# mauro3/KissMCMC.jl

Measured on AMD Instinct MI355X. Metric: walker-steps/sec, higher is better.
Workload: dtype f64

## Files before the change

include/kissmcmc_hip.h:

```cpp
#ifndef KISSMCMC_HIP_H
#define KISSMCMC_HIP_H

#include <stdint.h>

#ifdef __cplusplus
extern "C" {
#endif

#define KMC_VERSION 100

typedef enum kmc_status {
    KMC_OK = 0,
    KMC_ERR_A_SCALE = 1,
    KMC_ERR_ODD_WALKERS = 2,
    KMC_ERR_TOO_FEW_WALKERS = 3,
    KMC_ERR_BAD_ARG = 4,
    KMC_ERR_NONFINITE_LOGP = 5,
    KMC_ERR_HIP = 6,
    KMC_ERR_OOM = 7,
    KMC_ERR_NO_DEVICE = 8,
    KMC_ERR_UNSUPPORTED = 9
} kmc_status;

typedef enum kmc_density {
// ... 220 lines not shown
    int64_t  nchains;
    int64_t  ndim;
    int64_t  niter;
    int64_t  nburnin;
    int64_t  nthin;
    const double* step;
    uint64_t seed;
    uint32_t flags;
    int32_t  device;
    void*    user_density;
    kmc_host_logpdf_fn   host_logpdf;
    void*                host_user;
    kmc_host_accepted_fn host_accepted;
    kmc_host_propose_fn  host_propose;
} kmc_metropolis_config;

typedef struct kmc_metropolis_outputs {
    double*  chain;
    double*  chain_logp;
    double*  accept_ratio;
    int64_t* naccept;
    double*  final_pos;
    double*  final_logp;
    double*  chain_sum;
    double*  chain_sumsq;
    int64_t  nsamples;
    double   device_ms;
    double*  blobs;
    double*  final_blob;
} kmc_metropolis_outputs;

kmc_status  kmc_metropolis_validate(const kmc_metropolis_config* cfg);
kmc_status  kmc_metropolis_run(const kmc_metropolis_config* cfg, const double* theta0 ,
                               kmc_metropolis_outputs* out);

kmc_status  kmc_int_acorr(const double* chain_host, int64_t nsamples, int64_t nwalkers, int64_t ndim, double c ,
                          int device, double* tau , double* converged );
kmc_status  kmc_sampler_int_acorr(kmc_sampler* s, double c, double* tau, double* converged);

kmc_status  kmc_sampler_order_stats(kmc_sampler* s, int64_t first_sample, const uint8_t* walker_mask ,
                                    const int64_t* ranks, int32_t nranks,
                                    double* theta_out , double* logp_out , int64_t* n_out);
kmc_status  kmc_sampler_chain_argmax(kmc_sampler* s, int64_t first_sample, const uint8_t* walker_mask,
                                     int64_t* sample, int64_t* walker, double* theta , double* logp);
kmc_status  kmc_chain_order_stats(const double* chain_host , const double* logp_host ,
                                  int64_t nsamples, int64_t nwalkers, int64_t ndim, int64_t first_sample, const uint8_t* walker_mask,
                                  const int64_t* ranks, int32_t nranks, int device, double* theta_out, double* logp_out, int64_t* n_out);
kmc_status  kmc_chain_argmax(const double* chain_host, const double* logp_host, int64_t nsamples, int64_t nwalkers, int64_t ndim,
                             int64_t first_sample, const uint8_t* walker_mask, int device,
                             int64_t* sample, int64_t* walker, double* theta, double* logp);

kmc_status  kmc_sampler_histograms(kmc_sampler* s, int64_t first_sample, const uint8_t* walker_mask ,
                                   const int32_t* dims, int32_t ndims, const double* edges , int32_t nbins,
                                   int32_t with_logp, int64_t* counts1 , int64_t* outside ,
                                   int64_t* counts2 , int64_t* n_out);
kmc_status  kmc_chain_histograms(const double* chain_host , const double* logp_host ,
                                 int64_t nsamples, int64_t nwalkers, int64_t ndim, int64_t first_sample, const uint8_t* walker_mask,
                                 const int32_t* dims, int32_t ndims, const double* edges, int32_t nbins, int device,
                                 int64_t* counts1, int64_t* outside, int64_t* counts2, int64_t* n_out);
kmc_status  kmc_hist_pair_plan(int32_t ndims, int32_t nbins, int32_t* pairs_per_group, int32_t* ngroups, int32_t* lds_budget);

#define KMC_CONV_NEED_LAGS 1
#define KMC_CONV_TRUNCATED 2
kmc_status  kmc_sampler_lag_sums(kmc_sampler* s, int64_t first_sample, const uint8_t* walker_mask , int32_t split,
                                 int32_t with_logp, int64_t lag0, int64_t nlags, double* chain_mean, double* chain_var, double* lagsum,
                                 int64_t* m_out, int64_t* h_out);
kmc_status  kmc_chain_lag_sums(const double* chain_host , const double* logp_host ,
                               int64_t nsamples, int64_t nwalkers, int64_t ndim, int64_t first_sample, const uint8_t* walker_mask,
                               int32_t split, int64_t lag0, int64_t nlags, int device, double* chain_mean, double* chain_var,
                               double* lagsum, int64_t* m_out, int64_t* h_out);
kmc_status  kmc_convergence_stats(int64_t m, int64_t h, int64_t ncols, const double* chain_mean, const double* chain_var,
                                  const double* lagsum, int64_t nlags, int64_t max_lag, double* mean, double* W, double* B,
                                  double* var_plus, double* rhat, double* ess, double* mcse, int64_t* T, int32_t* flags);
kmc_status  kmc_sampler_convergence(kmc_sampler* s, int64_t first_sample, const uint8_t* walker_mask, int32_t split, int32_t with_logp,
                                    int64_t max_lag, double* mean, double* W, double* B, double* var_plus, double* rhat, double* ess,
                                    double* mcse, int64_t* T, int32_t* flags, int64_t* m_out, int64_t* h_out, int64_t* info);
kmc_status  kmc_convergence_plan(int32_t* lag_block, int32_t* tile_samples, int32_t* lanes, int32_t* lds_bytes);
kmc_status  kmc_chain_convergence(const double* chain_host, const double* logp_host , int64_t nsamples, int64_t nwalkers,
                                  int64_t ndim, int64_t first_sample, const uint8_t* walker_mask, int32_t split, int64_t max_lag,
                                  int device, double* mean, double* W, double* B, double* var_plus, double* rhat, double* ess,
                                  double* mcse, int64_t* T, int32_t* flags, int64_t* m_out, int64_t* h_out, int64_t* info);
kmc_status  kmc_convergence_plan(int32_t* lag_block, int32_t* tile_samples, int32_t* lanes, int32_t* lds_bytes);

#define KMC_CONV_HAS_NAN 4
kmc_status  kmc_rank_plan(int32_t* tile_keys, int32_t* digit_bits, int32_t* passes, int32_t* lds_bytes);
kmc_status  kmc_rank_normal_scores(const int64_t* rank2, int64_t n, int64_t S, double* z);
kmc_status  kmc_sampler_rank_scores(kmc_sampler* s, int64_t first_sample, const uint8_t* walker_mask , int32_t split,
                                    int32_t with_logp, int32_t folded, int64_t* rank2, double* z, double* centre, int64_t* nan_count,
                                    int64_t* m_out, int64_t* h_out);
kmc_status  kmc_chain_rank_scores(const double* chain_host , const double* logp_host ,
                                  int64_t nsamples, int64_t nwalkers, int64_t ndim, int64_t first_sample, const uint8_t* walker_mask,
                                  int32_t split, int32_t folded, int device, int64_t* rank2, double* z, double* centre,
                                  int64_t* nan_count, int64_t* m_out, int64_t* h_out);
kmc_status  kmc_sampler_rank_convergence(kmc_sampler* s, int64_t first_sample, const uint8_t* walker_mask, int32_t split, int32_t with_logp,
                                         int64_t max_lag, double* rhat, double* rhat_bulk, double* rhat_folded, double* ess_bulk,
                                         double* ess_tail, double* ess_q05, double* ess_q95, double* median, double* q05, double* q95,
                                         int64_t* T, int32_t* flags, int64_t* m_out, int64_t* h_out, int64_t* info);
kmc_status  kmc_chain_rank_convergence(const double* chain_host, const double* logp_host , int64_t nsamples, int64_t nwalkers,
                                       int64_t ndim, int64_t first_sample, const uint8_t* walker_mask, int32_t split, int64_t max_lag,
                                       int device, double* rhat, double* rhat_bulk, double* rhat_folded, double* ess_bulk,
                                       double* ess_tail, double* ess_q05, double* ess_q95, double* median, double* q05, double* q95,
                                       int64_t* T, int32_t* flags, int64_t* m_out, int64_t* h_out, int64_t* info);

kmc_status  kmc_sampler_covariance(kmc_sampler* s, int64_t first_sample, const uint8_t* walker_mask ,
                                   int32_t with_logp, double* mean, double* cov, int64_t* n_out, int64_t* info);
kmc_status  kmc_chain_covariance(const double* chain_host , const double* logp_host ,
                                 int64_t nsamples, int64_t nwalkers, int64_t ndim, int64_t first_sample, const uint8_t* walker_mask,
                                 int device, double* mean, double* cov, int64_t* n_out, int64_t* info);
kmc_status  kmc_cov_plan(int64_t ncols, int32_t* tile_cols, int32_t* strip_tiles, int32_t* nstrips, int32_t* rows_per_wave_block);
kmc_status  kmc_cov_correlation(int64_t ncols, const double* cov, double* corr, double* sd);

kmc_status  kmc_sampler_pointwise_stats(kmc_sampler* s, int64_t first_sample, const uint8_t* walker_mask ,
                                        int64_t thin, const double* data , int64_t ndata2, int32_t ncols2,
                                        double* stats, int64_t* n_out, int64_t* info);
kmc_status  kmc_chain_pointwise_stats(kmc_user_density* density, const double* params, const double* chain_host ,
                                      int64_t nsamples, int64_t nwalkers, int64_t ndim, int64_t first_sample, const uint8_t* walker_mask,
                                      int64_t thin, const double* data, int64_t ndata2, int32_t ncols2, int device, double* stats,
                                      int64_t* n_out, int64_t* info);
kmc_status  kmc_sampler_pointwise_loglike(kmc_sampler* s, int64_t first_sample, const uint8_t* walker_mask, int64_t thin, const double* data,
                                          int64_t ndata2, int32_t ncols2, int64_t obs_first, int64_t obs_count, double* out, int64_t* n_out);
kmc_status  kmc_chain_pointwise_loglike(kmc_user_density* density, const double* params, const double* chain_host, int64_t nsamples,
                                        int64_t nwalkers, int64_t ndim, int64_t first_sample, const uint8_t* walker_mask, int64_t thin,
                                        const double* data, int64_t ndata2, int32_t ncols2, int64_t obs_first, int64_t obs_count, int device,
                                        double* out, int64_t* n_out);
kmc_status  kmc_pointwise_plan(int64_t n, int64_t ndata, int64_t* run_len, int64_t* nruns, int32_t* lanes_per_run, int32_t* slots,
                               int64_t* nwaves);
kmc_status  kmc_waic_stats(int64_t J, int64_t n, const double* stats, double* lppd_j, double* p_waic_j, double* elpd_j, double* totals);

kmc_status  kmc_sampler_psis_loo(kmc_sampler* s, int64_t first_sample, const uint8_t* walker_mask , int64_t thin,
                                 double r_eff, int64_t obs_first, int64_t obs_count, int64_t workspace_bytes, double* stats, double* lppd_j,
                                 int64_t* n_out, int64_t* info);
kmc_status  kmc_chain_psis_loo(kmc_user_density* density, const double* params, const double* chain_host ,
                               int64_t nsamples, int64_t nwalkers, int64_t ndim, int64_t first_sample, const uint8_t* walker_mask, int64_t thin,
                               double r_eff, int64_t obs_first, int64_t obs_count, int64_t workspace_bytes, int device, double* stats,
                               double* lppd_j, int64_t* n_out, int64_t* info);
kmc_status  kmc_sampler_psis_tail(kmc_sampler* s, int64_t first_sample, const uint8_t* walker_mask, int64_t thin, double r_eff, int64_t obs_first,
                                  int64_t obs_count, int64_t workspace_bytes, double* tail, double* m_j, double* xc_j, int32_t* n_tail_j,
                                  int64_t* tail_len, int64_t* n_out);
kmc_status  kmc_chain_psis_tail(kmc_user_density* density, const double* params, const double* chain_host, int64_t nsamples, int64_t nwalkers,
                                int64_t ndim, int64_t first_sample, const uint8_t* walker_mask, int64_t thin, double r_eff, int64_t obs_first,
                                int64_t obs_count, int64_t workspace_bytes, int device, double* tail, double* m_j, double* xc_j,
                                int32_t* n_tail_j, int64_t* tail_len, int64_t* n_out);
kmc_status  kmc_psis_plan(int64_t n, int64_t ndata, double r_eff, int64_t workspace_bytes, int64_t* tail_len, int64_t* m_est,
                          int64_t* obs_per_block, int64_t* passes);
kmc_status  kmc_loo_stats(int64_t J, int64_t n, const double* stats, const double* lppd_j, double* p_loo_j, double* totals);
kmc_status  kmc_psis_smooth_host(int64_t nt, const double* x, double xc, double* k_hat, double* sigma, double* s, double* sums);

kmc_status  kmc_debug_accept_terms(uint64_t seed, uint64_t step, uint64_t walker0, int64_t n, int64_t nhalf, double a_scale,
                                   int64_t ndim, int device, int64_t* partner_host, double* z_host, double* t1_host, double* lu_host);
kmc_status  kmc_debug_chain_by_walker(const void* src_host, int is_float, int64_t K, int64_t nl, int64_t ld, int64_t nd, int64_t w0,
                                      int64_t nw, int64_t dst_stride, double* dst_host, int64_t dst_len, int device);
kmc_status  kmc_debug_rows_compact(const double* src_host, int64_t rows, int64_t ld, int64_t nd, double* dst_host, int64_t dst_len,
                                   int device);

#ifdef __cplusplus
}
#endif
#endif
```

kissmcmc.jl_amd/_lib.py:

```python
from __future__ import annotations

import ctypes as C
import os

_HERE = os.path.dirname(os.path.abspath(__file__))
LIB_PATH = os.environ.get("KMC_LIB_PATH") or os.path.join(_HERE, "libkissmcmc_hip.so")

OK, ERR_A_SCALE, ERR_ODD_WALKERS, ERR_TOO_FEW_WALKERS, ERR_BAD_ARG, ERR_NONFINITE_LOGP, \
    ERR_HIP, ERR_OOM, ERR_NO_DEVICE, ERR_UNSUPPORTED = range(10)
GAUSSIAN_ISO, EXPONENTIAL, ROSENBROCK, LOGNORMAL, MVNORMAL2 = range(5)
USER_DENSITY = 100
HOST_DENSITY = 101
DATA_DENSITY = 102
HOST_LOGPDF_FN = C.CFUNCTYPE(C.c_int, C.POINTER(C.c_double), C.c_int64, C.c_int64, C.POINTER(C.c_double), C.c_void_p)
HOST_PROPOSE_FN = C.CFUNCTYPE(C.c_int, C.POINTER(C.c_double), C.c_int64, C.c_int64, C.POINTER(C.c_double), C.c_void_p)
HOST_ACCEPTED_FN = C.CFUNCTYPE(C.c_int, C.POINTER(C.c_uint8), C.c_int64, C.c_int64, C.c_int64, C.c_int32, C.c_void_p)
F64 = 0
F32 = 1
STORE_CHAIN, STORE_LOGP, MOMENTS, NO_GRAPH, P2P, ISLANDS, P2P_FINEGRAINED, P2P_PUSH = 1, 2, 4, 8, 16, 64, 128, 512
STREAM_CHAIN = 2048
CHAIN_BY_WALKER = 4096
STORE_BLOBS = 8192
MOVE_STRETCH, MOVE_DE, MOVE_SNOOKER, MOVE_MIX = 0, 1, 3, 4
MIX_MAX = 4
TEMPS_MAX = 64
CONV_NEED_LAGS, CONV_TRUNCATED = 1, 2
CONV_HAS_NAN = 4
TEMPER_WHOLE, TEMPER_LIKELIHOOD = 0, 1
P2P_HANDLE_BYTES = 128
RCCL_ID_BYTES = 128

SYMBOLS = [
    "kmc_version", "kmc_device_count", "kmc_last_error", "kmc_status_string", "kmc_validate",
    "kmc_g_pdf", "kmc_cdf_g_inv", "kmc_emcee_run", "kmc_sampler_create", "kmc_sampler_destroy",
    "kmc_sampler_set_stream", "kmc_sampler_bind_positions", "kmc_sampler_p2p_export", "kmc_sampler_p2p_connect", "kmc_sampler_p2p_connect_local", "kmc_sampler_p2p_link_probe", "kmc_sampler_set_positions", "kmc_sampler_init_ball", "kmc_sampler_set_state", "kmc_sampler_run", "kmc_sampler_half_step",
    "kmc_sampler_sync", "kmc_sampler_last_run_ms", "kmc_sampler_generation", "kmc_sampler_nsamples",
    "kmc_sampler_launch_count", "kmc_sampler_describe", "kmc_sampler_device_ptr", "kmc_sampler_get_positions",
    "kmc_sampler_get_logp", "kmc_sampler_get_naccept", "kmc_sampler_get_accept_ratio",
    "kmc_sampler_get_moments", "kmc_sampler_get_chain", "kmc_sampler_get_chain_by_walker", "kmc_logpdf_eval", "kmc_logpdf_eval_host",
    "kmc_user_density_create", "kmc_user_density_create_body", "kmc_user_density_destroy", "kmc_metropolis_validate", "kmc_metropolis_run", "kmc_int_acorr", "kmc_sampler_int_acorr",
    "kmc_sizeof_config", "kmc_sizeof_metropolis_config", "kmc_sizeof_outputs", "kmc_sizeof_metropolis_outputs", "kmc_deal_seed", "kmc_deal_perm", "kmc_sampler_deal_pack", "kmc_sampler_deal_unpack",
    "kmc_sampler_get_walker_ids", "kmc_sampler_set_walker_ids", "kmc_sampler_set_chain_host", "kmc_rccl_unique_id", "kmc_sampler_rccl_init",
    "kmc_sampler_rccl_capture", "kmc_sampler_rccl_set_capture", "kmc_rccl_version", "kmc_device_free_bytes",
    "kmc_sampler_launch_mode", "kmc_updated_budget", "kmc_set_updated_budget_mb", "kmc_debug_accept_terms",
    "kmc_debug_chain_by_walker", "kmc_debug_rows_compact",
    "kmc_user_density_create_body_blob", "kmc_user_density_nblob", "kmc_logpdf_blob_eval_host", "kmc_sampler_get_blobs",
    "kmc_device_cache_release", "kmc_user_density_is_separable", "kmc_host_prefault", "kmc_data_density_create",
    "kmc_sampler_get_rung_state", "kmc_sampler_set_rung_state", "kmc_sampler_get_swaps",
    "kmc_sampler_get_rung_loglike", "kmc_sampler_set_rung_loglike_sum", "kmc_sampler_get_ladder", "kmc_sampler_set_ladder",
    "kmc_sampler_order_stats", "kmc_sampler_chain_argmax", "kmc_chain_order_stats", "kmc_chain_argmax",
    "kmc_sampler_histograms", "kmc_chain_histograms", "kmc_hist_pair_plan",
    "kmc_sampler_lag_sums", "kmc_chain_lag_sums", "kmc_convergence_stats", "kmc_sampler_convergence", "kmc_chain_convergence",
    "kmc_convergence_plan",
    "kmc_rank_plan", "kmc_rank_normal_scores", "kmc_sampler_rank_scores", "kmc_chain_rank_scores", "kmc_sampler_rank_convergence",
    "kmc_chain_rank_convergence",
    "kmc_sampler_covariance", "kmc_chain_covariance", "kmc_cov_plan", "kmc_cov_correlation",
    "kmc_sampler_pointwise_stats", "kmc_chain_pointwise_stats", "kmc_sampler_pointwise_loglike", "kmc_chain_pointwise_loglike",
    "kmc_pointwise_plan", "kmc_waic_stats",
    "kmc_sampler_psis_loo", "kmc_chain_psis_loo", "kmc_sampler_psis_tail", "kmc_chain_psis_tail", "kmc_psis_plan", "kmc_loo_stats",
    "kmc_psis_smooth_host",
]


class Config(C.Structure):
    _fields_ = [
        ("dtype", C.c_int32),
        ("density", C.c_int32),
        ("params", C.c_double * 8),
        ("nwalkers", C.c_int64),
        ("ndim", C.c_int64),
        ("ngenerations", C.c_int64),
        ("nburnin", C.c_int64),
        ("nthin", C.c_int64),
        ("a_scale", C.c_double),
        ("seed", C.c_uint64),
        ("flags", C.c_uint32),
        ("device", C.c_int32),
        ("shard_rank", C.c_int32),
        ("shard_count", C.c_int32),
        ("user_density", C.c_void_p),
        ("island_gens", C.c_int32),
        ("island_size", C.c_int32),
        ("host_logpdf", C.c_void_p),
        ("host_user", C.c_void_p),
        ("host_accepted", C.c_void_p),
        ("deal_rank", C.c_int32),
        ("deal_count", C.c_int32),
        ("temper_mode", C.c_int32),
        ("temper_pad_", C.c_int32),
        ("adapt_until", C.c_int64),
        ("adapt_lag", C.c_double),
        ("adapt_time", C.c_double),
        ("adapt", C.c_int32),
        ("adapt_pad_", C.c_int32),
        ("snooker_gamma", C.c_double),
        ("mix_count", C.c_int32),
        ("mix_move0", C.c_int32), ("mix_move1", C.c_int32), ("mix_move2", C.c_int32), ("mix_move3", C.c_int32),
        ("mix_pad0_", C.c_int32), ("mix_pad1_", C.c_int32), ("mix_pad2_", C.c_int32),
        ("mix_weight0", C.c_double), ("mix_weight1", C.c_double), ("mix_weight2", C.c_double), ("mix_weight3", C.c_double),
        ("mix_gamma0", C.c_double), ("mix_gamma1", C.c_double), ("mix_gamma2", C.c_double), ("mix_gamma3", C.c_double),
        ("mix_sigma0", C.c_double), ("mix_sigma1", C.c_double), ("mix_sigma2", C.c_double), ("mix_sigma3", C.c_double),
        ("betas", C.c_void_p),
        ("ntemps", C.c_int32),
        ("swap_every", C.c_int32),
        ("move", C.c_int32),
        ("move_pad_", C.c_int32),
        ("de_gamma0", C.c_double),
        ("de_sigma", C.c_double),
    ]


class Outputs(C.Structure):
    _fields_ = [
        ("chain", C.POINTER(C.c_double)),
        ("chain_logp", C.POINTER(C.c_double)),
        ("accept_ratio", C.POINTER(C.c_double)),
        ("naccept", C.POINTER(C.c_int64)),
        ("final_pos", C.POINTER(C.c_double)),
        ("final_logp", C.POINTER(C.c_double)),
        ("sum", C.POINTER(C.c_double)),
        ("sumsq", C.POINTER(C.c_double)),
        ("nmoment", C.c_int64),
        ("nsamples", C.c_int64),
        ("device_ms", C.c_double),
        ("blobs", C.POINTER(C.c_double)),
    ]


class MetropolisConfig(C.Structure):
    _fields_ = [
        ("dtype", C.c_int32),
        ("density", C.c_int32),
        ("params", C.c_double * 8),
        ("nchains", C.c_int64),
        ("ndim", C.c_int64),
        ("niter", C.c_int64),
        ("nburnin", C.c_int64),
        ("nthin", C.c_int64),
        ("step", C.POINTER(C.c_double)),
        ("seed", C.c_uint64),
        ("flags", C.c_uint32),
        ("device", C.c_int32),
        ("user_density", C.c_void_p),
        ("host_logpdf", C.c_void_p),
        ("host_user", C.c_void_p),
        ("host_accepted", C.c_void_p),
        ("host_propose", C.c_void_p),
    ]


class MetropolisOutputs(C.Structure):
    _fields_ = [
        ("chain", C.POINTER(C.c_double)),
        ("chain_logp", C.POINTER(C.c_double)),
        ("accept_ratio", C.POINTER(C.c_double)),
        ("naccept", C.POINTER(C.c_int64)),
        ("final_pos", C.POINTER(C.c_double)),
        ("final_logp", C.POINTER(C.c_double)),
        ("chain_sum", C.POINTER(C.c_double)),
        ("chain_sumsq", C.POINTER(C.c_double)),
        ("nsamples", C.c_int64),
        ("device_ms", C.c_double),
        ("blobs", C.POINTER(C.c_double)),
        ("final_blob", C.POINTER(C.c_double)),
    ]


class KmcError(RuntimeError):

    def __init__(self, status: int, message: str):
        super().__init__(message)
        self.status = status


_lib = None


def lib() -> C.CDLL:
    global _lib
    if _lib is not None:
        return _lib
    if "no-torch-preload" not in os.environ.get("KMC_DEBUG", "").split(","):
        try:
            import torch
        except Exception:
            pass
    if not os.path.exists(LIB_PATH):
        raise ImportError(
            f"{LIB_PATH} is missing: build it with `python -m kissmcmc_jl_amd.build` "
            "(hipcc --offload-arch=gfx950). The emcee hot path has no CPU fallback.")
    L = C.CDLL(LIB_PATH)
    dp = C.POINTER(C.c_double)
    ip = C.POINTER(C.c_int64)
    vp = C.c_void_p
    cfgp = C.POINTER(Config)
    L.kmc_version.restype = C.c_int
    L.kmc_device_count.restype = C.c_int
    L.kmc_last_error.restype = C.c_char_p
    L.kmc_status_string.restype = C.c_char_p
    L.kmc_status_string.argtypes = [C.c_int]
    L.kmc_validate.argtypes = [cfgp]
    L.kmc_g_pdf.restype = C.c_double
    L.kmc_g_pdf.argtypes = [C.c_double, C.c_double]
    L.kmc_cdf_g_inv.restype = C.c_double
    L.kmc_cdf_g_inv.argtypes = [C.c_double, C.c_double]
    L.kmc_emcee_run.argtypes = [cfgp, dp, C.POINTER(Outputs)]
    L.kmc_sampler_create.argtypes = [cfgp, C.POINTER(vp)]
    L.kmc_sampler_destroy.restype = None
    L.kmc_sampler_destroy.argtypes = [vp]
    L.kmc_sampler_set_stream.argtypes = [vp, vp]
    L.kmc_sampler_bind_positions.argtypes = [vp, vp]
    L.kmc_sampler_p2p_export.argtypes = [vp, vp]
    L.kmc_sampler_p2p_connect.argtypes = [vp, vp]
    L.kmc_sampler_p2p_connect_local.argtypes = [vp, C.POINTER(C.c_void_p)]
    L.kmc_sampler_p2p_link_probe.argtypes = [vp, C.c_int, C.c_int64, C.c_int, C.POINTER(C.c_double), C.POINTER(C.c_double)]
    L.kmc_sampler_set_positions.argtypes = [vp, dp]
    L.kmc_sampler_init_ball.argtypes = [vp, dp, dp, C.c_uint64, C.c_int, C.c_int]
    L.kmc_sampler_set_state.argtypes = [vp, dp, dp, ip, C.c_int64]
    L.kmc_sampler_get_rung_state.argtypes = [vp, dp, dp, ip, dp]
    L.kmc_sampler_set_rung_state.argtypes = [vp, dp, dp, ip, C.POINTER(C.c_uint64), dp, C.c_int64]
    L.kmc_sampler_get_swaps.argtypes = [vp, C.POINTER(C.c_uint64)]
    L.kmc_sampler_get_rung_loglike.argtypes = [vp, dp, dp, dp]
    L.kmc_sampler_set_rung_loglike_sum.argtypes = [vp, dp]
    L.kmc_sampler_get_ladder.argtypes = [vp, dp, dp, C.POINTER(C.c_uint64), C.POINTER(C.c_uint64)]
    L.kmc_sampler_set_ladder.argtypes = [vp, dp, dp, C.POINTER(C.c_uint64), C.POINTER(C.c_uint64)]
    L.kmc_sampler_run.argtypes = [vp, C.c_int64]
    L.kmc_sampler_half_step.argtypes = [vp, C.c_int]
    L.kmc_sampler_sync.argtypes = [vp]
    L.kmc_sampler_last_run_ms.argtypes = [vp, dp]
    L.kmc_sampler_generation.restype = C.c_int64
    L.kmc_sampler_generation.argtypes = [vp]
    L.kmc_sampler_nsamples.restype = C.c_int64
    L.kmc_sampler_nsamples.argtypes = [vp]
    L.kmc_sampler_launch_count.restype = C.c_int64
    L.kmc_sampler_launch_count.argtypes = [vp]
    L.kmc_sampler_describe.argtypes = [vp, C.c_char_p, C.c_int64]
    L.kmc_sampler_device_ptr.restype = vp
    L.kmc_sampler_device_ptr.argtypes = [vp, C.c_int]
    L.kmc_sampler_get_positions.argtypes = [vp, dp]
    L.kmc_sampler_get_logp.argtypes = [vp, dp]
    L.kmc_sampler_get_naccept.argtypes = [vp, ip]
    L.kmc_sampler_get_accept_ratio.argtypes = [vp, dp]
    L.kmc_sampler_get_moments.argtypes = [vp, dp, dp, ip]
    L.kmc_sampler_get_chain.argtypes = [vp, dp, dp]
    L.kmc_sampler_get_chain_by_walker.argtypes = [vp, dp, dp]
    L.kmc_logpdf_eval.argtypes = [cfgp, vp, vp, C.c_int64, vp]
    L.kmc_logpdf_eval_host.argtypes = [cfgp, dp, dp, C.c_int64]
    L.kmc_user_density_create.argtypes = [C.c_char_p, C.c_char_p, C.POINTER(vp)]
    L.kmc_user_density_create_body.argtypes = [C.c_char_p, C.POINTER(vp)]
    L.kmc_user_density_create_body_blob.argtypes = [C.c_char_p, C.c_int, C.POINTER(vp)]
    L.kmc_data_density_create.argtypes = [C.c_char_p, C.c_char_p, C.POINTER(C.c_double), C.c_int64, C.c_int32, C.POINTER(vp)]
    L.kmc_user_density_is_separable.restype = C.c_int
    L.kmc_user_density_is_separable.argtypes = [vp]
    L.kmc_user_density_nblob.restype = C.c_int
    L.kmc_user_density_nblob.argtypes = [vp]
    L.kmc_logpdf_blob_eval_host.argtypes = [cfgp, dp, dp, dp, C.c_int64]
    L.kmc_sampler_get_blobs.argtypes = [vp, dp, dp, C.c_int]
    L.kmc_user_density_destroy.restype = None
    L.kmc_user_density_destroy.argtypes = [vp]
    L.kmc_metropolis_validate.argtypes = [C.POINTER(MetropolisConfig)]
    L.kmc_metropolis_run.argtypes = [C.POINTER(MetropolisConfig), dp, C.POINTER(MetropolisOutputs)]
    L.kmc_int_acorr.argtypes = [dp, C.c_int64, C.c_int64, C.c_int64, C.c_double, C.c_int, dp, dp]
    L.kmc_sampler_int_acorr.argtypes = [vp, C.c_double, dp, dp]
    bp = C.POINTER(C.c_uint8)
    L.kmc_sampler_order_stats.argtypes = [vp, C.c_int64, bp, ip, C.c_int32, dp, dp, ip]
    L.kmc_sampler_chain_argmax.argtypes = [vp, C.c_int64, bp, ip, ip, dp, dp]
    L.kmc_chain_order_stats.argtypes = [dp, dp, C.c_int64, C.c_int64, C.c_int64, C.c_int64, bp, ip, C.c_int32, C.c_int, dp, dp, ip]
    L.kmc_chain_argmax.argtypes = [dp, dp, C.c_int64, C.c_int64, C.c_int64, C.c_int64, bp, C.c_int, ip, ip, dp, dp]
    i32p = C.POINTER(C.c_int32)
    L.kmc_sampler_histograms.argtypes = [vp, C.c_int64, bp, i32p, C.c_int32, dp, C.c_int32, C.c_int32, ip, ip, ip, ip]
    L.kmc_chain_histograms.argtypes = [dp, dp, C.c_int64, C.c_int64, C.c_int64, C.c_int64, bp, i32p, C.c_int32, dp, C.c_int32, C.c_int, ip, ip, ip, ip]
    L.kmc_hist_pair_plan.argtypes = [C.c_int32, C.c_int32, i32p, i32p, i32p]
    L.kmc_sampler_lag_sums.argtypes = [vp, C.c_int64, bp, C.c_int32, C.c_int32, C.c_int64, C.c_int64, dp, dp, dp, ip, ip]
    L.kmc_chain_lag_sums.argtypes = [dp, dp, C.c_int64, C.c_int64, C.c_int64, C.c_int64, bp, C.c_int32, C.c_int64, C.c_int64, C.c_int, dp, dp, dp, ip, ip]
    L.kmc_convergence_stats.argtypes = [C.c_int64, C.c_int64, C.c_int64, dp, dp, dp, C.c_int64, C.c_int64, dp, dp, dp, dp, dp, dp, dp, ip, i32p]
    L.kmc_sampler_convergence.argtypes = [vp, C.c_int64, bp, C.c_int32, C.c_int32, C.c_int64, dp, dp, dp, dp, dp, dp, dp, ip, i32p, ip, ip, ip]
    L.kmc_chain_convergence.argtypes = [dp, dp, C.c_int64, C.c_int64, C.c_int64, C.c_int64, bp, C.c_int32, C.c_int64, C.c_int, dp, dp, dp, dp, dp, dp, dp, ip, i32p, ip, ip, ip]
    L.kmc_convergence_plan.argtypes = [i32p, i32p, i32p, i32p]
    L.kmc_rank_plan.argtypes = [i32p, i32p, i32p, i32p]
    L.kmc_rank_normal_scores.argtypes = [ip, C.c_int64, C.c_int64, dp]
    L.kmc_sampler_rank_scores.argtypes = [vp, C.c_int64, bp, C.c_int32, C.c_int32, C.c_int32, ip, dp, dp, ip, ip, ip]
    L.kmc_chain_rank_scores.argtypes = [dp, dp, C.c_int64, C.c_int64, C.c_int64, C.c_int64, bp, C.c_int32, C.c_int32, C.c_int, ip, dp, dp, ip, ip, ip]
    L.kmc_sampler_rank_convergence.argtypes = [vp, C.c_int64, bp, C.c_int32, C.c_int32, C.c_int64] + [dp] * 10 + [ip, i32p, ip, ip, ip]
    L.kmc_chain_rank_convergence.argtypes = [dp, dp, C.c_int64, C.c_int64, C.c_int64, C.c_int64, bp, C.c_int32, C.c_int64, C.c_int] + [dp] * 10 + [ip, i32p, ip, ip, ip]
    L.kmc_sampler_covariance.argtypes = [vp, C.c_int64, bp, C.c_int32, dp, dp, ip, ip]
    L.kmc_chain_covariance.argtypes = [dp, dp, C.c_int64, C.c_int64, C.c_int64, C.c_int64, bp, C.c_int, dp, dp, ip, ip]
    L.kmc_cov_plan.argtypes = [C.c_int64, i32p, i32p, i32p, i32p]
    L.kmc_cov_correlation.argtypes = [C.c_int64, dp, dp, dp]
    held_out = [dp, C.c_int64, C.c_int32]
    host_chain = [vp, dp, dp, C.c_int64, C.c_int64, C.c_int64, C.c_int64, bp, C.c_int64]
    L.kmc_sampler_pointwise_stats.argtypes = [vp, C.c_int64, bp, C.c_int64] + held_out + [dp, ip, ip]
    L.kmc_chain_pointwise_stats.argtypes = host_chain + held_out + [C.c_int, dp, ip, ip]
    L.kmc_sampler_pointwise_loglike.argtypes = [vp, C.c_int64, bp, C.c_int64] + held_out + [C.c_int64, C.c_int64, dp, ip]
    L.kmc_chain_pointwise_loglike.argtypes = host_chain + held_out + [C.c_int64, C.c_int64, C.c_int, dp, ip]
    L.kmc_pointwise_plan.argtypes = [C.c_int64, C.c_int64, ip, ip, i32p, i32p, ip]
    L.kmc_waic_stats.argtypes = [C.c_int64, C.c_int64, dp, dp, dp, dp, dp]
    psis_sel = [C.c_double, C.c_int64, C.c_int64, C.c_int64]
    L.kmc_sampler_psis_loo.argtypes = [vp, C.c_int64, bp, C.c_int64] + psis_sel + [dp, dp, ip, ip]
    L.kmc_chain_psis_loo.argtypes = host_chain + psis_sel + [C.c_int, dp, dp, ip, ip]
    L.kmc_sampler_psis_tail.argtypes = [vp, C.c_int64, bp, C.c_int64] + psis_sel + [dp, dp, dp, i32p, ip, ip]
    L.kmc_chain_psis_tail.argtypes = host_chain + psis_sel + [C.c_int, dp, dp, dp, i32p, ip, ip]
    L.kmc_psis_plan.argtypes = [C.c_int64, C.c_int64, C.c_double, C.c_int64, ip, ip, ip, ip]
    L.kmc_loo_stats.argtypes = [C.c_int64, C.c_int64, dp, dp, dp, dp]
    L.kmc_psis_smooth_host.argtypes = [C.c_int64, dp, C.c_double, dp, dp, dp, dp]
    L.kmc_deal_seed.restype = C.c_uint64
    L.kmc_deal_seed.argtypes = [C.c_uint64, C.c_int32]
    L.kmc_deal_perm.argtypes = [C.c_uint64, C.c_int64, C.c_int32, C.c_int64, ip, ip]
    L.kmc_sampler_deal_pack.argtypes = [vp, C.c_int64, vp]
    L.kmc_sampler_deal_unpack.argtypes = [vp, vp]
    L.kmc_sampler_get_walker_ids.argtypes = [vp, ip]
    L.kmc_sampler_set_walker_ids.argtypes = [vp, ip]
    L.kmc_sampler_set_chain_host.argtypes = [vp, dp, dp]
    L.kmc_rccl_unique_id.argtypes = [vp]
    L.kmc_sampler_rccl_init.argtypes = [vp, vp]
    L.kmc_sampler_rccl_capture.argtypes = [vp, C.POINTER(C.c_int)]
    L.kmc_sampler_rccl_set_capture.argtypes = [vp, C.c_int]
    L.kmc_rccl_version.argtypes = [C.POINTER(C.c_int), C.c_char_p, C.c_int64]
    L.kmc_device_free_bytes.argtypes = [C.c_int, C.POINTER(C.c_uint64), C.POINTER(C.c_uint64)]
    L.kmc_device_cache_release.argtypes = []
    L.kmc_device_cache_release.restype = None
    L.kmc_host_prefault.argtypes = [C.c_void_p, C.c_uint64, C.c_int]
    L.kmc_host_prefault.restype = None
    L.kmc_sampler_launch_mode.restype = C.c_int
    L.kmc_sampler_launch_mode.argtypes = [vp, C.POINTER(C.c_int)]
    L.kmc_updated_budget.restype = None
    L.kmc_updated_budget.argtypes = [ip, ip]
    L.kmc_set_updated_budget_mb.restype = None
    L.kmc_set_updated_budget_mb.argtypes = [C.c_double]
    L.kmc_debug_accept_terms.argtypes = [C.c_uint64, C.c_uint64, C.c_uint64, C.c_int64, C.c_int64, C.c_double, C.c_int64, C.c_int, ip, dp, dp, dp]
    L.kmc_debug_chain_by_walker.argtypes = [vp, C.c_int, C.c_int64, C.c_int64, C.c_int64, C.c_int64, C.c_int64, C.c_int64, C.c_int64, dp, C.c_int64, C.c_int]
    L.kmc_debug_rows_compact.argtypes = [dp, C.c_int64, C.c_int64, C.c_int64, dp, C.c_int64, C.c_int]
    for fn, T in ((L.kmc_sizeof_config, Config), (L.kmc_sizeof_metropolis_config, MetropolisConfig),
                  (L.kmc_sizeof_outputs, Outputs), (L.kmc_sizeof_metropolis_outputs, MetropolisOutputs)):
        if fn() != C.sizeof(T):
            raise ImportError(f"{LIB_PATH}: struct layout mismatch ({fn.__name__}() = {fn()}, the ctypes mirror {T.__name__} is {C.sizeof(T)} bytes): "
                              "rebuild the library or update kissmcmc_jl_amd/_lib.py from include/kissmcmc_hip.h")
    _lib = L
    return L


def check(status: int) -> None:
    if status != OK:
        L = lib()
        msg = L.kmc_last_error().decode() or L.kmc_status_string(status).decode()
        raise KmcError(status, msg)
```

kissmcmc.jl_amd/build.py:

```python
from __future__ import annotations

import os
import shutil
import subprocess

_HERE = os.path.dirname(os.path.abspath(__file__))
CSRC = os.path.join(_HERE, "csrc")
LIB = os.path.join(_HERE, "libkissmcmc_hip.so")
SOURCES = ["kmc_sampler.hip", "kmc_plan.hip", "kmc_launch.hip", "kmc_updated.hip", "kmc_state.hip", "kmc_copy.hip", "kmc_rtc.hip", "kmc_p2p.hip", "kmc_metropolis_api.hip", "kmc_acorr.hip", "kmc_summary.hip", "kmc_hist.hip", "kmc_convergence.hip", "kmc_rank.hip", "kmc_cov.hip", "kmc_pointwise.hip", "kmc_rccl.hip", "kmc_diag.hip", "kmc_inst_host.hip", "kmc_inst_host_temper.hip", "kmc_inst_host_temper_snooker.hip", "kmc_data.hip"] + \
          [f"kmc_inst_{d}{part}.hip" for part in ("", "_var", "_p2p", "_lds", "_de", "_snooker", "_temper", "_temper_snooker") for d in ("lognormal", "exponential", "gaussian_iso", "rosenbrock", "mvnormal2")]
HEADERS = ["kmc_psis_fit.hpp", "kmc_host.hpp", "kmc_sampler.hpp", "kmc_device.hpp", "kmc_kernels.hpp", "kmc_islands.hpp", "kmc_generation.hpp", "kmc_copy_kernels.hpp", "kmc_summary_kernels.hpp", "kmc_hist_kernels.hpp", "kmc_convergence_kernels.hpp", "kmc_convergence_host.hpp", "kmc_rank_kernels.hpp", "kmc_cov_kernels.hpp", "kmc_chain_view.hpp", "kmc_chain_kernels.hpp", "kmc_metropolis.hpp", "kmc_tables.hpp", "kmc_recognise.hpp", "kmc_data.hpp", "kmc_pointwise.hpp", os.path.join("..", "..", "include", "kissmcmc_hip.h")]
PRELOAD = ["-mllvm", "-amdgpu-kernarg-preload-count=14"]
FLAGS = ["--offload-arch=gfx950", "-O3", "-std=c++17", "-fPIC", "-ffp-contract=off",
         "-fvisibility=hidden", "-Wall", "-Wno-unused-function"]


def _hipcc() -> str:
    for c in (shutil.which("hipcc"), "/opt/rocm/bin/hipcc"):
        if c and os.path.exists(c):
            return c
    raise RuntimeError("hipcc not found: the HIP library cannot be built")




def stale(lib: str = LIB) -> bool:
    if not os.path.exists(lib):
        return True
    t = os.path.getmtime(lib)
    deps = [os.path.join(CSRC, f) for f in SOURCES + HEADERS]
    return any(os.path.getmtime(d) > t for d in deps)


def build(force: bool = False, verbose: bool = False, extra_flags=(), out: str = LIB, preload: bool = True) -> str:
    if not (force or out != LIB or stale()):
        return out
    from concurrent.futures import ThreadPoolExecutor
    hipcc = _hipcc()
    objdir = os.path.join(_HERE, "build_obj" + ("" if out == LIB else "_" + os.path.basename(out)))
    os.makedirs(objdir, exist_ok=True)

    def compile_one(src):
        obj = os.path.join(objdir, os.path.splitext(src)[0] + ".o")
        cmd = [hipcc, *FLAGS, *(PRELOAD if preload else ()), *extra_flags, "-c", os.path.join(CSRC, src), "-o", obj]
        if verbose:
            print(" ".join(cmd))
        subprocess.check_call(cmd)
        return obj

    order = sorted(SOURCES, key=lambda f: not f.startswith("kmc_inst_"))
    with ThreadPoolExecutor(max_workers=min(len(SOURCES), os.cpu_count() or 1)) as ex:
        objs = list(ex.map(compile_one, order))
    cmd = [hipcc, "--offload-arch=gfx950", "-shared", "-fPIC", *objs, "-o", out + ".tmp", "-lhiprtc", "-ldl"]
    if verbose:
        print(" ".join(cmd))
    subprocess.check_call(cmd)
    os.replace(out + ".tmp", out)
    shutil.rmtree(objdir, ignore_errors=True)
    return out


if __name__ == "__main__":
    print(build(force=True, verbose=True))
```

kissmcmc.jl_amd/csrc/kmc_kernels.hpp:

```cpp
#pragma once
#include "kmc_device.hpp"

namespace kmc {

constexpr int kTPB = 256;
__host__ __device__ constexpr int vec_tpb(int L) { return L <= 8 ? 128 : L == 16 ? 64 : kTPB; }

struct SchedEntry {
    int64_t  gen;
    int64_t  slot;
    uint32_t flags;
    uint32_t nbefore;
    uint32_t pad_[2];
};
static_assert(sizeof(SchedEntry) == 32, "schedule_of loads an entry as eight dwords");
enum : uint32_t { kCount = 1u, kSample = 2u };

__host__ __device__ inline SchedEntry make_sched(int64_t gen, int64_t nburnin, int64_t nthin, int64_t nsamples, int64_t ring_slots = 0)
{
    SchedEntry e{gen, 0, 0u, 0u, {0u, 0u}};
    const int64_t n = gen + 1 - nburnin;
    if (n > 1) {
        const int64_t nb = (n - 1) / nthin;
        e.nbefore = (uint32_t)(nb < nsamples ? nb : nsamples);
    }
    if (n > 0) {
        e.flags |= kCount;
        if (n % nthin == 0) {
            const int64_t k = n / nthin - 1;
            if (k < nsamples) { e.flags |= kSample; e.slot = ring_slots > 0 ? k % ring_slots : k; }
        }
    }
    return e;
}

struct HalfStepArgs {
    double*           pos;
    double*           logp;
    uint32_t*         naccept;
    const SchedEntry* sched_table;
    SchedEntry        sched_inline;
    int32_t           sched_index;
    int32_t           half;
    int64_t           gw0;
    int64_t           own_row0;
    int64_t           oth_row0;
    int32_t           n_active;
    int32_t           ndim;
    int32_t           ld;
    int32_t           hloc_shift;
    uint32_t          hloc;
    int32_t           nranks;
    double*           peer_pos[8];
    const unsigned long long* flags;
    unsigned long long* err;
    DrawConsts        dc;
    DensityParams     dp;
    double*           chain;
    double*           chain_logp;
    int64_t           chain_rows;
    int64_t           chain_row0;
    double*           msum;
    double*           msumsq;
    int64_t           macc_stride;
    uint32_t*         klast;
    double2*          ring;
    int64_t           ring_rows;
    int32_t           ring_slot;
    int32_t           prop_ld;
    double*           prop_out;
    const double*     p1_in;
    unsigned char*    acc_out;
    double2*          mring;
    double*           mring_w;
    uint32_t*         mcnt;
    const uint32_t*   mswept;
    int32_t           mring_depth;
    double*           blob;
    double*           chain_blob;
};

__host__ __device__ inline int32_t pack_ranks(int nranks, int me, bool push) { return (int32_t)(nranks | (me << 8) | (push ? 1 << 16 : 0)); }
__device__ __forceinline__ int  p2p_nranks(const HalfStepArgs& a) { return a.nranks & 0xff; }
__device__ __forceinline__ int  p2p_me(const HalfStepArgs& a) { return (a.nranks >> 8) & 0xff; }
__device__ __forceinline__ bool p2p_push(const HalfStepArgs& a) { return ((a.nranks >> 16) & 1) != 0; }

struct HalfStepFront {
    double*           pos;
    const SchedEntry* sched;
    const double2*    ring_now;
    double*           logp;
    uint32_t          gw0;
    uint32_t          nact_half;
    uint32_t          seed_lo, seed_hi, nhalf;
    uint32_t          step;
    __host__ __device__ int32_t n_active() const { return (int32_t)(nact_half & 0x7fffffffu); }
    __host__ __device__ int32_t half() const { return (int32_t)(nact_half >> 31); }
};
#define KMC_FRONT_PARAMS double* f_pos, const kmc::SchedEntry* f_sched, const double2* f_ring_now, double* f_logp, uint32_t f_gw0, \
                         uint32_t f_nact_half, uint32_t f_seed_lo, uint32_t f_seed_hi, uint32_t f_nhalf, uint32_t f_step
#define KMC_FRONT_PACK kmc::HalfStepFront{f_pos, f_sched, f_ring_now, f_logp, f_gw0, f_nact_half, f_seed_lo, f_seed_hi, f_nhalf, f_step}
#define KMC_FRONT_TYPES double*, const kmc::SchedEntry*, const double2*, double*, uint32_t, uint32_t, uint32_t, uint32_t, uint32_t, uint32_t

__device__ __forceinline__ SchedEntry schedule_entry(const HalfStepFront& f)
{
    typedef uint32_t u32x8 __attribute__((ext_vector_type(8)));
    u32x8 r;
    asm volatile("s_load_dwordx8 %0, %1, 0x0\n\ts_waitcnt lgkmcnt(0)" : "=s"(r) : "s"(f.sched));
    SchedEntry t;
    t.gen     = (int64_t)(((uint64_t)r[1] << 32) | r[0]);
    t.slot    = (int64_t)(((uint64_t)r[3] << 32) | r[2]);
    t.flags   = r[4];
    t.nbefore = r[5];
    return t;
}
__device__ __forceinline__ SchedEntry schedule_of(const HalfStepFront& f, const HalfStepArgs& a)
{
    if (f.sched == nullptr) return a.sched_inline;
    return schedule_entry(f);
}

__device__ __forceinline__ void store_wt(double2* p, const double2& v)
{
    typedef double v2d __attribute__((ext_vector_type(2)));
    const v2d t = {v.x, v.y};
    asm volatile("global_store_dwordx4 %0, %1, off sc0 sc1\n\ts_nop 1" :: "v"(p), "v"(t) : "memory");
}
__device__ __forceinline__ void store_wt(double* p, double v)
{
    asm volatile("global_store_dwordx2 %0, %1, off sc0 sc1\n\ts_nop 1" :: "v"(p), "v"(v) : "memory");
}
__device__ __forceinline__ void store_wt(uint32_t* p, uint32_t v)
{
    asm volatile("global_store_dword %0, %1, off sc0 sc1\n\ts_nop 0" :: "v"(p), "v"(v) : "memory");
}
__device__ __forceinline__ void store_wt(unsigned char* p, unsigned char v)
{
    const uint32_t t = v;
    asm volatile("global_store_byte %0, %1, off sc0 sc1\n\ts_nop 0" :: "v"(p), "v"(t) : "memory");
}
__device__ __forceinline__ double2 load_row16(const double2* p)
{
    return *p;
}

template <class T> struct RowOf;
template <> struct RowOf<double> { using V2 = double2; };
template <> struct RowOf<float>  { using V2 = float2; };
__device__ __forceinline__ void store_wt(float2* p, const float2& v)
{
    typedef float v2f __attribute__((ext_vector_type(2)));
    const v2f t = {v.x, v.y};
    asm volatile("global_store_dwordx2 %0, %1, off sc0 sc1\n\ts_nop 1" :: "v"(p), "v"(t) : "memory");
}
__device__ __forceinline__ double2 load_row(const double2* p) { return load_row16(p); }
__device__ __forceinline__ double2 load_row(const float2* p) { const float2 v = *p; return make_double2((double)v.x, (double)v.y); }
__device__ __forceinline__ void store_row(double2* p, const double2& v) { store_wt(p, v); }
__device__ __forceinline__ void store_row(float2* p, const double2& v) { store_wt(p, make_float2((float)v.x, (float)v.y)); }
template <class T> __device__ __forceinline__ double as_stored(double v)
{
    if constexpr (sizeof(T) == 4) return (double)(float)v; else return v;
}

__device__ __forceinline__ double2 sel2(bool c, const double2& a, const double2& b)
{
    return make_double2(c ? a.x : b.x, c ? a.y : b.y);
}

template <int L, int K>
struct FoldT {
    static constexpr bool on = (K == 2) && (L == 8 || L == 16 || L == 32);
    static constexpr int NVL = on ? (8 * L) / 64 : 1;
};

__device__ __forceinline__ double swap16_sum(double a, double b)
{
    const auto lo = __builtin_amdgcn_permlane16_swap((unsigned)__double2loint(a), (unsigned)__double2loint(b), false, false);
    const auto hi = __builtin_amdgcn_permlane16_swap((unsigned)__double2hiint(a), (unsigned)__double2hiint(b), false, false);
    return __hiloint2double((int)hi[0], (int)lo[0]) + __hiloint2double((int)hi[1], (int)lo[1]);
}
__device__ __forceinline__ double swap32_sum(double a, double b)
{
    const auto lo = __builtin_amdgcn_permlane32_swap((unsigned)__double2loint(a), (unsigned)__double2loint(b), false, false);
    const auto hi = __builtin_amdgcn_permlane32_swap((unsigned)__double2hiint(a), (unsigned)__double2hiint(b), false, false);
    return __hiloint2double((int)hi[0], (int)lo[0]) + __hiloint2double((int)hi[1], (int)lo[1]);
}

template <int L, int K>
__device__ __forceinline__ void fold_scatter(int lane, const double2 (&ms)[K], const double2 (&mq)[K], double (&v)[8])
{
    static_assert(FoldT<L, K>::on, "K == 2, L = 8 / 16 / 32");
    {
        v[0] = ms[0].x; v[1] = ms[0].y; v[2] = ms[1].x; v[3] = ms[1].y; v[4] = mq[0].x; v[5] = mq[0].y; v[6] = mq[1].x; v[7] = mq[1].y;
        int n = 8;
        if constexpr (L == 8) {
            const bool hi = (lane & 8) != 0;
#pragma unroll
            for (int i = 0; i < 4; ++i) {
                double lo_v = v[i], hi_v = v[i + 4];
                asm volatile("" : "+v"(lo_v), "+v"(hi_v));
                const double keep = hi ? hi_v : lo_v, send = hi ? lo_v : hi_v;
                v[i] = keep + dpp_f64<0x128>(send);
            }
            n = 4;
        }
        if constexpr (L <= 16) {
#pragma unroll
            for (int i = 0; i < 4; ++i) if (i < n / 2) v[i] = swap16_sum(v[i], v[i + n / 2]);
            n /= 2;
        }
#pragma unroll
        for (int i = 0; i < 4; ++i) if (i < n / 2) v[i] = swap32_sum(v[i], v[i + n / 2]);
    }
}

template <int L, int K, bool HAVE_OLD>
__device__ __forceinline__ void accumulate_wave(double* msum, double* msumsq, int64_t stride, int tid, int g,
                                                double2 (&ms)[K], double2 (&mq)[K],
                                                const double2 (&olds)[K], const double2 (&oldq)[K], const double (&oldt)[4])
{
    if constexpr (FoldT<L, K>::on) {
        constexpr int NVL = FoldT<L, K>::NVL;
        const int lane = tid & 63;
        double v[8];
        fold_scatter<L, K>(lane, ms, mq, v);
        double* slot = msum + ((int64_t)(tid >> 6) * NVL) * 64 + lane;
#pragma unroll
        for (int r = 0; r < NVL; ++r) store_wt(&slot[r * 64], (HAVE_OLD ? oldt[r] : slot[r * 64]) + v[r]);
        return;
    }
    if constexpr (L < 64) {
#pragma unroll
        for (int k = 0; k < K; ++k) {
            ms[k].x = wave_fold<L>(ms[k].x); ms[k].y = wave_fold<L>(ms[k].y);
            mq[k].x = wave_fold<L>(mq[k].x); mq[k].y = wave_fold<L>(mq[k].y);
        }
    }
    if (g == 0) {
        double2* s = reinterpret_cast<double2*>(msum);
        double2* q = reinterpret_cast<double2*>(msumsq);
#pragma unroll
        for (int k = 0; k < K; ++k) {
            const int64_t idx = (int64_t)k * stride + tid;
            const double2 sv = HAVE_OLD ? olds[k] : s[idx], qv = HAVE_OLD ? oldq[k] : q[idx];
            if constexpr (HAVE_OLD) {
                store_wt(&s[idx], make_double2(sv.x + ms[k].x, sv.y + ms[k].y));
                store_wt(&q[idx], make_double2(qv.x + mq[k].x, qv.y + mq[k].y));
            } else {
                s[idx] = make_double2(sv.x + ms[k].x, sv.y + ms[k].y);
                q[idx] = make_double2(qv.x + mq[k].x, qv.y + mq[k].y);
            }
        }
    }
}

__device__ __forceinline__ void wait_for_peers(const HalfStepArgs& a, unsigned long long need, int lane)
{
    const int nranks = p2p_nranks(a);
    bool ok = lane >= nranks ||
              __hip_atomic_load(a.flags + lane, __ATOMIC_RELAXED, __HIP_MEMORY_SCOPE_SYSTEM) >= need;
    unsigned spins = 0;
    if (__hip_atomic_load(a.err, __ATOMIC_RELAXED, __HIP_MEMORY_SCOPE_AGENT) != 0ull) ok = true;
    while (!__all(ok)) {
        __builtin_amdgcn_s_sleep(2);
        ok = lane >= nranks ||
             __hip_atomic_load(a.flags + lane, __ATOMIC_RELAXED, __HIP_MEMORY_SCOPE_SYSTEM) >= need;
        if (++spins > 30000000u) {
            if (lane == 0) __hip_atomic_store(a.err, need + 1ull, __ATOMIC_RELAXED, __HIP_MEMORY_SCOPE_AGENT);
            break;
        }
    }
    __builtin_amdgcn_fence(__ATOMIC_ACQUIRE, "wavefront");
}

__device__ __forceinline__ double2 load_row_sys(const double2* p)
{
    const unsigned long long* q = reinterpret_cast<const unsigned long long*>(p);
    const unsigned long long lo = __hip_atomic_load(q, __ATOMIC_RELAXED, __HIP_MEMORY_SCOPE_SYSTEM);
    const unsigned long long hi = __hip_atomic_load(q + 1, __ATOMIC_RELAXED, __HIP_MEMORY_SCOPE_SYSTEM);
    return make_double2(__longlong_as_double((long long)lo), __longlong_as_double((long long)hi));
}

#ifdef KMC_PROBE
static __device__ unsigned long long g_probe[2][8192][8];
#define KMC_STAMP_AT(lo, hi) asm volatile("s_memrealtime s[" #lo ":" #hi "]" ::: "s" #lo, "s" #hi, "memory")
#define KMC_STAMP(i) KMC_STAMP_##i
#define KMC_STAMP_0 KMC_STAMP_AT(80, 81)
#define KMC_STAMP_7 KMC_STAMP_AT(94, 95)
#if KMC_PROBE == 2
#define KMC_PROBE_PINS 0
#define KMC_STAMP_1 do { } while (0)
#define KMC_STAMP_2 do { } while (0)
#define KMC_STAMP_3 do { } while (0)
#define KMC_STAMP_4 do { } while (0)
#define KMC_STAMP_5 do { } while (0)
#define KMC_STAMP_6 do { } while (0)
#define KMC_STAMP_READ(dst, lo, hi) do { if ((lo) == 80 || (lo) == 94) asm volatile("s_mov_b64 %0, s[" #lo ":" #hi "]" : "=s"(dst)); else (dst) = 0ull; } while (0)
#else
#define KMC_PROBE_PINS 1
#define KMC_STAMP_1 KMC_STAMP_AT(82, 83)
#define KMC_STAMP_2 KMC_STAMP_AT(84, 85)
#define KMC_STAMP_3 KMC_STAMP_AT(86, 87)
#define KMC_STAMP_4 KMC_STAMP_AT(88, 89)
#define KMC_STAMP_5 KMC_STAMP_AT(90, 91)
#define KMC_STAMP_6 KMC_STAMP_AT(92, 93)
#define KMC_STAMP_READ(dst, lo, hi) asm volatile("s_mov_b64 %0, s[" #lo ":" #hi "]" : "=s"(dst))
#endif
#else
#define KMC_PROBE_PINS 0
#define KMC_STAMP(i) do { } while (0)
#endif

template <class Dens, int L, int K, int ITER, bool P2P, bool RAGGED, class T = double, Move M = Move::Stretch, bool TEMPER = false>
__device__ __forceinline__ void half_step_vec_body(const HalfStepFront& f, const HalfStepArgs& a, const DrawConsts* over = nullptr)
{
    static_assert(!TEMPER || (!P2P && sizeof(T) == 8 && BlobTrait<Dens>::n == 0), "tempering: one GPU, double rows, no blobs (kmc_validate)");
    const uint32_t rung = TEMPER ? (uint32_t)blockIdx.y : 0u;
    const uint32_t rung_w0 = TEMPER ? rung * (2u * f.nhalf) : 0u;
    static_assert(M != Move::Mix, "a mixture picks its member in front of the body (half_step_mix_vec_body)");
    static_assert(L >= 1 && L <= 64 && (L & (L - 1)) == 0, "L must be a power of two <= 64");
    static_assert(!P2P || sizeof(T) == 8, "the peer-to-peer kernels keep double rows");
    constexpr bool kDE = M == Move::DE;
    constexpr bool kSnk = M == Move::Snooker;
    constexpr bool kOwn = kDE || kSnk;
    static_assert(!kOwn || (!P2P && sizeof(T) == 8 && BlobTrait<Dens>::n == 0), "the DE move: one GPU, double rows, no blobs (kmc_validate)");
    using V2 = typename RowOf<T>::V2;
    T* const posT = reinterpret_cast<T*>(f.pos);
    static_assert(ITER >= 1 && ITER <= L, "a group's scalar lanes must cover its iterations");
    constexpr int G = 64 / L;
    constexpr int W = G * ITER;
    const uint64_t ndim_tag = RAGGED ? reinterpret_cast<uint64_t>(f.logp) >> 48 : 0ull;
    double* const logp_p = RAGGED ? reinterpret_cast<double*>(reinterpret_cast<char*>(f.logp) - (ndim_tag << 48)) : f.logp;
    const int ndim = RAGGED ? (int)ndim_tag : 2 * L * K;
    const int64_t ld = RAGGED ? (int64_t)((ndim + 1) & ~1) : (int64_t)(2 * L * K);
    const int tid   = blockIdx.x * vec_tpb(L) + threadIdx.x;
    const int lane  = threadIdx.x & 63;
    const int j     = lane & (L - 1);
    const int g     = lane / L;
    const int gbase = lane & ~(L - 1);
    const int w0    = (tid >> 6) * W;
    const int nact  = f.n_active();
    const int half  = f.half();
    const int64_t own_row0 = P2P ? (int64_t)half * nact : (int64_t)f.gw0;
    bool cv[K];
#pragma unroll
    for (int k = 0; k < K; ++k) cv[k] = !RAGGED || 2 * (k * L + j) < (int)ld;
    int ck[K];
#pragma unroll
    for (int k = 0; k < K; ++k) ck[k] = cv[k] ? k * L + j : (int)(ld >> 1) - 1;
    auto row_off = [&](int64_t row) -> int64_t { return RAGGED ? (int64_t)((uint64_t)(uint32_t)row * (uint64_t)(uint32_t)ld) : row * ld; };
    const double2 zero2 = make_double2(0.0, 0.0);
    KMC_STAMP(0);

    constexpr int Q = (L / ITER) >= 4 ? 4 : (L / ITER);
    constexpr bool kRing = !kOwn && Q >= 2 && L >= 16 && L <= 32;
    const int64_t oth_row0 = (int64_t)(1 - half) * (int64_t)(P2P ? (uint32_t)nact : f.nhalf);
    const int  jq     = j / ITER, js = j - jq * ITER;
    const bool useA   = jq == 0;
    const int  iA     = w0 + (kOwn || jq < Q ? js : 0) * G + g;
    const bool validA = useA && (iA < nact);
    const int      iAc = iA < nact ? iA : nact - 1;
    const int64_t  rowA = own_row0 + iAc;
    const bool ring_on = kRing && f.ring_now != nullptr;
    double2 e0 = zero2, e1 = zero2;
    if constexpr (kRing) {
        if (ring_on && useA) { e0 = f.ring_now[2 * rowA]; e1 = f.ring_now[2 * rowA + 1]; }
    }

    bool    validB[ITER];
    double2 xc[ITER][K], xo[ITER][K];
    double2 xk[ITER][K];
    double2 xl[ITER][K];
#pragma unroll
    for (int it = 0; it < ITER; ++it) {
        const int i = w0 + it * G + g;
        validB[it] = i < nact;
        const V2* own = reinterpret_cast<const V2*>(posT + row_off(own_row0 + (validB[it] ? i : nact - 1)));
#pragma unroll
        for (int k = 0; k < K; ++k) xc[it][k] = load_row(&own[ck[k]]);
    }

    const int64_t nrows_blk = 2 * (int64_t)(P2P ? (uint32_t)nact : f.nhalf);
    uint32_t* const naccept_p = reinterpret_cast<uint32_t*>(logp_p + nrows_blk);
    uint32_t* const klast_p = naccept_p + nrows_blk;
    const double   p0 = logp_p[rowA];
    const uint32_t na = naccept_p[rowA];
    const uint32_t kl = klast_p[rowA];

    const bool eager = f.sched == nullptr;
    SchedEntry sch_t{0, 0, 0u, 0u, {0u, 0u}};
    if (!eager) sch_t = schedule_entry(f);
    const uint64_t step = eager ? (uint64_t)f.step : 2ull * (uint64_t)sch_t.gen + (uint64_t)half;
    DrawConsts dcf{};
    dcf.seed_lo = f.seed_lo; dcf.seed_hi = f.seed_hi; dcf.nhalf = f.nhalf;
    const uint32_t e1y_lo = (uint32_t)__double2loint(e1.y), e1y_hi = (uint32_t)__double2hiint(e1.y);
    const bool fresh = ring_on && __all(!useA || e1y_hi == (uint32_t)step);
    U4 bits{0u, 0u, 0u, 0u};
    uint32_t partnerA = e1y_lo;
    uint32_t partnerK = 0u;
    uint32_t partnerL = 0u;
    if constexpr (kSnk) {
        bits = de_bits(f.seed_lo, f.seed_hi, step, f.gw0 + (uint32_t)iAc + rung_w0, 2u);
        snooker_partners(bits, f.nhalf, &partnerA, &partnerK, &partnerL);
    } else if constexpr (kDE) {
        bits = de_bits(f.seed_lo, f.seed_hi, step, f.gw0 + (uint32_t)iAc + rung_w0, 0u);
        partnerA = __umulhi(bits.x, f.nhalf);
        partnerK = de_partner_k(bits.y, f.nhalf, partnerA);
    } else if (!fresh) {
        bits = draw_bits(dcf, step + 2ull * (uint64_t)jq, (uint64_t)f.gw0 + (uint64_t)iAc + (uint64_t)rung_w0);
        partnerA = draw_partner(dcf, bits);
    }
#if KMC_PROBE_PINS
    if constexpr (!kOwn) asm volatile("" :: "v"(partnerA));
#endif
    KMC_STAMP(1);

    unsigned long long addrA = 0ull;
    const int nranks = P2P ? p2p_nranks(a) : 1, me_rank = P2P ? p2p_me(a) : 0;
    const bool push = P2P && p2p_push(a);
    const int64_t shard_stride = 2 * (int64_t)a.hloc * ld;
    auto load_partner_rows = [&](int it) {
        const V2* oth;
        const V2* othk = nullptr;
        const V2* othl = nullptr;
        if constexpr (!P2P) {
            const uint32_t partner = (uint32_t)__builtin_amdgcn_ds_bpermute((gbase + it) * 4, (int)partnerA);
            const uint32_t pk = kOwn ? (uint32_t)__builtin_amdgcn_ds_bpermute((gbase + it) * 4, (int)partnerK) : 0u;
            oth = reinterpret_cast<const V2*>(posT + row_off(oth_row0 + partner));
            if constexpr (kOwn) othk = reinterpret_cast<const V2*>(posT + row_off(oth_row0 + pk));
            if constexpr (kSnk) {
                const uint32_t pl = (uint32_t)__builtin_amdgcn_ds_bpermute((gbase + it) * 4, (int)partnerL);
                othl = reinterpret_cast<const V2*>(posT + row_off(oth_row0 + pl));
            }
        } else {
            const int src = (gbase + it) * 4;
            const unsigned lo = (unsigned)__builtin_amdgcn_ds_bpermute(src, (int)(unsigned)addrA);
            const unsigned hi = (unsigned)__builtin_amdgcn_ds_bpermute(src, (int)(unsigned)(addrA >> 32));
            const unsigned long long ad = ((unsigned long long)hi << 32) | lo;
            oth = reinterpret_cast<const V2*>(ad);
        }
        if constexpr (P2P) {
            if (nranks > 1) {
#pragma unroll
                for (int k = 0; k < K; ++k) xo[it][k] = load_row_sys(reinterpret_cast<const double2*>(&oth[ck[k]]));
                return;
            }
        }
#pragma unroll
        for (int k = 0; k < K; ++k) xo[it][k] = load_row(&oth[ck[k]]);
        if constexpr (kOwn) {
#pragma unroll
            for (int k = 0; k < K; ++k) xk[it][k] = load_row(&othk[ck[k]]);
        }
        if constexpr (kSnk) {
#pragma unroll
            for (int k = 0; k < K; ++k) xl[it][k] = load_row(&othl[ck[k]]);
        }
    };
    if constexpr (P2P) {
        const uint32_t q = a.hloc_shift >= 0 ? partnerA >> a.hloc_shift : partnerA / a.hloc;
        const uint32_t r = partnerA - q * a.hloc;
        const double* base = a.peer_pos[0];
#pragma unroll
        for (int t = 1; t < 8; ++t) base = (q == (uint32_t)t) ? a.peer_pos[t] : base;
        if (push) base = (q == (uint32_t)me_rank) ? a.pos : a.pos + (int64_t)(1u + q) * shard_stride;
        addrA = (unsigned long long)(base + (oth_row0 + r) * ld);
        if (nranks > 1) {
            if ((threadIdx.x >> 6) == 0) wait_for_peers(a, step, lane);
            __syncthreads();
        }
    }
    constexpr int kFirst = ITER >= 2 && !kSnk ? ITER / 2 : ITER;
#pragma unroll
    for (int it = 0; it < kFirst; ++it) load_partner_rows(it);
    __builtin_amdgcn_sched_barrier(0);
    KMC_STAMP(2);

    asm volatile("" :: "s"(a.chain), "s"(a.chain_logp), "s"(a.chain_rows), "s"(a.chain_row0),
                 "s"(a.msum), "s"(a.msumsq), "s"(a.macc_stride), "s"(a.sched_inline.gen), "s"(a.sched_inline.slot),
                 "s"(a.sched_inline.flags), "s"(a.sched_inline.nbefore));
    int eager_late = eager ? 1 : 0;
    asm volatile("" : "+v"(eager_late));
    eager_late = __builtin_amdgcn_readfirstlane(eager_late);
    SchedEntry sch = sch_t;
    if (eager_late != 0) sch = a.sched_inline;
    const bool count  = (sch.flags & kCount) != 0;
    const bool sample = (sch.flags & kSample) != 0 && (!TEMPER || rung == 0u);
    double beta = 1.0;
    if constexpr (TEMPER) beta = reinterpret_cast<const double*>(a.peer_pos[1])[rung];
    DrawConsts dc = a.dc;
    dc.seed_lo = f.seed_lo; dc.seed_hi = f.seed_hi; dc.nhalf = f.nhalf;
    if (over != nullptr) { dc.c0 = over->c0; dc.c1 = over->c1; }
    const bool do_mom = count && a.msum != nullptr && (!TEMPER || rung == 0u);
    constexpr bool kPrefetchAcc = K <= 2 && L != 64;
    constexpr bool kMomRing = !kPrefetchAcc && !FoldT<L, K>::on && L == 64;
    if constexpr (kMomRing) asm volatile("" :: "s"(a.mring), "s"(a.mring_w), "s"(a.mcnt), "s"(a.mswept), "s"(a.mring_depth));
    double2 accs[K], accq[K];
    double  acct[4] = {0.0, 0.0, 0.0, 0.0};
    constexpr bool kWgFold = FoldT<L, K>::on && vec_tpb(L) > 64 && ITER >= 4;
    const bool acc_owner = !kWgFold || (threadIdx.x >> 6) == 0;
    if constexpr (FoldT<L, K>::on) {
        if (do_mom && acc_owner) {
#pragma unroll
            for (int r = 0; r < FoldT<L, K>::NVL; ++r) acct[r] = a.msum[((int64_t)(tid >> 6) * FoldT<L, K>::NVL + r) * 64 + lane];
        }
    } else if constexpr (kPrefetchAcc) {
        if (do_mom && g == 0) {
#pragma unroll
            for (int k = 0; k < K; ++k) {
                const int64_t idx = (int64_t)k * a.macc_stride + tid;
                accs[k] = reinterpret_cast<const double2*>(a.msum)[idx];
                accq[k] = reinterpret_cast<const double2*>(a.msumsq)[idx];
            }
        }
    }
    uint32_t ring_posted = 0u, ring_swept = 0u;
    if constexpr (kMomRing) {
        if (do_mom && a.mring != nullptr) { ring_posted = a.mcnt[tid >> 6]; ring_swept = a.mswept[tid >> 6]; }
    }
#if KMC_PROBE_PINS
    if constexpr (!kOwn) asm volatile("" :: "s"(count ? 1 : 0), "s"(a.dc.c0));
#endif
    KMC_STAMP(3);
    Draw dr;
    dr.partner = partnerA; dr.z = e1.x; dr.t1 = e0.x; dr.lu = e0.y;
    double ua = 0.5;
    if constexpr (kSnk) {
        bits = de_bits(f.seed_lo, f.seed_hi, step, f.gw0 + (uint32_t)iAc + rung_w0, 3u);
        dr.z = dc.c0;
        dr.t1 = 0.0;
    } else if constexpr (kDE) {
        const U4 b1 = de_bits(f.seed_lo, f.seed_hi, step, f.gw0 + (uint32_t)iAc + rung_w0, 1u);
        dr.z = de_gamma(dc, b1.x);
        dr.t1 = 0.0;
    } else if (!fresh) {
        const double uz = ((double)bits.y + 0.5) * 0x1.0p-32;
        const double t  = fma(uz, dc.c1, dc.c0);
        dr.z = t * t;
        const uint64_t kk = ((uint64_t)bits.z << 20) | (uint64_t)(bits.w >> 12);
        ua = ((double)kk + 0.5) * 0x1.0p-52;
        dr.t1 = dc.nm1 * log_pos_normal(dr.z);
    }
    __builtin_amdgcn_sched_barrier(0);
#pragma unroll
    for (int it = kFirst; it < ITER; ++it) load_partner_rows(it);
    __builtin_amdgcn_sched_barrier(0);
    if constexpr (kOwn) {
        dr.lu = log_pos_normal(de_accept_u(bits));
    } else if (!fresh) {
        dr.lu = log_pos_normal(ua);
        if constexpr (kRing) {
            if (ring_on && jq >= 1 && jq < Q && iA < nact) {
                double2* slot = a.ring + ((int64_t)((a.ring_slot + jq) & 3) * a.ring_rows + rowA) * 2;
                store_wt(&slot[0], make_double2(dr.t1, dr.lu));
                store_wt(&slot[1], make_double2(dr.z, __hiloint2double((int)(uint32_t)(step + 2ull * (uint64_t)jq), (int)dr.partner)));
            }
        }
    }
#if KMC_PROBE_PINS
    if constexpr (!kOwn) asm volatile("" :: "v"(dr.lu), "v"(dr.t1));
#endif
    KMC_STAMP(4);
    double zB[ITER];
#pragma unroll
    for (int it = 0; it < ITER; ++it) zB[it] = kSnk ? dc.c0 : bperm_f64((gbase + it) * 4, dr.z);

    double myp1 = 0.0;
    double mys = 0.0;
    constexpr int kRowND = RowEvalTrait<Dens>::n;
    double blob1[BlobTrait<Dens>::n > 0 ? BlobTrait<Dens>::n : 1];
#pragma unroll
    for (int it = 0; it < ITER; ++it) {
        if constexpr (kSnk) {
            double vn[K], vq[K];
#pragma unroll
            for (int k = 0; k < K; ++k) {
                const int e0 = 2 * (k * L + j);
                const double dx = xc[it][k].x - xo[it][k].x, dy = xc[it][k].y - xo[it][k].y;
                const double nx = dx * dx, ny = dy * dy;
                const double qx = dx * (xk[it][k].x - xl[it][k].x), qy = dy * (xk[it][k].y - xl[it][k].y);
                vn[k] = group_sum<L>(((e0 < ndim) ? nx : 0.0) + ((e0 + 1 < ndim) ? ny : 0.0));
                vq[k] = group_sum<L>(((e0 < ndim) ? qx : 0.0) + ((e0 + 1 < ndim) ? qy : 0.0));
                xo[it][k] = make_double2(dx, dy);
            }
#pragma unroll
            for (int w = 1; w < K; w *= 2) {
#pragma unroll
                for (int k = 0; k + w < K; k += 2 * w) { vn[k] = vn[k] + vn[k + w]; vq[k] = vq[k] + vq[k + w]; }
            }
            const double sB = snooker_s(zB[it], vq[0] + 0.0, vn[0] + 0.0);
            mys = (j == it) ? sB : mys;
            zB[it] = sB;
        }
#pragma unroll
        for (int k = 0; k < K; ++k) {
            if constexpr (kSnk) {
                xo[it][k].x = xc[it][k].x + xo[it][k].x * zB[it];
                xo[it][k].y = xc[it][k].y + xo[it][k].y * zB[it];
            } else if constexpr (kDE) {
                xo[it][k].x = xc[it][k].x + zB[it] * (xo[it][k].x - xk[it][k].x);
                xo[it][k].y = xc[it][k].y + zB[it] * (xo[it][k].y - xk[it][k].y);
            } else {
                xo[it][k].x = as_stored<T>(fma(zB[it], xc[it][k].x - xo[it][k].x, xo[it][k].x));
                xo[it][k].y = as_stored<T>(fma(zB[it], xc[it][k].y - xo[it][k].y, xo[it][k].y));
            }
        }
        if constexpr (MultiSumTrait<Dens>::n > 0) {
            double S[MultiSumTrait<Dens>::n];
            Dens::template frag_partial_n<L, K>(xo[it], j, ndim, a.dp, S);
#pragma unroll
            for (int q = 0; q < MultiSumTrait<Dens>::n; ++q) S[q] = group_sum<L>(S[q]);
            const double p1 = Dens::finish_n(S, a.dp);
            myp1 = (j == it) ? p1 : myp1;
        } else if constexpr (kRowND == 0) {
            const double S  = group_sum<L>(Dens::template frag_partial<L, K>(xo[it], j, ndim, a.dp));
            const double p1 = Dens::finish(S, a.dp);
            myp1 = (j == it) ? p1 : myp1;
        }
    }
    if constexpr (kRowND > 0) {
        extern __shared__ __attribute__((aligned(16))) double vec_rows[];
        constexpr int TS = 2 * L * K + 2;
        double* tile = vec_rows + (size_t)(threadIdx.x >> 6) * (size_t)(W * TS);
#pragma unroll
        for (int it = 0; it < ITER; ++it) {
#pragma unroll
            for (int k = 0; k < K; ++k)
                *reinterpret_cast<double2*>(&tile[(it * G + g) * TS + 2 * (k * L + j)]) = xo[it][k];
        }
        __builtin_amdgcn_fence(__ATOMIC_RELEASE, "wavefront");
        __builtin_amdgcn_wave_barrier();
        __builtin_amdgcn_fence(__ATOMIC_ACQUIRE, "wavefront");
        if constexpr (BlobTrait<Dens>::n > 0) {
            if (useA) {
#pragma unroll 1
                for (int i = 0; i < BlobTrait<Dens>::n; ++i) blob1[i] = 0.0;
                myp1 = Dens::eval_row(&tile[(js * G + g) * TS], ndim, a.dp, blob1);
            }
        } else {
            if (useA) myp1 = Dens::eval_row(&tile[(js * G + g) * TS], ndim, a.dp);
        }
    }

#if KMC_PROBE_PINS
    if constexpr (!kOwn) asm volatile("" :: "v"(myp1));
#endif
    KMC_STAMP(5);
    bool snk_ok = true;
    if constexpr (kSnk) snk_ok = snooker_hastings(dr, dc.nm1, mys);
    const bool acc = validA && snk_ok && (TEMPER ? accept_test_beta<M>(dr, myp1, p0, beta) : kDE ? de_accept_test(dr, myp1, p0) : accept_test(dr, myp1, p0));
    const unsigned long long accmask = __ballot(acc);
    if (acc) {
        store_wt(&logp_p[rowA], myp1);
        if (count) store_wt(&naccept_p[rowA], na + 1u);
        if (do_mom) store_wt(&klast_p[rowA], sch.nbefore);
    }
    if constexpr (BlobTrait<Dens>::n > 0) {
        constexpr int NB = BlobTrait<Dens>::n;
        const bool keep = validA && sample && a.chain_blob != nullptr;
        if (acc || keep) {
            double* cur = a.blob + rowA * NB;
            double* dst = a.chain_blob + (sch.slot * a.chain_rows + a.chain_row0 + iA) * NB;
#pragma unroll 1
            for (int i = 0; i < NB; ++i) {
                const double b = acc ? blob1[i] : cur[i];
                if (acc) cur[i] = b;
                if (keep) dst[i] = b;
            }
        }
    }
    const uint32_t wA = (acc && do_mom) ? sch.nbefore - kl : 0u;
    const bool any_w = __ballot(wA != 0u) != 0ull;
    if (sample && a.chain_logp != nullptr && validA)
        store_wt(&a.chain_logp[sch.slot * a.chain_rows + a.chain_row0 + iA], acc ? myp1 : p0);

    KMC_STAMP(6);
    double2 ms[K], mq[K];
#pragma unroll
    for (int k = 0; k < K; ++k) { ms[k] = make_double2(0.0, 0.0); mq[k] = make_double2(0.0, 0.0); }
    const bool use_ring = kMomRing && a.mring != nullptr && ring_posted - ring_swept + (uint32_t)ITER <= (uint32_t)a.mring_depth;
    uint32_t ring_new = 0u;
#pragma unroll
    for (int it = 0; it < ITER; ++it) {
        const bool accB = ((accmask >> (gbase + it)) & 1ull) != 0;
        if (accB) {
            V2* own = reinterpret_cast<V2*>(posT + row_off(own_row0 + w0 + it * G + g));
#pragma unroll
            for (int k = 0; k < K; ++k) store_row(&own[ck[k]], xo[it][k]);
            if constexpr (P2P) {
                if (push) {
                    const int64_t off = (int64_t)(1 + me_rank) * shard_stride + (own_row0 + w0 + it * G + g) * ld;
                    for (int r = 0; r < nranks; ++r) {
                        if (r == me_rank) continue;
                        double2* rem = reinterpret_cast<double2*>(a.peer_pos[r] + off);
#pragma unroll
                        for (int k = 0; k < K; ++k) if (cv[k]) store_wt(&rem[k * L + j], xo[it][k]);
                    }
                }
            }
        }
        if (any_w) {
            const double wB = (double)(uint32_t)__builtin_amdgcn_ds_bpermute((gbase + it) * 4, (int)wA);
            if (use_ring) {
                if (wB != 0.0) {
                    const int64_t e = (int64_t)(tid >> 6) * a.mring_depth + (int64_t)((ring_posted + ring_new) % (uint32_t)a.mring_depth);
                    double2* slot = a.mring + e * K * 64 + lane;
#pragma unroll
                    for (int k = 0; k < K; ++k) slot[k * 64] = xc[it][k];
                    if (lane == 0) a.mring_w[e] = wB;
                    ring_new += 1u;
                }
            } else {
#pragma unroll
                for (int k = 0; k < K; ++k) {
                    ms[k].x += xc[it][k].x * wB; ms[k].y += xc[it][k].y * wB;
                    mq[k].x += (xc[it][k].x * xc[it][k].x) * wB; mq[k].y += (xc[it][k].y * xc[it][k].y) * wB;
                }
            }
        }
        if (sample && a.chain != nullptr && validB[it]) {
            V2* dst = reinterpret_cast<V2*>(reinterpret_cast<T*>(a.chain) + (sch.slot * a.chain_rows + a.chain_row0 + w0 + it * G + g) * ld);
#pragma unroll
            for (int k = 0; k < K; ++k) store_row(&dst[ck[k]], sel2(accB, xo[it][k], xc[it][k]));
        }
    }
    if constexpr (kWgFold) {
        if (do_mom) {
            constexpr int NVL = FoldT<L, K>::NVL, NWV = vec_tpb(L) / 64;
            __shared__ double wg_fold[NWV - 1][NVL][64];
            const int wv = (int)(threadIdx.x >> 6);
            double v[8] = {0.0, 0.0, 0.0, 0.0, 0.0, 0.0, 0.0, 0.0};
            if (any_w) fold_scatter<L, K>(lane, ms, mq, v);
            if (wv != 0) {
#pragma unroll
                for (int r = 0; r < NVL; ++r) wg_fold[wv - 1][r][lane] = v[r];
            }
            lds_barrier();
            if (wv == 0) {
                double* slot = a.msum + ((int64_t)(tid >> 6) * NVL) * 64 + lane;
#pragma unroll
                for (int r = 0; r < NVL; ++r) {
                    double t = v[r];
#pragma unroll
                    for (int w = 0; w < NWV - 1; ++w) t += wg_fold[w][r][lane];
                    store_wt(&slot[r * 64], acct[r] + t);
                }
            }
        }
    } else if (any_w) {
        if (use_ring) {
            if (lane == 0) a.mcnt[tid >> 6] = ring_posted + ring_new;
        } else {
            if constexpr (kPrefetchAcc) accumulate_wave<L, K, true>(a.msum, a.msumsq, a.macc_stride, tid, g, ms, mq, accs, accq, acct);
            else accumulate_wave<L, K, false>(a.msum, a.msumsq, a.macc_stride, tid, g, ms, mq, accs, accq, acct);
        }
    }
    KMC_STAMP(7);
#ifdef KMC_PROBE
    if constexpr (!kOwn) {
        unsigned long long st[8];
        asm volatile("s_waitcnt lgkmcnt(0)" ::: "memory");
        KMC_STAMP_READ(st[0], 80, 81); KMC_STAMP_READ(st[1], 82, 83); KMC_STAMP_READ(st[2], 84, 85); KMC_STAMP_READ(st[3], 86, 87);
        KMC_STAMP_READ(st[4], 88, 89); KMC_STAMP_READ(st[5], 90, 91); KMC_STAMP_READ(st[6], 92, 93); KMC_STAMP_READ(st[7], 94, 95);
        if (lane == 0 && (tid >> 6) < 8192) for (int q = 0; q < 8; q += (KMC_PROBE == 2 ? 7 : 1)) g_probe[half][tid >> 6][q] = st[q];
    }
#endif
}

template <class Dens, int L, int K, int ITER, bool P2P, bool RAGGED, class T = double>
__global__ __launch_bounds__(vec_tpb(L)) void half_step_vec(KMC_FRONT_PARAMS, const HalfStepArgs a)
{
    half_step_vec_body<Dens, L, K, ITER, P2P, RAGGED, T>(KMC_FRONT_PACK, a);
}
template <class Dens, int L, int K, int ITER, bool RAGGED>
__global__ __launch_bounds__(vec_tpb(L)) void half_step_de_vec(KMC_FRONT_PARAMS, const HalfStepArgs a)
{
    half_step_vec_body<Dens, L, K, ITER, false, RAGGED, double, Move::DE>(KMC_FRONT_PACK, a);
}
template <class Dens, int L, int K, int ITER, bool RAGGED>
__global__ __launch_bounds__(vec_tpb(L)) void half_step_snooker_vec(KMC_FRONT_PARAMS, const HalfStepArgs a)
{
    half_step_vec_body<Dens, L, K, ITER, false, RAGGED, double, Move::Snooker>(KMC_FRONT_PACK, a);
}
__device__ __forceinline__ const MixTable* mix_table(const HalfStepArgs& a) { return reinterpret_cast<const MixTable*>(a.peer_pos[0]); }
__device__ __forceinline__ bool mix_pick(const HalfStepArgs& a, uint32_t seed_lo, uint32_t seed_hi, uint64_t step, DrawConsts* dc)
{
    const MixTable* t = mix_table(a);
    const int i = mix_member(t, seed_lo, seed_hi, step);
    *dc = a.dc;
    dc->c0 = i == 0 ? t->c0[0] : i == 1 ? t->c0[1] : i == 2 ? t->c0[2] : t->c0[3];
    dc->c1 = i == 0 ? t->c1[0] : i == 1 ? t->c1[1] : i == 2 ? t->c1[2] : t->c1[3];
    const int mv = i == 0 ? t->move[0] : i == 1 ? t->move[1] : i == 2 ? t->move[2] : t->move[3];
    return mv == kMoveIdSnooker;
}
template <class Dens, int L, int K, int ITER, bool RAGGED, bool TEMPER = false>
__device__ __forceinline__ void half_step_mix_vec_body(const HalfStepFront& f, const HalfStepArgs& a)
{
    const uint64_t step = f.sched == nullptr ? (uint64_t)f.step : 2ull * (uint64_t)schedule_entry(f).gen + (uint64_t)f.half();
    DrawConsts dc;
    if (mix_pick(a, f.seed_lo, f.seed_hi, step, &dc)) half_step_vec_body<Dens, L, K, ITER, false, RAGGED, double, Move::Snooker, TEMPER>(f, a, &dc);
    else half_step_vec_body<Dens, L, K, ITER, false, RAGGED, double, Move::DE, TEMPER>(f, a, &dc);
}
template <class Dens, int L, int K, int ITER, bool RAGGED>
__global__ __launch_bounds__(vec_tpb(L)) void half_step_mix_vec(KMC_FRONT_PARAMS, const HalfStepArgs a)
{
    half_step_mix_vec_body<Dens, L, K, ITER, RAGGED>(KMC_FRONT_PACK, a);
}
template <int L, int K, bool RAGGED>
__device__ __forceinline__ HalfStepFront temper_front(HalfStepFront f)
{
    const uint64_t t = blockIdx.y, nw = 2ull * f.nhalf;
    const uint64_t ld = RAGGED ? (((reinterpret_cast<uint64_t>(f.logp) >> 48) + 1ull) & ~1ull) : (uint64_t)(2 * L * K);
    f.pos += t * nw * ld;
    f.logp += t * nw * 2ull;
    return f;
}
template <class Dens, int L, int K, int ITER, bool RAGGED, Move M>
__global__ __launch_bounds__(vec_tpb(L)) void half_step_temper_vec(KMC_FRONT_PARAMS, const HalfStepArgs a)
{
    const HalfStepFront f = temper_front<L, K, RAGGED>(KMC_FRONT_PACK);
    if constexpr (M == Move::Mix) half_step_mix_vec_body<Dens, L, K, ITER, RAGGED, true>(f, a);
    else half_step_vec_body<Dens, L, K, ITER, false, RAGGED, double, M, true>(f, a);
}

struct FlushArgs {
    const double* pos;
    uint32_t*     klast;
    double*       msum;
    double*       msumsq;
    int64_t       macc_stride;
    int64_t       row0;
    int32_t       n_active;
    uint32_t      nsamp;
    int32_t       ld;
};

template <int L, int K, int ITER, class T = double>
__global__ __launch_bounds__(vec_tpb(L)) void flush_moments_vec(const FlushArgs a)
{
    using V2 = typename RowOf<T>::V2;
    constexpr int G = 64 / L;
    constexpr int W = G * ITER;
    const int64_t ld = a.ld;
    const int tid  = blockIdx.x * vec_tpb(L) + threadIdx.x;
    const int lane = threadIdx.x & 63;
    const int j    = lane & (L - 1);
    const int g    = lane / L;
    const int w0   = (tid >> 6) * W;
    double2 ms[K], mq[K];
#pragma unroll
    for (int k = 0; k < K; ++k) { ms[k] = make_double2(0.0, 0.0); mq[k] = make_double2(0.0, 0.0); }
#pragma unroll
    for (int it = 0; it < ITER; ++it) {
        const int i = w0 + it * G + g;
        if (i < a.n_active) {
            const int64_t row = a.row0 + i;
            const double w = (double)(a.nsamp - a.klast[row]);
            const V2* x = reinterpret_cast<const V2*>(reinterpret_cast<const T*>(a.pos) + row * ld);
#pragma unroll
            for (int k = 0; k < K; ++k) {
                const double2 v = 2 * (k * L + j) < (int)ld ? load_row(&x[k * L + j]) : make_double2(0.0, 0.0);
                ms[k].x += v.x * w; ms[k].y += v.y * w;
                mq[k].x += (v.x * v.x) * w; mq[k].y += (v.y * v.y) * w;
            }
        }
    }
    __syncthreads();
#pragma unroll
    for (int it = 0; it < ITER; ++it) {
        const int i = w0 + it * G + g;
        if (i < a.n_active && j == 0) a.klast[a.row0 + i] = a.nsamp;
    }
    const double none[4] = {0.0, 0.0, 0.0, 0.0};
    accumulate_wave<L, K, false>(a.msum, a.msumsq, a.macc_stride, tid, g, ms, mq, ms, mq, none);
}

template <class Dens, bool P2P, class T = double, Move M = Move::Stretch, bool TEMPER = false>
__device__ __forceinline__ void half_step_generic_body(const HalfStepFront& f, const HalfStepArgs& a, const DrawConsts* over = nullptr)
{
    static_assert(!TEMPER || (!P2P && sizeof(T) == 8 && BlobTrait<Dens>::n == 0), "tempering: one GPU, double rows, no blobs");
    const bool rung0 = !TEMPER || blockIdx.y == 0u;
    static_assert(!P2P || sizeof(T) == 8, "the peer-to-peer kernels keep double rows");
    static_assert(M != Move::Mix, "a mixture picks its member in front of the body (half_step_mix_generic_body)");
    constexpr bool kDE = M == Move::DE;
    constexpr bool kSnk = M == Move::Snooker;
    constexpr bool kOwn = kDE || kSnk;
    static_assert(!kOwn || (!P2P && sizeof(T) == 8 && BlobTrait<Dens>::n == 0), "the DE move: one GPU, double rows, no blobs (kmc_validate)");
    const int tid = blockIdx.x * 256 + threadIdx.x;
    const SchedEntry sch = schedule_of(f, a);
    const uint64_t step = 2ull * (uint64_t)sch.gen + (uint64_t)a.half;
    if constexpr (P2P) { if (p2p_nranks(a) > 1) wait_for_peers(a, step, (int)(threadIdx.x & 63)); }
    if (tid >= a.n_active) return;
    const int ndim = a.ndim;
    const bool count  = (sch.flags & kCount) != 0;
    const bool sample = (sch.flags & kSample) != 0 && rung0;
    const int64_t gw = a.own_row0 + tid;
    uint32_t partner_k = 0u;
    uint32_t partner_l = 0u;
    const DrawConsts& dcm = over != nullptr ? *over : a.dc;
    Draw dr = kSnk ? snooker_draw(dcm, step, (uint32_t)(a.gw0 + tid), &partner_k, &partner_l)
            : kDE ? de_draw(dcm, step, (uint32_t)(a.gw0 + tid), &partner_k)
                  : draw_step(a.dc, step, (uint64_t)(a.gw0 + tid));
    const int64_t ld = a.ld;
    T* own = reinterpret_cast<T*>(a.pos) + gw * ld;
    const T* oth;
    const T* othk = nullptr;
    const T* othl = nullptr;
    if constexpr (!P2P) {
        oth = reinterpret_cast<const T*>(a.pos) + (a.oth_row0 + dr.partner) * ld;
        if constexpr (kOwn) othk = reinterpret_cast<const T*>(a.pos) + (a.oth_row0 + partner_k) * ld;
        if constexpr (kSnk) othl = reinterpret_cast<const T*>(a.pos) + (a.oth_row0 + partner_l) * ld;
    } else {
        const uint32_t q = a.hloc_shift >= 0 ? dr.partner >> a.hloc_shift : dr.partner / a.hloc;
        const uint32_t r = dr.partner - q * a.hloc;
        const double* base = a.peer_pos[0];
#pragma unroll
        for (int t = 1; t < 8; ++t) base = (q == (uint32_t)t) ? a.peer_pos[t] : base;
        oth = reinterpret_cast<const T*>(base) + (a.oth_row0 + r) * ld;
    }
    const double p0 = a.logp[gw];
    auto oth_at = [&](int d) -> double {
        if constexpr (P2P) {
            if (p2p_nranks(a) > 1)
                return __longlong_as_double((long long)__hip_atomic_load(reinterpret_cast<const unsigned long long*>(oth) + d,
                                                                         __ATOMIC_RELAXED, __HIP_MEMORY_SCOPE_SYSTEM));
// ... 921 lines not shown
```

kissmcmc.jl_amd/csrc/kmc_launch.hip:

```cpp
#include <algorithm>
#include <cmath>
#include <cstdio>
#include <cstdlib>

#define KMC_DEFINE_LAUNCH_KERNELS
#include "kmc_sampler.hpp"

using namespace kmc;
using namespace kmc_host;

namespace kmc_host {

template <int L, int K, int ITER, class T>
FlushFn flush_one()
{
    if constexpr (ITER <= L && ITER * K <= 16) return flush_moments_vec<L, K, ITER, T>;
    else return nullptr;
}

template <int L, int K>
FlushFn flush_iter(int iter, bool f32)
{
    switch (iter) {
    case 1: return f32 ? flush_one<L, K, 1, float>() : flush_one<L, K, 1, double>();
// ... 487 lines not shown
        if (!s->host_ev[i]) HIP_TRY(hipEventCreateWithFlags(&s->host_ev[i], hipEventDisableTiming));
    bool zero_copy = npiece == 1 && s->h_prop_dev != nullptr && hh * nd * sizeof(double) <= ((size_t)256 << 10);
    { std::string e; if (debug_opt("host-zerocopy", &e)) zero_copy = e == "1" && npiece == 1 && s->h_prop_dev != nullptr; }
    for (; ngen > 0; --ngen) {
        KMC_TRY(chain_before(s, s->generation + 1));
        for (int half = 0; half < 2; ++half) {
            HalfStepArgs a = make_args(s, half, false, s->generation);
            a.prop_out = zero_copy ? s->h_prop_dev : s->d_prop;
            a.prop_ld = zero_copy ? (int32_t)nd : (int32_t)ld;
            HIP_TRY(launch_half_kernel(s, a));
            bool cb_failed = false;
            if (npiece == 1) {
                if (!zero_copy) HIP_TRY(hipMemcpy2DAsync(s->h_prop, nd * sizeof(double), s->d_prop, ld * sizeof(double), nd * sizeof(double), hh,
                                                         hipMemcpyDeviceToHost, s->stream));
                HIP_TRY(hipStreamSynchronize(s->stream));
                cb_failed = s->cfg.host_logpdf(s->h_prop, (int64_t)hh, (int64_t)nd, s->h_p1, s->cfg.host_user) != 0;
            } else {
                auto r0 = [&](int c) { return hh * (size_t)c / (size_t)npiece; };
                for (int c = 0; c < npiece; ++c) {
                    HIP_TRY(hipMemcpy2DAsync(s->h_prop + r0(c) * nd, nd * sizeof(double), s->d_prop + r0(c) * ld, ld * sizeof(double), nd * sizeof(double),
                                             r0(c + 1) - r0(c), hipMemcpyDeviceToHost, s->stream));
                    HIP_TRY(hipEventRecord(s->host_ev[c], s->stream));
                }
                for (int c = 0; c < npiece; ++c) {
                    HIP_TRY(hipEventSynchronize(s->host_ev[c]));
                    if (!cb_failed)
                        cb_failed = s->cfg.host_logpdf(s->h_prop + r0(c) * nd, (int64_t)(r0(c + 1) - r0(c)), (int64_t)nd, s->h_p1 + r0(c), s->cfg.host_user) != 0;
                }
            }
            if (cb_failed) {
                s->positions_set = false;
                return fail(KMC_ERR_BAD_ARG, "the host log-pdf callback failed in generation " + std::to_string(s->generation));
            }
            if (!zero_copy) HIP_TRY(hipMemcpyAsync(s->d_p1, s->h_p1, hh * sizeof(double), hipMemcpyHostToDevice, s->stream));
            a.prop_out = nullptr;
            a.p1_in = zero_copy ? s->h_p1_dev : s->d_p1;
            a.acc_out = s->d_acc;
            HIP_TRY(launch_half_kernel(s, a));
            s->launches += 2;
            if (s->cfg.host_accepted) {
                HIP_TRY(hipMemcpyAsync(s->h_acc, s->d_acc, hh, hipMemcpyDeviceToHost, s->stream));
                HIP_TRY(hipStreamSynchronize(s->stream));
                const int32_t stored = (a.sched_inline.flags & kSample) != 0 ? 1 : 0;
                if (s->cfg.host_accepted(s->h_acc, (int64_t)hh, (int64_t)half * (int64_t)hh, s->generation, stored, s->cfg.host_user) != 0) {
                    s->positions_set = false;
                    return fail(KMC_ERR_BAD_ARG, "the host accept callback failed in generation " + std::to_string(s->generation));
                }
            }
        }
        s->generation += 1;
        KMC_TRY(chain_after(s));
    }
    return KMC_OK;
}

kmc_status eager_generations(kmc_sampler* s, int64_t n, int64_t* left)
{
    for (; n > 0; --n, --*left) {
        KMC_TRY(chain_before(s, s->generation + 1));
        if (s->fused) {
            HIP_TRY(launch_generation(s, s->fused_cur, false, s->generation));
            s->fused_cur ^= 1;
        } else {
            for (int half = 0; half < 2; ++half) KMC_TRY(launch_half(s, half, false, s->generation));
        }
        s->generation += 1;
        s->launches += launches_per_generation(s);
        if (!s->fused && ++s->gens_since_sweep >= kSweepEvery) HIP_TRY(launch_sweep(s));
        KMC_TRY(chain_after(s));
    }
    return KMC_OK;
}

kmc_status graph_chunk(kmc_sampler* s, int64_t* left)
{
    if (s->fused) HIP_TRY(generation_settle(s));
    KMC_TRY(ensure_graph(s));
    if (!s->graph_exec) return eager_generations(s, kGraphChunk, left);
    KMC_TRY(sync_device_counter(s));
    KMC_TRY(chain_before(s, s->generation + kGraphChunk));
    HIP_TRY(hipGraphLaunch(s->graph_exec, s->stream));
    if (!s->fused) HIP_TRY(launch_sweep(s));
    s->generation += kGraphChunk;
    s->dev_gen += kGraphChunk;
    s->launches += (launches_per_generation(s) + (s->temper ? 1 : 0)) * kGraphChunk;
    *left -= kGraphChunk;
    return chain_after(s);
}

kmc_status updated_chunk(kmc_sampler* s, int64_t* left)
{
    if (s->fused) HIP_TRY(generation_settle(s));
    KMC_TRY(chain_before(s, s->generation + s->uchunk));
    bool launched = false;
    if (launch_updated_graph(s, &launched) != KMC_OK) {
        s->launch_mode = 1;
        if (debug_opt("feed-stats")) std::fprintf(stderr, "[kissmcmc_hip] the updated-graph replay failed (%s): table graph from here on\n", kmc_last_error());
        if (!launched) return KMC_OK;
        HIP_TRY(hipStreamSynchronize(s->stream));
    }
    if (!s->fused) HIP_TRY(launch_sweep(s));
    s->generation += s->uchunk;
    s->launches += launches_per_generation(s) * s->uchunk;
    *left -= s->uchunk;
    return chain_after(s);
}

inline int64_t calib_gens(const kmc_sampler* s) { return std::max<int64_t>(4 * kGraphChunk, 2 * s->uchunk); }
inline int64_t calib_min(const kmc_sampler* s) { return kGraphChunk + 2 * std::max<int64_t>(kGraphChunk, s->uchunk) + 2 * calib_gens(s) + kGraphChunk; }

kmc_status calibrate(kmc_sampler* s, bool with_updated, int64_t* left)
{
    hipEvent_t e0 = nullptr, e1 = nullptr, e2 = nullptr;
    HIP_TRY(hipEventCreate(&e0));
    HIP_TRY(hipEventCreate(&e1));
    HIP_TRY(hipEventCreate(&e2));
    const int64_t gens = calib_gens(s);
    kmc_status st = graph_chunk(s, left);
    if (st == KMC_OK) st = with_updated ? updated_chunk(s, left) : eager_generations(s, kGraphChunk, left);
    if (st == KMC_OK) st = with_updated ? updated_chunk(s, left) : eager_generations(s, kGraphChunk, left);
    if (st == KMC_OK && hipEventRecord(e0, s->stream) != hipSuccess) st = KMC_ERR_HIP;
    for (int64_t r = 0; r < gens / kGraphChunk && st == KMC_OK; ++r) st = graph_chunk(s, left);
    if (st == KMC_OK && hipEventRecord(e1, s->stream) != hipSuccess) st = KMC_ERR_HIP;
    if (with_updated) { for (int64_t r = 0; r < gens / s->uchunk && st == KMC_OK && s->launch_mode == 0; ++r) st = updated_chunk(s, left); }
    else if (st == KMC_OK) st = eager_generations(s, gens, left);
    if (st == KMC_OK && hipEventRecord(e2, s->stream) != hipSuccess) st = KMC_ERR_HIP;
    float tg = 0.f, tu = 0.f;
    if (st == KMC_OK && (hipEventSynchronize(e2) != hipSuccess || hipEventElapsedTime(&tg, e0, e1) != hipSuccess ||
                         hipEventElapsedTime(&tu, e1, e2) != hipSuccess)) st = KMC_ERR_HIP;
    (void)hipEventDestroy(e0); (void)hipEventDestroy(e1); (void)hipEventDestroy(e2);
    if (st != KMC_OK) return st == KMC_ERR_HIP ? fail(st, "launch-mode calibration failed") : st;
    if (s->launch_mode == 0) {
        s->launch_mode = tu < 0.98f * tg ? (with_updated ? 3 : 2) : 1;
        s->calib_graph_ms = tg * (float)kGraphChunk / (float)gens; s->calib_eager_ms = tu * (float)kGraphChunk / (float)gens;
    }
    return KMC_OK;
}

enum class LaunchEnv { none, graph, eager, updated, updated_budget };
LaunchEnv launch_env()
{
    static const char* const names[] = {"graph", "eager", "updated", "updated,budget"};
    const char* const e = std::getenv("KMC_LAUNCH");
    for (int i = 0; e && i < 4; ++i)
        if (std::strcmp(e, names[i]) == 0) return (LaunchEnv)(i + 1);
    return LaunchEnv::none;
}

kmc_status decide_launch_mode(kmc_sampler* s, LaunchEnv env, bool use_graph, int64_t* left)
{
    constexpr int64_t kWorthMeasuring = 4096;
    const bool long_job = s->cfg.ngenerations >= kWorthMeasuring || s->generation + *left >= kWorthMeasuring;
    const bool updated_asked = env == LaunchEnv::updated || env == LaunchEnv::updated_budget;
    if (use_graph && s->launch_mode == 0 && s->user && updated_graph_possible(s) && !s->uexec[0] && (updated_asked || (long_job && *left >= calib_min(s)))) {
        if (ensure_updated_graph(s) != KMC_OK) {
            (void)hipGetLastError();
            drop_updated_graph(s);
            s->updated_refused = true;
        }
    }
    if (s->temper && updated_asked) s->temper_updated_fallback = true;
    if (!use_graph || s->launch_mode != 0) return KMC_OK;
    if (env == LaunchEnv::graph) s->launch_mode = 1;
    else if (env == LaunchEnv::eager) s->launch_mode = 2;
    else if (env == LaunchEnv::updated && updated_graph_possible(s)) { s->launch_mode = 3; s->updated_forced = true; }
    else if (env == LaunchEnv::updated_budget && updated_graph_possible(s) && update_budget_left(s)) s->launch_mode = 3;
    else if (!updated_graph_possible(s)) s->launch_mode = 1;
    else if (*left >= calib_min(s) && long_job) {
        const bool room = update_budget_left(s);
        if (!room) note_budget_spent(s);
        KMC_TRY(calibrate(s, room, left));
    }
    return KMC_OK;
}

kmc_status run_launches(kmc_sampler* s, int64_t ngen)
{
    if (s->fused && s->fused_L > 0 && ngen > 0 && !(s->pos2_current && s->own_pos && !s->pos_exposed)) {
        HIP_TRY(generation_settle(s));
        HIP_TRY(hipMemcpyAsync(s->d_pos2, s->d_pos, (size_t)s->nrows * (size_t)s->ld * sizeof(double), hipMemcpyDeviceToDevice, s->stream));
        HIP_TRY(hipMemcpyAsync(s->d_logp2, s->d_logp, (size_t)s->nrows * sizeof(double), hipMemcpyDeviceToDevice, s->stream));
        s->pos2_current = true;
    }
    int64_t left = ngen;
    bool use_graph = !(s->cfg.flags & KMC_NO_GRAPH);
    if (s->comm && !s->comm_graph_ok) use_graph = false;
    KMC_TRY(decide_launch_mode(s, launch_env(), use_graph, &left));
    while (use_graph && s->launch_mode == 3 && left >= s->uchunk) {
        if (!s->updated_forced && !update_budget_left(s)) {
            note_budget_spent(s);
            s->launch_mode = 0;
            if (left >= calib_min(s)) KMC_TRY(calibrate(s, false, &left));
            break;
        }
        KMC_TRY(updated_chunk(s, &left));
    }
    if (s->launch_mode == 2) use_graph = false;
    while (use_graph && left >= kGraphChunk) KMC_TRY(graph_chunk(s, &left));
    KMC_TRY(eager_generations(s, left, &left));
    if (s->fused) HIP_TRY(generation_settle(s));
    return KMC_OK;
}

}

KMC_EXPORT kmc_status kmc_sampler_run(kmc_sampler* s, int64_t ngen)
{
    if (!s || ngen < 0) return fail(KMC_ERR_BAD_ARG, "bad argument");
    if (!s->positions_set) return fail(KMC_ERR_BAD_ARG, "kmc_sampler_set_positions has not succeeded yet");
    if (s->cfg.shard_count != 1 && !s->p2p && !s->comm)
        return fail(KMC_ERR_UNSUPPORTED, "kmc_sampler_run needs shard_count == 1, KMC_P2P or an RCCL communicator (kmc_sampler_rccl_init); "
                                         "other replica-sharded drivers call kmc_sampler_half_step and exchange themselves");
    if (s->p2p && !s->connected) return fail(KMC_ERR_BAD_ARG, "kmc_sampler_p2p_connect has not been called");
    if (s->generation + ngen >= (int64_t)1 << 31) return fail(KMC_ERR_UNSUPPORTED, "at most 2^31 - 1 generations (the step index is 32 bits)");
    if (s->stream_chain && ((s->d_chain && !s->dst_chain) || (s->d_chain_logp && !s->dst_logp)))
        return fail(KMC_ERR_BAD_ARG, "KMC_STREAM_CHAIN: call kmc_sampler_set_chain_host before kmc_sampler_run");
    HIP_TRY(hipSetDevice(s->cfg.device));
    HIP_TRY(hipEventRecord(s->ev0, s->stream));
    const kmc_status st = s->resident ? run_resident(s, ngen) : s->islands ? run_islands(s, ngen) : s->data_eval ? run_data(s, ngen) :
                          s->host_eval ? run_host(s, ngen) : run_launches(s, ngen);
    KMC_TRY(st);
    HIP_TRY(hipEventRecord(s->ev1, s->stream));
    s->have_run_events = true;
    return KMC_OK;
}

KMC_EXPORT kmc_status kmc_sampler_half_step(kmc_sampler* s, int half)
{
    if (!s || (half != 0 && half != 1)) return fail(KMC_ERR_BAD_ARG, "bad argument");
    if (!s->positions_set) return fail(KMC_ERR_BAD_ARG, "kmc_sampler_set_positions has not succeeded yet");
    if (s->p2p && !s->connected) return fail(KMC_ERR_BAD_ARG, "kmc_sampler_p2p_connect has not been called");
    if (s->islands) return fail(KMC_ERR_UNSUPPORTED, "island mode advances whole generations: use kmc_sampler_run");
    if (s->data_eval) return fail(KMC_ERR_UNSUPPORTED, "KMC_DATA_DENSITY: whole generations only; use kmc_sampler_run");
    if (s->host_eval) return fail(KMC_ERR_UNSUPPORTED, "KMC_HOST_DENSITY: a half-step includes the host callback; use kmc_sampler_run");
    if (s->resident) return fail(KMC_ERR_UNSUPPORTED, "this small ensemble runs in resident mode (whole generations per launch); create it with KMC_NO_GRAPH to step by halves");
    HIP_TRY(hipSetDevice(s->cfg.device));
    if (s->fused) KMC_TRY(unfuse(s));
    if (s->generation >= ((int64_t)1 << 31) - 1) return fail(KMC_ERR_UNSUPPORTED, "at most 2^31 - 1 generations (the step index is 32 bits)");
    if (half == 0) KMC_TRY(chain_before(s, s->generation + 1));
    KMC_TRY(launch_half(s, half, false, s->generation));
    s->launches += 1;
    if (half == 1) {
        s->generation += 1;
        if (++s->gens_since_sweep >= kSweepEvery) HIP_TRY(launch_sweep(s));
        KMC_TRY(chain_after(s));
    }
    return KMC_OK;
}

KMC_EXPORT kmc_status kmc_sampler_sync(kmc_sampler* s)
{
    if (!s) return fail(KMC_ERR_BAD_ARG, "null sampler");
    HIP_TRY(hipSetDevice(s->cfg.device));
    HIP_TRY(hipStreamSynchronize(s->stream));
    KMC_TRY(chain_flush(s));
    return check_p2p_err(s);
}

KMC_EXPORT kmc_status kmc_sampler_last_run_ms(kmc_sampler* s, double* ms)
{
    if (!s || !ms) return fail(KMC_ERR_BAD_ARG, "null argument");
    if (!s->have_run_events) return fail(KMC_ERR_BAD_ARG, "no kmc_sampler_run yet");
    HIP_TRY(hipSetDevice(s->cfg.device));
    HIP_TRY(hipEventSynchronize(s->ev1));
    float f = 0.f;
    HIP_TRY(hipEventElapsedTime(&f, s->ev0, s->ev1));
    *ms = (double)f;
    return KMC_OK;
}

KMC_EXPORT int kmc_sampler_launch_mode(const kmc_sampler* s, int* budget_fallback)
{
    if (!s) return -1;
    if (budget_fallback) *budget_fallback = s->budget_fallback ? 1 : 0;
    if (s->resident || s->islands || s->host_eval) return KMC_LAUNCH_SINGLE;
    if ((s->cfg.flags & KMC_NO_GRAPH) || (s->comm && !s->comm_graph_ok)) return KMC_LAUNCH_EAGER;
    return s->launch_mode;
}
```

kissmcmc.jl_amd/csrc/kmc_plan.hip:

```cpp
#include <algorithm>
#include <cmath>
#include <cstdlib>
#include <cstring>

#include "kmc_sampler.hpp"

using namespace kmc;
using namespace kmc_host;

namespace kmc_host {
bool lookup(int density, int L, int K, int iter, bool p2p, bool ragged, bool f32, HalfStepFn* vec, HalfStepFn* gen)
{
    return with_density(density, false, [&](auto d) {
        using D = decltype(d);
        if (p2p && f32) { *vec = nullptr; *gen = nullptr; }
        else if (p2p) density_part<D, 2>(L, K, iter, ragged, false, vec, gen);
        else if (ragged || f32) density_part<D, 1>(L, K, iter, ragged, f32, vec, gen);
        else density_part<D, 0>(L, K, iter, false, false, vec, gen);
        return true;
    });
}

bool lookup_move(int move, int density, int L, int K, int iter, bool ragged, HalfStepFn* vec, HalfStepFn* gen)
{
    return with_density(density, false, [&](auto d) {
        if (move == KMC_MOVE_SNOOKER) density_part<decltype(d), 4>(L, K, iter, ragged, false, vec, gen);
        else if (move == KMC_MOVE_MIX) density_part<decltype(d), 5>(L, K, iter, ragged, false, vec, gen);
        else density_part<decltype(d), 3>(L, K, iter, ragged, false, vec, gen);
        return true;
    });
}

bool lookup_temper(int move, int density, int L, int K, int iter, bool ragged, HalfStepFn* vec, HalfStepFn* gen)
{
    return with_density(density, false, [&](auto d) {
        using D = decltype(d);
        if (move == KMC_MOVE_SNOOKER) temper_part<D, Move::Snooker>(L, K, iter, ragged, vec, gen);
        else if (move == KMC_MOVE_MIX) temper_part<D, Move::Mix>(L, K, iter, ragged, vec, gen);
        else if (move == KMC_MOVE_DE) temper_part<D, Move::DE>(L, K, iter, ragged, vec, gen);
        else temper_part<D, Move::Stretch>(L, K, iter, ragged, vec, gen);
        return true;
    });
}

LogpdfFn logpdf_fn(int density)
{
    return with_density(density, LogpdfFn(nullptr), [](auto d) { return logpdf_lookup<decltype(d)>(); });
}

bool resident_lane_wanted(int64_t ndim)
{
    std::string e;
    if (debug_opt("resident", &e) && e == "pair") return false;
    return ndim <= 8;
}
int lane_nd(int64_t ndim) { return (int)ndim; }

void philox_host(const uint32_t ctr[4], const uint32_t key[2], uint32_t out[4])
{
    uint32_t c0 = ctr[0], c1 = ctr[1], c2 = ctr[2], c3 = ctr[3], k0 = key[0], k1 = key[1];
    for (int r = 0; r < 10; ++r) {
        const uint64_t p0 = (uint64_t)0xD2511F53u * c0, p1 = (uint64_t)0xCD9E8D57u * c2;
        const uint32_t n0 = (uint32_t)(p1 >> 32) ^ c1 ^ k0, n2 = (uint32_t)(p0 >> 32) ^ c3 ^ k1;
        c0 = n0; c1 = (uint32_t)p1; c2 = n2; c3 = (uint32_t)p0;
        k0 += 0x9E3779B9u; k1 += 0xBB67AE85u;
    }
    out[0] = c0; out[1] = c1; out[2] = c2; out[3] = c3;
}

static void affine_perm(const uint32_t ctr[4], uint64_t seed, int64_t n, int64_t* A, int64_t* C)
{
    const uint32_t key[2] = {(uint32_t)seed, (uint32_t)(seed >> 32)};
    uint32_t w[4];
    philox_host(ctr, key, w);
    auto gcd = [](int64_t a, int64_t b) { while (b) { const int64_t t = a % b; a = b; b = t; } return a; };
    int64_t a = (int64_t)((((uint64_t)w[0] << 32) | w[1]) % (uint64_t)n);
    if (a < 1) a = 1;
    while (gcd(a, n) != 1) a = (a + 1 >= n) ? 1 : a + 1;
    *A = a;
    *C = (int64_t)((((uint64_t)w[2] << 32) | w[3]) % (uint64_t)n);
}

void island_perm(uint64_t seed, int64_t epoch, int64_t N, int64_t* A, int64_t* C)
{
    if (epoch == 0 || N <= 2) { *A = 1; *C = 0; return; }
    const uint32_t ctr[4] = {(uint32_t)epoch, (uint32_t)((uint64_t)epoch >> 32), 0x49534c41u, 0u};
    affine_perm(ctr, seed, N, A, C);
}

constexpr uint64_t kDealSeedStride = 0x9E3779B97F4A7C15ull;
uint64_t deal_seed(uint64_t seed, int32_t rank) { return seed + (uint64_t)(rank + 1) * kDealSeedStride; }
void deal_perm(uint64_t seed, int64_t epoch, int32_t rank, int64_t S, int64_t* A, int64_t* C)
{
    const uint32_t ctr[4] = {(uint32_t)epoch, (uint32_t)((uint64_t)epoch >> 32), 0x4445414cu, (uint32_t)rank};
    affine_perm(ctr, seed, S, A, C);
}

Plan make_plan(const kmc_config& c, int64_t n_active)
{
    Plan p;
    HalfStepFn vec = nullptr, gen = nullptr;
    int L = 0, K = 0, iter = 1;
    const char* env = std::getenv("KMC_PLAN");
    bool force_generic = false;
    if (env && std::strcmp(env, "generic") == 0) force_generic = true;
    else if (env && std::sscanf(env, "%d,%d,%d", &L, &K, &iter) == 3) {  }
    else {
        L = 0;
        const int64_t chunks = (c.ndim + 1) / 2;
        auto pow2ceil = [](int64_t v) { int p = 1; while (p < v) p <<= 1; return p; };
        if (chunks <= 4) { L = pow2ceil(chunks); K = 1; }
        else if (chunks <= 128) { L = pow2ceil((chunks + 1) / 2); K = 2; }
        else if (chunks <= 256) { L = 64; K = 4; }
        else if (chunks <= 512) { L = 64; K = 8; }
        if (c.density == KMC_USER_DENSITY && chunks > 64 && chunks <= 128) {
            const kmc_user_density* ud = static_cast<const kmc_user_density*>(c.user_density);
            if (ud && ud->is_body && !sep_routed(ud) && body_vec_possible(ud, c.ndim)) { L = 16; K = 8; }
        }
        iter = 1;
        if (L > 0) {
            const int64_t waves1 = n_active * L / 64;
            if (2 <= L && 2 * K <= 16 && waves1 >= 3072) iter = 2;
            while (iter >= 2 && iter * 2 <= L && iter * 2 * K <= 16 && waves1 / (iter * 2) >= 4096 && iter < 16) iter *= 2;
        }
    }
    const bool de = own_stream_move(c);
    const int tile_cap = c.move == KMC_MOVE_DE ? 8 : 4;
    if (de && (!env || c.move != KMC_MOVE_DE)) while (iter > 1 && iter * K > tile_cap) iter /= 2;
    const bool ragged = L > 0 && 2 * L * K != c.ndim;
    const bool f32 = c.dtype == KMC_F32;
    if ((ragged || f32) && iter > 4) iter = 4;
    if (tempered(c) && iter > 8) iter = 8;
    if ((c.flags & KMC_P2P) && iter > 8) iter = 8;
    p.ragged = ragged;
    if (c.density == KMC_HOST_DENSITY || c.density == KMC_DATA_DENSITY) {
        p.fn = c.move == KMC_MOVE_MIX ? half_step_host_mix() : c.move == KMC_MOVE_SNOOKER ? half_step_host_snooker() : de ? half_step_host_de() : half_step_host(); p.vec = false; p.ragged = false; p.L = 1; p.K = 1; p.ITER = 1;
        if (tempered(c)) {
            if (c.move == KMC_MOVE_SNOOKER) temper_part<HostEval, Move::Snooker>(1, 1, 1, false, &vec, &p.fn);
            else if (c.move == KMC_MOVE_MIX) temper_part<HostEval, Move::Mix>(1, 1, 1, false, &vec, &p.fn);
            else if (c.move == KMC_MOVE_DE) temper_part<HostEval, Move::DE>(1, 1, 1, false, &vec, &p.fn);
            else temper_part<HostEval, Move::Stretch>(1, 1, 1, false, &vec, &p.fn);
        }
        return p;
    }
    if (c.density == KMC_USER_DENSITY) {
        const kmc_user_density* ud = static_cast<const kmc_user_density*>(c.user_density);
        const bool body = ud && ud->is_body && !(sep_routed(ud) || body_vec_possible(ud, c.ndim));
        if (!body && !force_generic && L > 0 && 2 * L * K >= c.ndim && iter <= L && iter * K <= 16) {
            if (ud && ud->is_body && !sep_routed(ud)) while (iter > 1 && body_vec_lds_bytes(L, K, iter) > 65536) iter /= 2;
            p.vec = true; p.L = L; p.K = K; p.ITER = iter;
        } else {
            p.vec = false; p.L = 1; p.K = 1; p.ITER = 1;
        }
        return p;
    }
    if (tempered(c)) lookup_temper(c.move, c.density, L, K, iter, ragged, &vec, &gen);
    else if (de) lookup_move(c.move, c.density, L, K, iter, ragged, &vec, &gen);
    else lookup(c.density, L, K, iter, (c.flags & KMC_P2P) != 0, ragged, f32, &vec, &gen);
    if (!force_generic && L > 0 && 2 * L * K >= c.ndim && vec != nullptr) {
        p.fn = vec; p.vec = true; p.L = L; p.K = K; p.ITER = iter;
    } else {
        p.fn = gen; p.vec = false; p.L = 1; p.K = 1; p.ITER = 1;
    }
    return p;
}

kmc_status check_ndim(int density, int64_t ndim)
{
    if (density == KMC_ROSENBROCK && ndim < 2) return fail(KMC_ERR_BAD_ARG, "rosenbrock needs ndim >= 2");
    if (density == KMC_MVNORMAL2 && ndim != 2) return fail(KMC_ERR_BAD_ARG, "mvnormal2 needs ndim == 2");
    return KMC_OK;
}

}
kmc_status kmc_host::digest_params(const kmc_config& c, DensityParams* dp)
{
    for (double& v : dp->p) v = 0.0;
    dp->ndim = (int32_t)c.ndim;
    dp->pad_ = 0;
    const double* p = c.params;
    switch (c.density) {
    case KMC_USER_DENSITY:
        if (!c.user_density) return fail(KMC_ERR_BAD_ARG, "KMC_USER_DENSITY needs kmc_config.user_density");
        for (int i = 0; i < 6; ++i) dp->p[i] = p[i];
        return KMC_OK;
    case KMC_HOST_DENSITY:
        return KMC_OK;
    case KMC_DATA_DENSITY:
        if (!c.user_density) return fail(KMC_ERR_BAD_ARG, "KMC_DATA_DENSITY needs kmc_config.user_density");
        for (int i = 0; i < 6; ++i) dp->p[i] = p[i];
        return KMC_OK;
    case KMC_GAUSSIAN_ISO:
        if (!(p[1] > 0.0)) return fail(KMC_ERR_BAD_ARG, "gaussian: sigma must be > 0");
        dp->p[0] = p[0]; dp->p[1] = 1.0 / p[1];
        return KMC_OK;
    case KMC_EXPONENTIAL:
        if (!(p[0] > 0.0)) return fail(KMC_ERR_BAD_ARG, "exponential: rate must be > 0");
        dp->p[0] = p[0];
        return KMC_OK;
    case KMC_ROSENBROCK:
        if (!(p[2] > 0.0)) return fail(KMC_ERR_BAD_ARG, "rosenbrock: scale must be > 0");
        dp->p[0] = p[0]; dp->p[1] = p[1]; dp->p[2] = 1.0 / p[2];
        return KMC_OK;
    case KMC_LOGNORMAL:
        if (!(p[1] > 0.0)) return fail(KMC_ERR_BAD_ARG, "lognormal: sigma must be > 0");
        dp->p[0] = p[0]; dp->p[1] = p[1];
        return KMC_OK;
    case KMC_MVNORMAL2:
        for (int i = 0; i < 5; ++i) dp->p[i] = p[i];
        return KMC_OK;
    default:
        return fail(KMC_ERR_BAD_ARG, "unknown density id");
    }
}
```

kissmcmc.jl_amd/csrc/kmc_sampler.hip:

```cpp
#include <algorithm>
#include <cmath>
#include <cstdio>
#include <cstdlib>
#include <mutex>
#include <random>
#include <sstream>

#include "kmc_sampler.hpp"

using namespace kmc;
using namespace kmc_host;

thread_local std::string kmc_host::g_err;

KMC_EXPORT int kmc_version(void) { return KMC_VERSION; }

KMC_EXPORT int kmc_device_count(void)
{
    int n = 0;
    if (hipGetDeviceCount(&n) != hipSuccess) { (void)hipGetLastError(); return 0; }
    return n;
}

KMC_EXPORT const char* kmc_last_error(void) { return g_err.c_str(); }
// ... 842 lines not shown
        s->logpdf_fn = logpdf_fn(cfg->density);
        setup_menu_resident(s);
    }
    setup_generation(s);
    setup_launch_geometry(s);
    KMC_TRY(create_stream(s));
    KMC_TRY(alloc_exchange(s));
    KMC_TRY(alloc_tempering(s));
    KMC_TRY(alloc_state(s));
    KMC_TRY(alloc_draws(s));
    KMC_TRY(alloc_moments(s));
    KMC_TRY(alloc_second_state(s));
    if (s->data_eval) KMC_TRY(alloc_data_route(s));
    else if (s->host_eval) KMC_TRY(alloc_host_route(s));
    KMC_TRY(alloc_chain(s));
    HIP_TRY(hipStreamSynchronize(s->stream));
    if (s->p2p) {
        s->peer_pos[s->cfg.shard_rank] = s->d_pos;
        s->peer_flags[s->cfg.shard_rank] = s->d_flags;
        s->connected = s->cfg.shard_count == 1;
    }
    *out = owner.release();
    return KMC_OK;
}

KMC_EXPORT void kmc_sampler_destroy(kmc_sampler* s)
{
    if (!s) return;
    (void)hipSetDevice(s->cfg.device);
    if (s->stream) (void)hipStreamSynchronize(s->stream);
    if (s->copy_stream) (void)hipStreamSynchronize(s->copy_stream);
    if (s->foreign_stream_seen || s->cfg.shard_count > 1 || s->comm) (void)hipDeviceSynchronize();
    if (s->stream) check_guards(s);
    drop_updated_graph(s);
    if (s->graph_exec) (void)hipGraphExecDestroy(s->graph_exec);
    s->uk.keep.reset();
    if (s->graph) (void)hipGraphDestroy(s->graph);
    if (s->ev0) (void)hipEventDestroy(s->ev0);
    if (s->ev1) (void)hipEventDestroy(s->ev1);
    if (s->p2p) {
        for (int r = 0; r < 8; ++r) {
            if (r == s->cfg.shard_rank) continue;
            if (s->peer_pos[r]) (void)hipIpcCloseMemHandle(s->peer_pos[r]);
            if (s->peer_flags[r]) (void)hipIpcCloseMemHandle(s->peer_flags[r]);
        }
    }
    if (s->comm) { rccl_comm_destroy(s->comm); s->comm = nullptr; }
    if (s->copy_stream) { (void)hipStreamSynchronize(s->copy_stream); (void)hipStreamDestroy(s->copy_stream); }
    for (int i = 0; i < 3; ++i) {
        if (s->ev_filled[i]) (void)hipEventDestroy(s->ev_filled[i]);
        if (s->ev_copied[i]) (void)hipEventDestroy(s->ev_copied[i]);
    }
    chain_unregister(s);
    for (const DevAlloc& a : s->allocs) cache_free(a.p);
    if (s->p2p) {
        cache_free(s->d_flags);
        if ((s->cfg.flags & KMC_P2P_FINEGRAINED) && s->own_pos) cache_free(s->d_pos);
    }
    if (s->h_prop) (void)hipHostFree(s->h_prop);
    if (s->h_p1) (void)hipHostFree(s->h_p1);
    if (s->h_acc) (void)hipHostFree(s->h_acc);
    for (int i = 0; i < kHostPieces; ++i) if (s->host_ev[i]) (void)hipEventDestroy(s->host_ev[i]);
    if (s->own_stream && s->stream) (void)hipStreamDestroy(s->stream);
    (void)hipGetLastError();
    delete s;
}

KMC_EXPORT kmc_status kmc_sampler_set_stream(kmc_sampler* s, void* hip_stream)
{
    if (!s) return fail(KMC_ERR_BAD_ARG, "null sampler");
    HIP_TRY(hipSetDevice(s->cfg.device));
    HIP_TRY(hipStreamSynchronize(s->stream));
    if (s->own_stream && s->stream) (void)hipStreamDestroy(s->stream);
    s->stream = (hipStream_t)hip_stream;
    s->own_stream = false;
    s->foreign_stream_seen = true;
    return KMC_OK;
}

KMC_EXPORT kmc_status kmc_sampler_bind_positions(kmc_sampler* s, void* pos_dev)
{
    if (!s || !pos_dev) return fail(KMC_ERR_BAD_ARG, "null argument");
    if (s->p2p) return fail(KMC_ERR_UNSUPPORTED, "KMC_P2P samplers export their own position buffer");
    if (s->temper) return fail(KMC_ERR_UNSUPPORTED, "parallel tempering: the sampler keeps every rung's rows in its own buffer (no kmc_sampler_bind_positions)");
    if (s->f32) return fail(KMC_ERR_UNSUPPORTED, "kmc_sampler_bind_positions takes double rows; a KMC_F32 sampler keeps its own float rows");
    if (s->ld != s->cfg.ndim) return fail(KMC_ERR_UNSUPPORTED, "kmc_sampler_bind_positions needs an even ndim (16-byte rows)");
    HIP_TRY(hipSetDevice(s->cfg.device));
    HIP_TRY(hipStreamSynchronize(s->stream));
    if (s->graph_exec) { (void)hipGraphExecDestroy(s->graph_exec); s->graph_exec = nullptr; }
    if (s->graph) { (void)hipGraphDestroy(s->graph); s->graph = nullptr; }
    drop_updated_graph(s);
    if (s->own_pos) dev_free(s, s->d_pos);
    s->d_pos = static_cast<double*>(pos_dev);
    s->own_pos = false;
    s->pos2_current = false;
    s->positions_set = false;
    return KMC_OK;
}

KMC_EXPORT int64_t kmc_sampler_generation(const kmc_sampler* s) { return s ? s->generation : -1; }
KMC_EXPORT int64_t kmc_sampler_nsamples(const kmc_sampler* s) { return s ? s->nsamples : -1; }
KMC_EXPORT int64_t kmc_sampler_launch_count(const kmc_sampler* s) { return s ? s->launches : -1; }

namespace {
std::string launch_mode_text(const kmc_sampler* s, const char* what)
{
    std::string t = ((s->cfg.flags & KMC_NO_GRAPH) || s->launch_mode == 2) ? std::string(", eager launches (") + what + " among the preloaded kernel parameters)"
                    : s->launch_mode == 3 ? ", hipGraph replay of " + std::to_string(s->uchunk) + " generations with per-replay parameter updates (" + what + " preloaded)"
                                          : std::string(", hipGraph replay of 64 generations");
    if (s->calib_graph_ms > 0.f) {
        char b[128];
        std::snprintf(b, sizeof(b), " (measured per 64 generations: table graph %.3f ms, %s %.3f ms)", s->calib_graph_ms, s->launch_mode == 2 ? "eager launches" : "updated graph", s->calib_eager_ms);
        t += b;
    }
    return t;
}
}

KMC_EXPORT kmc_status kmc_sampler_describe(const kmc_sampler* s, char* buf, int64_t buflen)
{
    if (!s || !buf || buflen <= 0) return fail(KMC_ERR_BAD_ARG, "bad argument");
    std::ostringstream o;
    if (s->islands)
        o << "island mode: " << s->nislands << " islands of " << s->island_size << " walkers in LDS, " << s->island_gens
          << " generations per launch, rows 2 lanes x " << s->island_K << " chunks";
    else if (s->resident)
        o << "resident mode (exact): whole ensemble in one workgroup's LDS (" << s->resident_tpb
          << " threads), up to " << kDrawTableGens << " generations per launch, "
          << (s->resident_lane2 ? std::string("two walkers per thread") : s->resident_lane ? std::string("one walker per thread") : "rows 2 lanes x " + std::to_string(s->island_K) + " chunks")
          << ", the launch's draws from a wide kernel before it";
    else if (s->fused) {
        if (s->fused_L == 0)
            o << "one launch per generation (exact): generation_lane ND=" << s->cfg.ndim << ", one walker per lane, second-half walkers recompute their partner's first-half move, grid "
              << 2 * ((s->h + s->fused_tpb - 1) / s->fused_tpb) << " x " << s->fused_tpb;
        else
            o << "one launch per generation (exact): generation_group L=" << s->fused_L << " K=" << s->plan.K << ", rows lane-striped, second-half walkers recompute their partner's first-half move, grid "
              << 2 * ((s->h + s->fused_tpb / s->fused_L - 1) / (s->fused_tpb / s->fused_L)) << " x " << s->fused_tpb;
        o << launch_mode_text(s, "generation");
    } else if (s->data_eval) {
        const DataPlan& ph = s->plan_half;
        const int64_t np = (int64_t)s->ntemps * s->h;
        o << "data density (exact): per half-step propose kernel -> " << (ph.obs ? "data_partial_obs (one observation per lane, grid " + std::to_string(np)
                                                                                 : "data_partial_lane (one proposal per lane, grid " + std::to_string((np + 63) / 64))
          << " x " << ph.nblocks << " workgroups of 256, " << ph.rounds << " rounds per wave) -> " << (s->temper_like ? "data_fold_split" : "data_fold") << " -> accept kernel, eager launches; "
          << s->data_ud->ndata << " observations of " << s->data_ud->ncols << " doubles; scratch " << ph.nblocks << " x " << np
          << " tree nodes (at most 4096 x " << (s->temper_like ? "ntemps x " : "") << "nwalkers doubles)";
    } else if (s->host_eval)
        o << "host-evaluated density (exact): per half-step propose kernel -> D2H -> callback -> H2D -> accept kernel, grid "
          << s->grid << " x 256";
    else if (s->plan.vec) {
        o << "multi-launch (exact): half_step_vec L=" << s->plan.L << " K=" << s->plan.K << " ITER=" << s->plan.ITER
          << (s->plan.ragged ? " ragged" : " exact-size") << ", grid " << s->grid << " x " << s->tpb
          << launch_mode_text(s, "step");
    } else
        o << "multi-launch (exact): " << (s->user && s->uk.staged ? "half_step_staged (one walker per lane, rows staged through LDS)" : "half_step_generic (one walker per lane)")
          << ", grid " << s->grid << " x " << s->tpb;
    if (s->feed_replays > 0 && debug_opt("feed-stats")) {
        char b[200];
        std::snprintf(b, sizeof(b), "; feeding thread per replay of %lld generations: wait for a free executable %.1f us, parameter updates %.1f us, hipGraphLaunch %.1f us (%lld replays)",
                      (long long)s->uchunk, s->feed_wait_ns / 1e3 / s->feed_replays, s->feed_update_ns / 1e3 / s->feed_replays, s->feed_launch_ns / 1e3 / s->feed_replays, (long long)s->feed_replays);
        o << b;
    }
    if (s->cfg.move == KMC_MOVE_DE) {
        char b[160];
        std::snprintf(b, sizeof(b), "; differential-evolution move (KMC_MOVE_DE): gamma0 %.6g, sigma %.3g, kernel %s", de_gamma0_of(s->cfg), s->cfg.de_sigma,
                      s->host_eval ? "half_step_de_generic (propose / accept passes)" : s->plan.vec ? "half_step_de_vec" : "half_step_de_generic");
        o << b;
    }
    if (s->cfg.move == KMC_MOVE_SNOOKER) {
        char b[160];
        std::snprintf(b, sizeof(b), "; snooker move (KMC_MOVE_SNOOKER): gamma %.6g, kernel %s", snooker_gamma_of(s->cfg.snooker_gamma),
                      s->host_eval ? "half_step_snooker_generic (propose / accept passes)" : s->plan.vec ? "half_step_snooker_vec" : "half_step_snooker_generic");
        o << b;
    }
    if (s->cfg.move == KMC_MOVE_MIX) {
        double w[KMC_MIX_MAX] = {0.0, 0.0, 0.0, 0.0};
        const MixTable mt = mix_table_of(s->cfg, w);
        o << "; move mixture (KMC_MOVE_MIX), one member per half-step:";
        for (int i = 0; i < mt.count; ++i) {
            char b[160];
            if (mt.move[i] == KMC_MOVE_DE) std::snprintf(b, sizeof(b), " %.6g x DE (gamma0 %.6g, sigma %.3g)", w[i], mt.c0[i], mt.c1[i]);
            else std::snprintf(b, sizeof(b), " %.6g x snooker (gamma %.6g)", w[i], mt.c0[i]);
            o << (i ? "," : "") << b;
        }
        o << ", kernel " << (s->host_eval ? "half_step_mix_generic (propose / accept passes)" : s->plan.vec ? "half_step_mix_vec" : "half_step_mix_generic");
    }
    if (s->temper) {
        o << "; parallel tempering: ntemps " << s->ntemps << " rungs in one launch per half-step (grid y = rung), kernel "
          << (s->plan.vec ? "half_step_temper_vec" : "half_step_temper_generic") << ", betas 1 .. ";
        char b[64];
        std::snprintf(b, sizeof(b), "%.6g", s->betas.back());
        o << b << ", swap sweep " << (s->cfg.swap_every > 0 ? "every " + std::to_string(s->cfg.swap_every) + " generations (" + (s->adapt ? (s->temper_like ? "temper_sweep_adapt<like>" : "temper_sweep_adapt<whole>") : s->temper_like ? "temper_sweep_like" : "temper_sweep") + ")" : std::string("off"));
        if (s->adapt) {
            char ab[96];
            std::snprintf(ab, sizeof(ab), ", lag %.6g, time %.6g", s->cfg.adapt_lag, s->cfg.adapt_time);
            o << "; adaptive ladder: until generation " << s->cfg.adapt_until << ab << " (betas above: the initial ladder)";
        }
        if (s->temper_like) o << "; likelihood tempering: rung t samples prior + beta_t S, four launches per half-step for the whole ladder";
        if (s->temper_updated_fallback) o << "; KMC_LAUNCH=updated asked for: the updated-graph mode is not built for tempered samplers, fell back to the table graph";
    }
    if (s->budget_fallback) o << "; updated-graph budget of the process spent (kmc_set_updated_budget_mb): fell back to " << (s->launch_mode == 2 ? "eager launches" : "the table graph");
    if (s->push) o << "; accepted rows pushed into the peers' local copies (KMC_P2P_PUSH)";
    if (s->f32) o << "; rows kept in float (KMC_F32), arithmetic in double";
    if (s->stream_chain) o << "; chain streamed to host memory in blocks of " << s->ring_blk << " samples (device ring of 3 blocks" << (s->dst_chain_reg || s->dst_logp_reg ? ", destination page-locked" : "") << ")";
    if (s->d_ids) o << "; dealt sub-ensemble " << s->cfg.deal_rank << "/" << s->cfg.deal_count << " (walkers re-dealt between epochs)";
    if (s->d_mring) o << "; moments through a ring of " << s->mring_depth << " posted rows per wave";
    if (s->user) o << "; runtime-compiled density";
    if (s->user && s->user->is_body && s->fused)
        o << (s->fused_L == 0 ? " (function body, evaluated as written: one walker per lane)"
                              : " (function body recognised as a sum over elements and checked against the body on test rows: lane-striped)");
    else if (s->user && s->user->is_body && s->plan.vec && !s->resident && !s->islands)
    {
        const std::string& why_not = s->sep_off ? s->sep_off_note : s->user->sep_note;
        o << ((s->user->sep && !s->sep_off) ? " (function body recognised as a sum over elements and checked against the body on test rows: lane-striped)"
                                            : " (function body: rows lane-striped, the body evaluated per walker on the whole proposal" + (why_not.empty() ? std::string() : "; taken for a sum over elements, but " + why_not) + ")");
    }
    if (s->nblob > 0) o << " with a blob of " << s->nblob << " doubles per walker" << (s->d_chain_blob ? " (stored with every sample)" : "");
    if (s->p2p) o << "; P2P shard " << s->cfg.shard_rank << "/" << s->cfg.shard_count << (s->connected ? "" : " (not connected)");
    else if (s->cfg.shard_count > 1 || s->comm)
        o << "; replica shard " << s->cfg.shard_rank << "/" << s->cfg.shard_count
          << (s->comm ? ((s->comm_graph_ok && !(s->cfg.flags & KMC_NO_GRAPH) && s->launch_mode != 2) ? ", RCCL all-gather of the updated half after every half-step (captured in the graph)"
                                                                                                         : ", RCCL all-gather of the updated half after every half-step (enqueued launch by launch)") : "");
    if (debug_opt("geometry")) {
        const Plan& p = s->plan;
        auto data_plan_text = [](const DataPlan& d) { return std::to_string((int)d.obs) + "/" + std::to_string(d.rounds) + "/" + std::to_string(d.nblocks); };
        o << "; geometry: plan=" << (p.vec ? "vec" : "generic") << "/" << p.L << "/" << p.K << "/" << p.ITER << "/" << (p.ragged ? "ragged" : "exact")
          << " tpb=" << s->tpb << " grid=" << s->grid << " macc_stride=" << s->macc_stride << " macc_elems=" << s->macc_elems << " vec_lds=" << s->vec_lds
          << " nrows=" << s->nrows << " resident=" << s->resident << " resident_tpb=" << s->resident_tpb << " resident_lane=" << s->resident_lane
          << " resident_lane2=" << s->resident_lane2 << " islands=" << s->islands << " island_K=" << s->island_K << " island_ragged=" << s->island_ragged
          << " nislands=" << s->nislands << " island_lds=" << s->island_lds << " fused=" << s->fused << " fused_L=" << s->fused_L
          << " fused_tpb=" << s->fused_tpb << " fused_fold=" << s->fused_fold << " mring_depth=" << s->mring_depth << " mring_waves=" << s->mring_waves
          << " ring_blk=" << s->ring_blk << " ring_slots=" << s->ring_slots << " stream_by_walker=" << s->stream_by_walker << " push=" << s->push
          << " part_doubles=" << s->part_doubles << " plan_half=" << data_plan_text(s->plan_half) << " plan_all=" << data_plan_text(s->plan_all);
        const std::pair<const char*, const void*> bufs[] = {
            {"d_ring", s->d_ring}, {"d_draws", s->d_draws}, {"d_pos2", s->d_pos2}, {"d_glast", s->d_glast}, {"d_isum", s->d_isum}, {"d_msum", s->d_msum},
            {"d_mring", s->d_mring}, {"bw_scratch", s->bw_scratch}, {"bw_scratch_logp", s->bw_scratch_logp}, {"d_ids", s->d_ids}, {"d_mix", s->d_mix},
            {"d_like", s->d_like}, {"d_acc", s->d_acc}, {"d_prop", s->d_prop}, {"d_part", s->d_part}, {"d_betas", s->d_betas}, {"d_chain", s->d_chain},
            {"d_chain_logp", s->d_chain_logp}, {"d_blob", s->d_blob}, {"d_chain_blob", s->d_chain_blob}, {"d_err", s->d_err}};
        for (const auto& b : bufs) o << " " << b.first << "=" << (b.second != nullptr);
    }
    const std::string t = o.str();
    std::snprintf(buf, (size_t)buflen, "%s", t.c_str());
    return KMC_OK;
}

KMC_EXPORT void* kmc_sampler_device_ptr(kmc_sampler* s, int which)
{
    if (!s) return nullptr;
    if (which == 0 || which == 1) s->pos_exposed = true;
    switch (which) {
    case 0: return s->d_pos;
    case 1: return s->d_logp;
    case 2: return s->d_naccept;
    default: return nullptr;
    }
}


KMC_EXPORT int kmc_sizeof_config(void) { return (int)sizeof(kmc_config); }
KMC_EXPORT int kmc_sizeof_metropolis_config(void) { return (int)sizeof(kmc_metropolis_config); }
KMC_EXPORT int kmc_sizeof_outputs(void) { return (int)sizeof(kmc_outputs); }
KMC_EXPORT int kmc_sizeof_metropolis_outputs(void) { return (int)sizeof(kmc_metropolis_outputs); }
```

kissmcmc.jl_amd/csrc/kmc_sampler.hpp:

```cpp
#pragma once
#include <string>
#include <utility>
#include <vector>

#include "kmc_host.hpp"

KMC_EXPORT int kmc_version(void);

namespace kmc_host {

static_assert(1024 % kmc::kDrawBatch == 0, "the draw table holds whole batches");
constexpr int64_t kDrawTableGens = 1024;
constexpr int64_t kGraphChunk = 64;
constexpr int kUExec = 6;
constexpr size_t kGuardBytes = 4096;
constexpr int kHostPieces = 8;

struct Plan {
    kmc::HalfStepFn fn = nullptr;
    bool vec = false;
    bool ragged = false;
    int L = 1, K = 1, ITER = 1;
};

struct UserKernels {
    hipModule_t mod = nullptr;
    std::shared_ptr<void> keep;
    hipFunction_t vec = nullptr, generic = nullptr, logpdf = nullptr, resident = nullptr, island = nullptr, init_ball = nullptr;
    hipFunction_t generation = nullptr;
    hipFunction_t staged = nullptr;
    hipFunction_t logpdf_sep = nullptr;
};

struct UserModuleSpec {
    enum class Resident { None, Pair, Lane, Lane2 };
    enum class Generation { None, Lane, Striped, Quad };
    bool vec = false;
    int L = 0, K = 0, iter = 0;
    bool ragged = false;
    Resident resident = Resident::None;
    int pair_K = 0;
    bool pair_ragged = false;
    int lane_nd = 0;
    int lane_bound = 0;
    int island_S = 0;
    bool f32 = false;
    int64_t ndim = 0;
    bool p2p = false;
    Generation generation = Generation::None;
    int move = KMC_MOVE_STRETCH;
    bool temper = false;

    static UserModuleSpec logpdf_only(int64_t ndim) { UserModuleSpec s; s.ndim = ndim; return s; }
    static UserModuleSpec syntax_check(bool body) { return logpdf_only(body ? 4 : 0); }
    static UserModuleSpec sum_form_check() { UserModuleSpec s; s.vec = true; s.L = 4; s.K = 1; s.iter = 1; s.ndim = 8; return s; }
};

struct DataKernels {
    std::shared_ptr<void> keep, keep_data;
    hipFunction_t lane = nullptr, obs = nullptr, fold = nullptr, fold_split = nullptr;
    const double* data = nullptr;
};
struct DataPlan {
    bool obs = false;
    int32_t rounds = 1;
    int32_t nblocks = 1;
};
constexpr int64_t kDataMaxDim = 32, kDataMaxCols = 16, kDataMaxRows = (int64_t)1 << 30;

struct DevAlloc {
    void* p = nullptr;
    size_t bytes = 0;
    bool guarded = false;
};

}

struct kmc_sampler {
    kmc_config cfg{};
    int64_t h = 0, h_loc = 0, active_begin = 0, nlocal = 0, nsamples = 0;
    int64_t ld = 0;
    kmc::DensityParams dp{};
    kmc_host::Plan plan{};
    bool ragged_vec() const { return plan.vec && plan.ragged; }
    kmc::LogpdfFn logpdf_fn = nullptr;
    kmc_user_density* user = nullptr;
    kmc_host::UserKernels uk{};
    int grid = 0;
    int tpb = 256;
    hipStream_t stream = nullptr;
    bool own_stream = false;
    bool foreign_stream_seen = false;
    double* d_pos = nullptr;
    bool f32 = false;
    bool own_pos = true;
    double* d_logp = nullptr;
    uint32_t* d_naccept = nullptr;
    int64_t* d_gen = nullptr;
    kmc::SchedEntry* d_sched = nullptr;
    double* d_chain = nullptr;
    double* d_chain_logp = nullptr;
    int nblob = 0;
    double* d_blob = nullptr;
    double* d_chain_blob = nullptr;
    double* d_msum = nullptr;
    double* d_msumsq = nullptr;
    double2* d_mring = nullptr;
    double* d_mring_w = nullptr;
    uint32_t* d_mcnt = nullptr;
    int mring_depth = 0;
    int64_t mring_waves = 0;
    int64_t gens_since_sweep = 0;
    uint32_t* d_klast = nullptr;
    double2* d_draws = nullptr;
    double2* d_ring = nullptr;
    int64_t macc_stride = 0, macc_elems = 0;
    bool stream_chain = false;
    int64_t ring_blk = 0, ring_slots = 0;
    hipStream_t copy_stream = nullptr;
    hipEvent_t ev_filled[3] = {}, ev_copied[3] = {};
    double* dst_chain = nullptr;
    double* dst_logp = nullptr;
    bool dst_chain_reg = false, dst_logp_reg = false;
    int64_t blocks_copied = 0;
    int64_t blocks_waited = 0;
    void* comm = nullptr;
    bool comm_graph_ok = true;
    uint32_t* d_ids = nullptr;
    uint64_t user_seed = 0;
    int64_t moment_base = 0;
    int64_t generation = 0;
    int64_t dev_gen = 0;
    int64_t launches = 0;
    int launch_mode = 0;
    float calib_graph_ms = 0.f, calib_eager_ms = 0.f;
    hipGraphExec_t graph_exec = nullptr;
    hipGraph_t graph = nullptr;
    hipGraph_t ugraph = nullptr;
    hipGraphExec_t uexec[kmc_host::kUExec] = {};
    hipEvent_t udone[kmc_host::kUExec] = {};
    bool uinflight[kmc_host::kUExec] = {};
    int unext = 0;
    std::vector<hipGraphNode_t> unodes;
    int64_t uchunk = 128;
    bool updated_forced = false;
    int64_t feed_wait_ns = 0, feed_update_ns = 0, feed_launch_ns = 0, feed_replays = 0;
    unsigned vec_lds = 0;
    bool updated_refused = false;
    bool budget_fallback = false;
    std::vector<kmc_host::DevAlloc> allocs;
    hipEvent_t ev0 = nullptr, ev1 = nullptr;
    bool have_run_events = false;
    bool positions_set = false;
    bool host_eval = false;
    double* d_prop = nullptr;
    double* d_p1 = nullptr;
    double* h_prop = nullptr;
    double* h_p1 = nullptr;
    double* h_prop_dev = nullptr;
    double* h_p1_dev = nullptr;
    uint8_t* d_acc = nullptr;
    uint8_t* h_acc = nullptr;
    hipEvent_t host_ev[kmc_host::kHostPieces] = {};
    bool data_eval = false;
    kmc_user_density* data_ud = nullptr;
    kmc_host::DataKernels dk{};
    double* d_part = nullptr;
    size_t part_doubles = 0;
    kmc_host::DataPlan plan_half{}, plan_all{};
    bool temper_like = false;
    double* d_like = nullptr;
    double* d_prior = nullptr;
    double* d_like_sum = nullptr;
    bool resident = false;
    kmc::ResidentFn resident_kernel = nullptr;
    int resident_tpb = 256;
    bool resident_lane2 = false;
    bool resident_lane = false;
    bool fused = false;
    kmc::GenerationFn generation_kernel = nullptr;
    double* d_pos2 = nullptr;
    double* d_logp2 = nullptr;
    bool sep_off = false;
    std::string sep_off_note;
    bool pos_exposed = false;
    bool pos2_current = false;
    bool fused_fold = false;
    std::vector<double> carry_sum, carry_sumsq;
    uint32_t* d_glast = nullptr;
    int fused_cur = 0;
    int fused_L = 0;
    int fused_tpb = 64;
    bool islands = false;
    kmc::IslandFn island_kernel = nullptr;
    int island_K = 0;
    bool island_ragged = false;
    int64_t island_gens = 32, nislands = 0, island_size = kmc::kIslandSizeDefault;
    size_t island_lds = 0;
    double* d_isum = nullptr;
    double* d_isumsq = nullptr;
    bool p2p = false;
    bool connected = false;
    int64_t nrows = 0;
    unsigned long long* d_flags = nullptr;
    unsigned long long* d_err = nullptr;
    int ntemps = 1;
    bool temper = false;
    bool temper_updated_fallback = false;
    std::vector<double> betas;
    double* d_betas = nullptr;
    double* d_rung_sum = nullptr;
    double* d_tsum = nullptr;
    bool adapt = false;
    std::vector<double> S0;
    double* d_S = nullptr;
    unsigned long long* d_round_acc = nullptr;
    unsigned int* d_ticket = nullptr;
    unsigned long long* d_skipped = nullptr;
    double* d_stage = nullptr;
    unsigned long long* d_nswap = nullptr;
    kmc::MixTable* d_mix = nullptr;
    bool stream_by_walker = false;
    double *bw_scratch = nullptr, *bw_scratch_logp = nullptr;
    std::vector<double> bw_host;
    int64_t flushed_done = -1;
    bool push = false;
    double* peer_pos[8] = {nullptr, nullptr, nullptr, nullptr, nullptr, nullptr, nullptr, nullptr};
    unsigned long long* peer_flags[8] = {nullptr, nullptr, nullptr, nullptr, nullptr, nullptr, nullptr, nullptr};
};

namespace kmc_host {

inline int64_t samples_done(const kmc_sampler* s)
{
    const int64_t post = s->generation - s->cfg.nburnin;
    if (post <= 0) return 0;
    const int64_t k = post / s->cfg.nthin;
    return k < s->nsamples ? k : s->nsamples;
}

inline int64_t launches_per_generation(const kmc_sampler* s) { return s->fused ? 1 : 2; }

Plan make_plan(const kmc_config& c, int64_t n_active);
bool resident_lane_wanted(int64_t ndim);
int lane_nd(int64_t ndim);
void island_perm(uint64_t seed, int64_t epoch, int64_t N, int64_t* A, int64_t* C);
uint64_t deal_seed(uint64_t seed, int32_t rank);
void deal_perm(uint64_t seed, int64_t epoch, int32_t rank, int64_t S, int64_t* A, int64_t* C);

kmc_status ensure_graph(kmc_sampler* s);
kmc_status flush_moments_now(kmc_sampler* s);
kmc_status unfuse(kmc_sampler* s);
kmc::DrawConsts draw_consts(const kmc_sampler* s);
kmc::HalfStepArgs make_args(const kmc_sampler* s, int half, bool graph_mode, int64_t gen_offset);
kmc::HalfStepFront front_of(const kmc::HalfStepArgs& a, bool ragged_vec);
kmc::GenerationArgs make_generation_args(const kmc_sampler* s, int from, bool graph_mode, int64_t gen_offset);
kmc::GenerationFront generation_front_of(const kmc::GenerationArgs& a, int tpb);

bool updated_graph_possible(const kmc_sampler* s);
kmc_status ensure_updated_graph(kmc_sampler* s);
kmc_status launch_updated_graph(kmc_sampler* s, bool* launched);
void drop_updated_graph(kmc_sampler* s);
bool update_budget_left(const kmc_sampler* s);
void note_budget_spent(kmc_sampler* s);

hipError_t upload_rows(const kmc_sampler* s, double* dst_dev, const double* src_host, size_t rows);
hipError_t download_rows(const kmc_sampler* s, double* dst_host, const double* src_dev, size_t rows);
kmc_status chain_before(kmc_sampler* s, int64_t g_end);
kmc_status chain_after(kmc_sampler* s);
kmc_status chain_flush(kmc_sampler* s);
void chain_unregister(kmc_sampler* s);

kmc_status load_user(kmc_user_density* ud, const UserModuleSpec& spec, UserKernels* uk);
void set_offline_compiler_hint(bool wanted);
bool body_vec_possible(const kmc_user_density* ud, int64_t ndim);

kmc_status load_data(kmc_user_density* ud, int64_t ndim, DataKernels* dk);
std::string data_functor_source(const kmc_user_density* ud);
kmc_status data_on_device(kmc_user_density* ud, int dev, std::shared_ptr<void>* keep);
DataPlan data_plan(const kmc_user_density* ud, int64_t nprop);
hipError_t launch_data_eval(const DataKernels& dk, const kmc_user_density* ud, const DataPlan& p, const double* prop, int64_t nprop, int32_t ld,
                            const double* params, double* part, size_t part_doubles, double* out, hipStream_t st, bool split = false);

kmc_status check_p2p_err(kmc_sampler* s);

void check_guards(kmc_sampler* s);
void reinstall_abort_backtrace();

}
```

kissmcmc.jl_amd/csrc/kmc_tables.hpp:

```cpp
#pragma once
#include <type_traits>
#include "kmc_islands.hpp"
#include "kmc_generation.hpp"
#include "kmc_metropolis.hpp"

namespace kmc {

using HalfStepFn = void (*)(KMC_FRONT_TYPES, const HalfStepArgs);
using LogpdfFn = void (*)(const LogpdfArgs);
using FlushFn = void (*)(const FlushArgs);
using IslandFn = void (*)(const IslandArgs);
using ResidentFn = void (*)(const ResidentArgs);
using GenerationFn = void (*)(KMC_GEN_FRONT_TYPES, const GenerationArgs);
using InitBallFn = void (*)(const InitBallArgs);
using MetropolisFn = void (*)(const MetropolisArgs);
using MetropolisTabledFn = void (*)(const MetropolisArgs, const double*, int);

template <class D, int PART> void density_part(int L, int K, int iter, bool ragged, bool f32, HalfStepFn* vec, HalfStepFn* gen);
template <class D, Move M> void temper_part(int L, int K, int iter, bool ragged, HalfStepFn* vec, HalfStepFn* gen);
template <class D> LogpdfFn logpdf_lookup();
template <class D> InitBallFn init_ball_lookup();
template <class D> IslandFn island_lookup(int S, int K, bool ragged);
template <class D> ResidentFn resident_lookup(int tpb, int K, bool ragged);
template <class D> ResidentFn resident_lane_lookup(int ndim, bool f32);
template <class D> ResidentFn resident_lane2_lookup(int ndim);
template <class D> GenerationFn generation_lane_lookup(int ndim);
template <class D> GenerationFn generation_group_lookup(int L, int K);
template <class D> MetropolisFn metropolis_lookup(int ndim);
template <class D> MetropolisTabledFn metropolis_tabled_lookup(int ndim);
HalfStepFn half_step_host();
HalfStepFn half_step_host_de();
HalfStepFn half_step_host_snooker();
HalfStepFn half_step_host_mix();

#ifdef KMC_TABLES_IMPL
template <class D, int L, int K, int ITER, bool P2P, bool RAGGED, class T, Move M>
HalfStepFn vec_one()
{
    if constexpr (ITER > L || ITER * K > 16 || ((M == Move::Snooker || M == Move::Mix) && ITER > 1 && ITER * K > 4)) return nullptr;
    else if constexpr (M == Move::Snooker) return half_step_snooker_vec<D, L, K, ITER, RAGGED>;
    else if constexpr (M == Move::Mix) return half_step_mix_vec<D, L, K, ITER, RAGGED>;
    else if constexpr (M == Move::DE) return half_step_de_vec<D, L, K, ITER, RAGGED>;
    else return half_step_vec<D, L, K, ITER, P2P, RAGGED, T>;
}

template <class D, int L, int K, bool P2P, bool RAGGED, class T, Move M = Move::Stretch>
HalfStepFn vec_iter(int iter)
{
    constexpr bool kWide = !P2P && !RAGGED && sizeof(T) == 8;
    switch (iter) {
    case 1: return vec_one<D, L, K, 1, P2P, RAGGED, T, M>();
    case 2: return vec_one<D, L, K, 2, P2P, RAGGED, T, M>();
    case 4: return vec_one<D, L, K, 4, P2P, RAGGED, T, M>();
    case 8: if constexpr (kWide || (P2P && !RAGGED)) return vec_one<D, L, K, 8, P2P, RAGGED, T, M>(); else return nullptr;
    case 16: if constexpr (kWide) return vec_one<D, L, K, 16, P2P, RAGGED, T, M>(); else return nullptr;
    default: return nullptr;
    }
}

template <class D, int L, int K, int PART>
HalfStepFn vec_pick(int iter, bool ragged, bool f32)
{
    if constexpr (PART == 0) return vec_iter<D, L, K, false, false, double>(iter);
    else if constexpr (PART == 1) {
        if (f32) return ragged ? vec_iter<D, L, K, false, true, float>(iter) : vec_iter<D, L, K, false, false, float>(iter);
        return vec_iter<D, L, K, false, true, double>(iter);
    } else if constexpr (PART == 2) return ragged ? vec_iter<D, L, K, true, true, double>(iter) : vec_iter<D, L, K, true, false, double>(iter);
    else if constexpr (PART == 3) return ragged ? vec_iter<D, L, K, false, true, double, Move::DE>(iter) : vec_iter<D, L, K, false, false, double, Move::DE>(iter);
    else if constexpr (PART == 4) return ragged ? vec_iter<D, L, K, false, true, double, Move::Snooker>(iter) : vec_iter<D, L, K, false, false, double, Move::Snooker>(iter);
    else return ragged ? vec_iter<D, L, K, false, true, double, Move::Mix>(iter) : vec_iter<D, L, K, false, false, double, Move::Mix>(iter);
}

template <class D, int PART>
HalfStepFn vec_lookup(int L, int K, int iter, bool ragged, bool f32)
{
    if constexpr (!D::kHasFrag) {
        return nullptr;
    } else {
#define KMC_LK(l, k) if (L == l && K == k) return vec_pick<D, l, k, PART>(iter, ragged, f32);
        KMC_LK(1, 1) KMC_LK(2, 1) KMC_LK(4, 1) KMC_LK(4, 2) KMC_LK(8, 2) KMC_LK(16, 2) KMC_LK(32, 2) KMC_LK(64, 2)
        KMC_LK(64, 4) KMC_LK(64, 8)
#undef KMC_LK
        if constexpr (PART == 0 && std::is_same<D, GaussianIso>::value) {
#define KMC_LK(l, k) if (L == l && K == k) return vec_iter<D, l, k, false, false, double>(iter);
            KMC_LK(8, 1) KMC_LK(16, 1) KMC_LK(32, 1) KMC_LK(64, 1) KMC_LK(4, 4) KMC_LK(8, 4)
#undef KMC_LK
        }
        return nullptr;
    }
}

template <class D, int PART>
void density_part(int L, int K, int iter, bool ragged, bool f32, HalfStepFn* vec, HalfStepFn* gen)
{
    *vec = vec_lookup<D, PART>(L, K, iter, ragged, f32);
    if constexpr (PART == 0) *gen = half_step_generic<D, false, double>;
    else if constexpr (PART == 1) *gen = f32 ? half_step_generic<D, false, float> : half_step_generic<D, false, double>;
    else if constexpr (PART == 2) *gen = half_step_generic<D, true, double>;
    else if constexpr (PART == 3) *gen = half_step_de_generic<D>;
    else if constexpr (PART == 4) *gen = half_step_snooker_generic<D>;
    else *gen = half_step_mix_generic<D>;
}

template <class D, int L, int K, int ITER, bool RAGGED, Move M>
HalfStepFn temper_one()
{
    if constexpr (ITER > L || ITER * K > 16 || ((M == Move::Snooker || M == Move::Mix) && ITER > 1 && ITER * K > 4)) return nullptr;
    else return half_step_temper_vec<D, L, K, ITER, RAGGED, M>;
}
template <class D, int L, int K, bool RAGGED, Move M>
HalfStepFn temper_iter(int iter)
{
    switch (iter) {
    case 1: return temper_one<D, L, K, 1, RAGGED, M>();
    case 2: return temper_one<D, L, K, 2, RAGGED, M>();
    case 4: return temper_one<D, L, K, 4, RAGGED, M>();
    case 8: if constexpr (!RAGGED) return temper_one<D, L, K, 8, RAGGED, M>(); else return nullptr;
    default: return nullptr;
    }
}
template <class D, Move M>
void temper_part(int L, int K, int iter, bool ragged, HalfStepFn* vec, HalfStepFn* gen)
{
    *vec = nullptr;
    *gen = half_step_temper_generic<D, M>;
    if constexpr (D::kHasFrag) {
#define KMC_LK(l, k) if (L == l && K == k) *vec = ragged ? temper_iter<D, l, k, true, M>(iter) : temper_iter<D, l, k, false, M>(iter);
        KMC_LK(1, 1) KMC_LK(2, 1) KMC_LK(4, 1) KMC_LK(4, 2) KMC_LK(8, 2) KMC_LK(16, 2) KMC_LK(32, 2) KMC_LK(64, 2)
        KMC_LK(64, 4) KMC_LK(64, 8)
#undef KMC_LK
    }
}

template <class D>
LogpdfFn logpdf_lookup() { return logpdf_rows<D>; }
template <class D>
InitBallFn init_ball_lookup() { return init_ball<D>; }

template <class D, int S>
IslandFn island_lookup_s(int K, bool ragged)
{
    switch (K) {
    case 1: return ragged ? island_epoch<D, S, 1, true> : island_epoch<D, S, 1, false>;
    case 2: return ragged ? island_epoch<D, S, 2, true> : island_epoch<D, S, 2, false>;
    case 4: return ragged ? island_epoch<D, S, 4, true> : island_epoch<D, S, 4, false>;
    case 8: return ragged ? island_epoch<D, S, 8, true> : island_epoch<D, S, 8, false>;
    default: return nullptr;
    }
}

template <class D>
IslandFn island_lookup(int S, int K, bool ragged)
{
    if constexpr (!D::kHasFrag) {
        return nullptr;
    } else {
        switch (S) {
        case 64: return island_lookup_s<D, 64>(K, ragged);
        case 128: return island_lookup_s<D, 128>(K, ragged);
        case 256: return island_lookup_s<D, 256>(K, ragged);
        default: return nullptr;
        }
    }
}
template <class D, int TPB>
ResidentFn resident_lookup_t(int K, bool ragged)
{
    switch (K) {
    case 1: return ragged ? resident_epoch<D, 1, true, TPB> : resident_epoch<D, 1, false, TPB>;
    case 2: return ragged ? resident_epoch<D, 2, true, TPB> : resident_epoch<D, 2, false, TPB>;
    case 4: return ragged ? resident_epoch<D, 4, true, TPB> : resident_epoch<D, 4, false, TPB>;
    case 8: return ragged ? resident_epoch<D, 8, true, TPB> : resident_epoch<D, 8, false, TPB>;
    default: return nullptr;
    }
}

template <class D>
ResidentFn resident_lookup(int tpb, int K, bool ragged)
{
    if constexpr (!D::kHasFrag) {
        return nullptr;
    } else {
        switch (tpb) {
        case 256: return resident_lookup_t<D, 256>(K, ragged);
        case 512: return resident_lookup_t<D, 512>(K, ragged);
        case 1024: return resident_lookup_t<D, 1024>(K, ragged);
        default: return nullptr;
        }
    }
}
template <class D, class T>
ResidentFn resident_lane_lookup_t(int ndim)
{
    switch (ndim) {
    case 1: return resident_lane<D, 1, T>;
    case 2: return resident_lane<D, 2, T>;
    case 3: return resident_lane<D, 3, T>;
    case 4: return resident_lane<D, 4, T>;
    case 5: return resident_lane<D, 5, T>;
    case 6: return resident_lane<D, 6, T>;
    case 7: return resident_lane<D, 7, T>;
    case 8: return resident_lane<D, 8, T>;
    default: return nullptr;
    }
}
template <class D>
ResidentFn resident_lane_lookup(int ndim, bool f32)
{
    return f32 ? resident_lane_lookup_t<D, float>(ndim) : resident_lane_lookup_t<D, double>(ndim);
}
template <class D>
ResidentFn resident_lane2_lookup(int ndim)
{
    switch (ndim) {
    case 1: return resident_lane2<D, 1>;
    case 2: return resident_lane2<D, 2>;
    case 3: return resident_lane2<D, 3>;
    case 4: return resident_lane2<D, 4>;
    case 5: return resident_lane2<D, 5>;
    case 6: return resident_lane2<D, 6>;
    case 7: return resident_lane2<D, 7>;
    case 8: return resident_lane2<D, 8>;
    default: return nullptr;
    }
}
template <class D>
GenerationFn generation_lane_lookup(int ndim)
{
    switch (ndim) {
    case 1: return generation_lane<D, 1>;
    case 2: return generation_lane<D, 2>;
    case 3: return generation_lane<D, 3>;
    case 4: return generation_lane<D, 4>;
    case 5: return generation_lane<D, 5>;
    case 6: return generation_lane<D, 6>;
    case 7: return generation_lane<D, 7>;
    case 8: return generation_lane<D, 8>;
    default: return nullptr;
    }
}
template <class D>
GenerationFn generation_group_lookup(int L, int K)
{
    if constexpr (!D::kHasFrag) {
        return nullptr;
    } else {
#define KMC_LK(l, k) if (L == l && K == k) return generation_group<D, l, k>;
        KMC_LK(1, 1) KMC_LK(2, 1) KMC_LK(4, 1) KMC_LK(4, 2) KMC_LK(8, 2) KMC_LK(16, 2) KMC_LK(32, 2) KMC_LK(64, 2)
        KMC_LK(64, 4) KMC_LK(64, 8)
#undef KMC_LK
        return nullptr;
    }
}
template <class D>
MetropolisFn metropolis_lookup(int ndim)
{
    if (ndim <= 1) return metropolis_chains<D, 1>;
    if (ndim <= 2) return metropolis_chains<D, 2>;
    if (ndim <= 4) return metropolis_chains<D, 4>;
    if (ndim <= 8) return metropolis_chains<D, 8>;
    if (ndim <= 16) return metropolis_chains<D, 16>;
    if (ndim <= 32) return metropolis_chains<D, 32>;
    return metropolis_chains<D, 0>;
}
template <class D>
MetropolisTabledFn metropolis_tabled_lookup(int ndim)
{
    if (ndim <= 1) return metropolis_chains_tabled<D, 1>;
    if (ndim <= 2) return metropolis_chains_tabled<D, 2>;
    if (ndim <= 4) return metropolis_chains_tabled<D, 4>;
    if (ndim <= 8) return metropolis_chains_tabled<D, 8>;
    return nullptr;
}
#define KMC_INSTANTIATE_PART(D, PART) template void density_part<D, PART>(int, int, int, bool, bool, HalfStepFn*, HalfStepFn*)
#define KMC_INSTANTIATE_TEMPER(D, M) template void temper_part<D, M>(int, int, int, bool, HalfStepFn*, HalfStepFn*)
#define KMC_INSTANTIATE_ROWS(D) \
    template LogpdfFn logpdf_lookup<D>(); \
    template InitBallFn init_ball_lookup<D>()
#define KMC_INSTANTIATE_LDS(D) \
    template IslandFn island_lookup<D>(int, int, bool); \
    template ResidentFn resident_lookup<D>(int, int, bool); \
    template ResidentFn resident_lane_lookup<D>(int, bool); \
    template ResidentFn resident_lane2_lookup<D>(int); \
    template GenerationFn generation_lane_lookup<D>(int); \
    template GenerationFn generation_group_lookup<D>(int, int); \
    template MetropolisFn metropolis_lookup<D>(int); \
    template MetropolisTabledFn metropolis_tabled_lookup<D>(int)
#endif

}
```

kissmcmc.jl_amd/csrc/kmc_updated.hip:

```cpp
#include <atomic>
#include <chrono>
#include <cstdio>

#include "kmc_sampler.hpp"

using namespace kmc;
using namespace kmc_host;

namespace kmc_host {

namespace {
struct ParamPack {
    HalfStepFront hf;
    HalfStepArgs ha;
    GenerationFront gf;
    GenerationArgs ga;
    void* ptrs[11];
    explicit ParamPack(bool fused)
    {
        if (fused) {
            ptrs[0] = &gf.sched; ptrs[1] = &gf.pin; ptrs[2] = &gf.lin; ptrs[3] = &gf.pout; ptrs[4] = &gf.seed_lo; ptrs[5] = &gf.seed_hi;
            ptrs[6] = &gf.h; ptrs[7] = &gf.nb; ptrs[8] = &gf.ld; ptrs[9] = &gf.gen; ptrs[10] = &ga;
        } else {
            ptrs[0] = &hf.pos; ptrs[1] = &hf.sched; ptrs[2] = &hf.ring_now; ptrs[3] = &hf.logp; ptrs[4] = &hf.gw0; ptrs[5] = &hf.nact_half;
            ptrs[6] = &hf.seed_lo; ptrs[7] = &hf.seed_hi; ptrs[8] = &hf.nhalf; ptrs[9] = &hf.step; ptrs[10] = &ha;
        }
    }
};

hipKernelNodeParams node_params(const kmc_sampler* s, ParamPack* pk)
{
    hipKernelNodeParams np{};
    if (s->fused) {
        np.func = s->user ? reinterpret_cast<void*>(s->uk.generation) : reinterpret_cast<void*>(s->generation_kernel);
        np.gridDim = dim3(2u * pk->ga.nb);
        np.blockDim = dim3((unsigned)s->fused_tpb);
        np.sharedMemBytes = 0u;
    } else {
        np.func = s->user ? reinterpret_cast<void*>(s->uk.vec) : reinterpret_cast<void*>(s->plan.fn);
        np.gridDim = dim3((unsigned)s->grid);
        np.blockDim = dim3((unsigned)s->tpb);
        np.sharedMemBytes = s->user ? s->vec_lds : 0u;
    }
    np.kernelParams = pk->ptrs;
    np.extra = nullptr;
    return np;
}

template <class Visit>
kmc_status for_each_node(const kmc_sampler* s, int64_t g0, Visit&& visit)
{
    ParamPack pk(s->fused);
    const int64_t per_gen = launches_per_generation(s);
    for (int64_t k = 0; k < per_gen * s->uchunk; ++k) {
        const int64_t g = k / per_gen;
        if (s->fused) {
            pk.ga = make_generation_args(s, (int)(g & 1), false, g0 + g);
            pk.gf = generation_front_of(pk.ga, s->fused_tpb);
        } else {
            pk.ha = make_args(s, (int)(k & 1), false, g0 + g);
            pk.hf = front_of(pk.ha, s->ragged_vec());
        }
        KMC_TRY(visit(k, node_params(s, &pk)));
    }
    return KMC_OK;
}
}

void drop_updated_graph(kmc_sampler* s)
{
    for (int i = 0; i < kUExec; ++i) {
        if (s->uexec[i]) { (void)hipGraphExecDestroy(s->uexec[i]); s->uexec[i] = nullptr; }
        if (s->udone[i]) { (void)hipEventDestroy(s->udone[i]); s->udone[i] = nullptr; }
        s->uinflight[i] = false;
    }
    s->unext = 0;
    if (s->ugraph) { (void)hipGraphDestroy(s->ugraph); s->ugraph = nullptr; }
}

bool updated_graph_possible(const kmc_sampler* s)
{
    if (s->p2p || s->host_eval || s->islands || s->resident || s->comm || s->updated_refused) return false;
    if (s->temper) return false;
    if (s->fused) return s->user ? s->uk.generation != nullptr : s->generation_kernel != nullptr;
    return s->user ? (s->plan.vec && s->uk.vec != nullptr) : s->plan.fn != nullptr;
}

kmc_status ensure_updated_graph(kmc_sampler* s)
{
    if (s->uexec[0]) return KMC_OK;
    HIP_TRY(hipGraphCreate(&s->ugraph, 0));
    s->unodes.assign((size_t)(launches_per_generation(s) * s->uchunk), nullptr);
    hipGraphNode_t prev = nullptr;
    KMC_TRY(for_each_node(s, 0, [&](int64_t k, const hipKernelNodeParams& np) -> kmc_status {
        hipGraphNode_t node = nullptr;
        HIP_TRY(hipGraphAddKernelNode(&node, s->ugraph, prev ? &prev : nullptr, prev ? 1 : 0, &np));
        s->unodes[(size_t)k] = node;
        prev = node;
        return KMC_OK;
    }));
    for (int i = 0; i < kUExec; ++i) {
        HIP_TRY(hipGraphInstantiate(&s->uexec[i], s->ugraph, nullptr, nullptr, 0));
        HIP_TRY(hipEventCreateWithFlags(&s->udone[i], hipEventDisableTiming));
    }
    return KMC_OK;
}

namespace {
double update_bytes_each()
{
    static const double b = [] {
        int v = 0;
        return (hipRuntimeGetVersion(&v) == hipSuccess && v >= 70200000) ? 2.0 : 80.0;
    }();
    return b;
}
std::atomic<int64_t> g_update_calls{0};
std::atomic<int64_t>& update_budget()
{
    static std::atomic<int64_t> budget{[] {
        double mb = 64.0;
        std::string v;
        if (debug_opt("updated-budget-mb", &v) && !v.empty()) mb = std::atof(v.c_str());
        return (int64_t)(mb * 1048576.0 / update_bytes_each());
    }()};
    return budget;
}
}

bool update_budget_left(const kmc_sampler* s)
{
    return g_update_calls.load(std::memory_order_relaxed) + launches_per_generation(s) * s->uchunk <= update_budget().load(std::memory_order_relaxed);
}

void note_budget_spent(kmc_sampler* s)
{
    s->budget_fallback = true;
    static std::atomic<bool> said{false};
    if (!said.exchange(true))
        std::fprintf(stderr, "[kissmcmc_hip] the updated-graph launch mode has used up this process's budget (%lld parameter updates, "
                             "kmc_set_updated_budget_mb / KMC_DEBUG=updated-budget-mb=n; this HIP runtime keeps ~%.0f B per update): samplers now "
                             "choose between the table graph and eager launches (up to ~9 %% slower per half-step; results are identical)\n",
                     (long long)g_update_calls.load(std::memory_order_relaxed), update_bytes_each());
}

kmc_status launch_updated_graph(kmc_sampler* s, bool* launched)
{
    *launched = false;
    KMC_TRY(ensure_updated_graph(s));
    g_update_calls.fetch_add(launches_per_generation(s) * s->uchunk, std::memory_order_relaxed);
    const int i = s->unext;
    const auto t_wait0 = std::chrono::steady_clock::now();
    if (s->uinflight[i]) { HIP_TRY(hipEventSynchronize(s->udone[i])); s->uinflight[i] = false; }
    const auto t_upd0 = std::chrono::steady_clock::now();
    KMC_TRY(for_each_node(s, s->generation, [&](int64_t k, const hipKernelNodeParams& np) -> kmc_status {
        HIP_TRY(hipGraphExecKernelNodeSetParams(s->uexec[i], s->unodes[(size_t)k], &np));
        return KMC_OK;
    }));
    const auto t_upd1 = std::chrono::steady_clock::now();
    HIP_TRY(hipGraphLaunch(s->uexec[i], s->stream));
    const auto t_launch1 = std::chrono::steady_clock::now();
    s->feed_wait_ns += std::chrono::duration_cast<std::chrono::nanoseconds>(t_upd0 - t_wait0).count();
    s->feed_update_ns += std::chrono::duration_cast<std::chrono::nanoseconds>(t_upd1 - t_upd0).count();
    s->feed_launch_ns += std::chrono::duration_cast<std::chrono::nanoseconds>(t_launch1 - t_upd1).count();
    s->feed_replays += 1;
    *launched = true;
    HIP_TRY(hipEventRecord(s->udone[i], s->stream));
    s->uinflight[i] = true;
    s->unext = (i + 1) % kUExec;
    return KMC_OK;
}

}

KMC_EXPORT void kmc_updated_budget(int64_t* calls_used, int64_t* calls_budget)
{
    if (calls_used) *calls_used = g_update_calls.load(std::memory_order_relaxed);
    if (calls_budget) *calls_budget = update_budget().load(std::memory_order_relaxed);
}

KMC_EXPORT void kmc_set_updated_budget_mb(double mb)
{
    update_budget().store(mb <= 0.0 ? 0 : (int64_t)(mb * 1048576.0 / update_bytes_each()), std::memory_order_relaxed);
}
```

Before: 8.772 billion.

## Add phase-specialised half-step kernel variant for post-burn-in updated-graph replays

```diff
diff --git a/include/kissmcmc_hip.h b/include/kissmcmc_hip.h
--- a/include/kissmcmc_hip.h
+++ b/include/kissmcmc_hip.h
@@ -396,6 +396,7 @@
                                       int64_t nw, int64_t dst_stride, double* dst_host, int64_t dst_len, int device);
 kmc_status  kmc_debug_rows_compact(const double* src_host, int64_t rows, int64_t ld, int64_t nd, double* dst_host, int64_t dst_len,
                                    int device);
+int         kmc_debug_phase_spec(int density, int L, int K, int iter);
 
 #ifdef __cplusplus
 }
diff --git a/kissmcmc.jl_amd/_lib.py b/kissmcmc.jl_amd/_lib.py
--- a/kissmcmc.jl_amd/_lib.py
+++ b/kissmcmc.jl_amd/_lib.py
@@ -43,7 +43,7 @@
     "kmc_sampler_get_walker_ids", "kmc_sampler_set_walker_ids", "kmc_sampler_set_chain_host", "kmc_rccl_unique_id", "kmc_sampler_rccl_init",
     "kmc_sampler_rccl_capture", "kmc_sampler_rccl_set_capture", "kmc_rccl_version", "kmc_device_free_bytes",
     "kmc_sampler_launch_mode", "kmc_updated_budget", "kmc_set_updated_budget_mb", "kmc_debug_accept_terms",
-    "kmc_debug_chain_by_walker", "kmc_debug_rows_compact",
+    "kmc_debug_chain_by_walker", "kmc_debug_rows_compact", "kmc_debug_phase_spec",
     "kmc_user_density_create_body_blob", "kmc_user_density_nblob", "kmc_logpdf_blob_eval_host", "kmc_sampler_get_blobs",
     "kmc_device_cache_release", "kmc_user_density_is_separable", "kmc_host_prefault", "kmc_data_density_create",
     "kmc_sampler_get_rung_state", "kmc_sampler_set_rung_state", "kmc_sampler_get_swaps",
@@ -330,6 +330,8 @@
     L.kmc_debug_accept_terms.argtypes = [C.c_uint64, C.c_uint64, C.c_uint64, C.c_int64, C.c_int64, C.c_double, C.c_int64, C.c_int, ip, dp, dp, dp]
     L.kmc_debug_chain_by_walker.argtypes = [vp, C.c_int, C.c_int64, C.c_int64, C.c_int64, C.c_int64, C.c_int64, C.c_int64, C.c_int64, dp, C.c_int64, C.c_int]
     L.kmc_debug_rows_compact.argtypes = [dp, C.c_int64, C.c_int64, C.c_int64, dp, C.c_int64, C.c_int]
+    L.kmc_debug_phase_spec.restype = C.c_int
+    L.kmc_debug_phase_spec.argtypes = [C.c_int, C.c_int, C.c_int, C.c_int]
     for fn, T in ((L.kmc_sizeof_config, Config), (L.kmc_sizeof_metropolis_config, MetropolisConfig),
                   (L.kmc_sizeof_outputs, Outputs), (L.kmc_sizeof_metropolis_outputs, MetropolisOutputs)):
         if fn() != C.sizeof(T):
diff --git a/kissmcmc.jl_amd/build.py b/kissmcmc.jl_amd/build.py
--- a/kissmcmc.jl_amd/build.py
+++ b/kissmcmc.jl_amd/build.py
@@ -8,7 +8,7 @@
 CSRC = os.path.join(_HERE, "csrc")
 LIB = os.path.join(_HERE, "libkissmcmc_hip.so")
 SOURCES = ["kmc_sampler.hip", "kmc_plan.hip", "kmc_launch.hip", "kmc_updated.hip", "kmc_state.hip", "kmc_copy.hip", "kmc_rtc.hip", "kmc_p2p.hip", "kmc_metropolis_api.hip", "kmc_acorr.hip", "kmc_summary.hip", "kmc_hist.hip", "kmc_convergence.hip", "kmc_rank.hip", "kmc_cov.hip", "kmc_pointwise.hip", "kmc_rccl.hip", "kmc_diag.hip", "kmc_inst_host.hip", "kmc_inst_host_temper.hip", "kmc_inst_host_temper_snooker.hip", "kmc_data.hip"] + \
-          [f"kmc_inst_{d}{part}.hip" for part in ("", "_var", "_p2p", "_lds", "_de", "_snooker", "_temper", "_temper_snooker") for d in ("lognormal", "exponential", "gaussian_iso", "rosenbrock", "mvnormal2")]
+          [f"kmc_inst_{d}{part}.hip" for part in ("", "_var", "_p2p", "_lds", "_spec", "_de", "_snooker", "_temper", "_temper_snooker") for d in ("lognormal", "exponential", "gaussian_iso", "rosenbrock", "mvnormal2")]
 HEADERS = ["kmc_psis_fit.hpp", "kmc_host.hpp", "kmc_sampler.hpp", "kmc_device.hpp", "kmc_kernels.hpp", "kmc_islands.hpp", "kmc_generation.hpp", "kmc_copy_kernels.hpp", "kmc_summary_kernels.hpp", "kmc_hist_kernels.hpp", "kmc_convergence_kernels.hpp", "kmc_convergence_host.hpp", "kmc_rank_kernels.hpp", "kmc_cov_kernels.hpp", "kmc_chain_view.hpp", "kmc_chain_kernels.hpp", "kmc_metropolis.hpp", "kmc_tables.hpp", "kmc_recognise.hpp", "kmc_data.hpp", "kmc_pointwise.hpp", os.path.join("..", "..", "include", "kissmcmc_hip.h")]
 PRELOAD = ["-mllvm", "-amdgpu-kernarg-preload-count=14"]
 FLAGS = ["--offload-arch=gfx950", "-O3", "-std=c++17", "-fPIC", "-ffp-contract=off",
diff --git a/kissmcmc.jl_amd/csrc/kmc_inst_exponential_spec.hip b/kissmcmc.jl_amd/csrc/kmc_inst_exponential_spec.hip
--- /dev/null
+++ b/kissmcmc.jl_amd/csrc/kmc_inst_exponential_spec.hip
@@ -0,0 +1,6 @@
+#define KMC_TABLES_IMPL
+#include "kmc_tables.hpp"
+
+namespace kmc {
+KMC_INSTANTIATE_SPEC(Exponential);
+}
diff --git a/kissmcmc.jl_amd/csrc/kmc_inst_gaussian_iso_spec.hip b/kissmcmc.jl_amd/csrc/kmc_inst_gaussian_iso_spec.hip
--- /dev/null
+++ b/kissmcmc.jl_amd/csrc/kmc_inst_gaussian_iso_spec.hip
@@ -0,0 +1,13 @@
+#define KMC_TABLES_IMPL
+#include "kmc_tables.hpp"
+
+namespace kmc {
+KMC_INSTANTIATE_SPEC(GaussianIso);
+}
+
+#ifdef KMC_PROBE
+extern "C" __attribute__((visibility("default"))) int kmc_probe_read_spec(void* out)
+{
+    return (int)hipMemcpyFromSymbol(out, HIP_SYMBOL(kmc::g_probe), sizeof(kmc::g_probe));
+}
+#endif
diff --git a/kissmcmc.jl_amd/csrc/kmc_inst_lognormal_spec.hip b/kissmcmc.jl_amd/csrc/kmc_inst_lognormal_spec.hip
--- /dev/null
+++ b/kissmcmc.jl_amd/csrc/kmc_inst_lognormal_spec.hip
@@ -0,0 +1,6 @@
+#define KMC_TABLES_IMPL
+#include "kmc_tables.hpp"
+
+namespace kmc {
+KMC_INSTANTIATE_SPEC(LogNormal);
+}
diff --git a/kissmcmc.jl_amd/csrc/kmc_inst_mvnormal2_spec.hip b/kissmcmc.jl_amd/csrc/kmc_inst_mvnormal2_spec.hip
--- /dev/null
+++ b/kissmcmc.jl_amd/csrc/kmc_inst_mvnormal2_spec.hip
@@ -0,0 +1,6 @@
+#define KMC_TABLES_IMPL
+#include "kmc_tables.hpp"
+
+namespace kmc {
+KMC_INSTANTIATE_SPEC(MvNormal2);
+}
diff --git a/kissmcmc.jl_amd/csrc/kmc_inst_rosenbrock_spec.hip b/kissmcmc.jl_amd/csrc/kmc_inst_rosenbrock_spec.hip
--- /dev/null
+++ b/kissmcmc.jl_amd/csrc/kmc_inst_rosenbrock_spec.hip
@@ -0,0 +1,6 @@
+#define KMC_TABLES_IMPL
+#include "kmc_tables.hpp"
+
+namespace kmc {
+KMC_INSTANTIATE_SPEC(Rosenbrock);
+}
diff --git a/kissmcmc.jl_amd/csrc/kmc_kernels.hpp b/kissmcmc.jl_amd/csrc/kmc_kernels.hpp
--- a/kissmcmc.jl_amd/csrc/kmc_kernels.hpp
+++ b/kissmcmc.jl_amd/csrc/kmc_kernels.hpp
@@ -15,6 +15,7 @@
 };
 static_assert(sizeof(SchedEntry) == 32, "schedule_of loads an entry as eight dwords");
 enum : uint32_t { kCount = 1u, kSample = 2u };
+enum class Spec { Generic, Credit };
 
 __host__ __device__ inline SchedEntry make_sched(int64_t gen, int64_t nburnin, int64_t nthin, int64_t nsamples, int64_t ring_slots = 0)
 {
@@ -311,9 +312,12 @@
 #define KMC_STAMP(i) do { } while (0)
 #endif
 
-template <class Dens, int L, int K, int ITER, bool P2P, bool RAGGED, class T = double, Move M = Move::Stretch, bool TEMPER = false>
+template <class Dens, int L, int K, int ITER, bool P2P, bool RAGGED, class T = double, Move M = Move::Stretch, bool TEMPER = false, Spec SP = Spec::Generic>
 __device__ __forceinline__ void half_step_vec_body(const HalfStepFront& f, const HalfStepArgs& a, const DrawConsts* over = nullptr)
 {
+    constexpr bool kSpec = SP != Spec::Generic;
+    static_assert(!kSpec || (M == Move::Stretch && !P2P && !RAGGED && !TEMPER && sizeof(T) == 8 && ITER <= 2 && BlobTrait<Dens>::n == 0 && RowEvalTrait<Dens>::n == 0),
+                  "phase-specialised instances: the stretch move, one GPU, double rows of exact size, menu densities with a fragment form");
     static_assert(!TEMPER || (!P2P && sizeof(T) == 8 && BlobTrait<Dens>::n == 0), "tempering: one GPU, double rows, no blobs (kmc_validate)");
     const uint32_t rung = TEMPER ? (uint32_t)blockIdx.y : 0u;
     const uint32_t rung_w0 = TEMPER ? rung * (2u * f.nhalf) : 0u;
@@ -358,8 +362,8 @@
     const int  jq     = j / ITER, js = j - jq * ITER;
     const bool useA   = jq == 0;
     const int  iA     = w0 + (kOwn || jq < Q ? js : 0) * G + g;
-    const bool validA = useA && (iA < nact);
-    const int      iAc = iA < nact ? iA : nact - 1;
+    const bool validA = useA && (kSpec || iA < nact);
+    const int      iAc = kSpec || iA < nact ? iA : nact - 1;
     const int64_t  rowA = own_row0 + iAc;
     const bool ring_on = kRing && f.ring_now != nullptr;
     double2 e0 = zero2, e1 = zero2;
@@ -374,7 +378,7 @@
 #pragma unroll
     for (int it = 0; it < ITER; ++it) {
         const int i = w0 + it * G + g;
-        validB[it] = i < nact;
+        validB[it] = kSpec || i < nact;
         const V2* own = reinterpret_cast<const V2*>(posT + row_off(own_row0 + (validB[it] ? i : nact - 1)));
 #pragma unroll
         for (int k = 0; k < K; ++k) xc[it][k] = load_row(&own[ck[k]]);
@@ -387,7 +391,7 @@
     const uint32_t na = naccept_p[rowA];
     const uint32_t kl = klast_p[rowA];
 
-    const bool eager = f.sched == nullptr;
+    const bool eager = kSpec || f.sched == nullptr;
     SchedEntry sch_t{0, 0, 0u, 0u, {0u, 0u}};
     if (!eager) sch_t = schedule_entry(f);
     const uint64_t step = eager ? (uint64_t)f.step : 2ull * (uint64_t)sch_t.gen + (uint64_t)half;
@@ -476,22 +480,28 @@
     __builtin_amdgcn_sched_barrier(0);
     KMC_STAMP(2);
 
+    if constexpr (SP == Spec::Generic)
     asm volatile("" :: "s"(a.chain), "s"(a.chain_logp), "s"(a.chain_rows), "s"(a.chain_row0),
                  "s"(a.msum), "s"(a.msumsq), "s"(a.macc_stride), "s"(a.sched_inline.gen), "s"(a.sched_inline.slot),
                  "s"(a.sched_inline.flags), "s"(a.sched_inline.nbefore));
-    int eager_late = eager ? 1 : 0;
-    asm volatile("" : "+v"(eager_late));
-    eager_late = __builtin_amdgcn_readfirstlane(eager_late);
+    else asm volatile("" :: "s"(a.msum), "s"(a.msumsq), "s"(a.macc_stride), "s"(a.sched_inline.nbefore));
     SchedEntry sch = sch_t;
-    if (eager_late != 0) sch = a.sched_inline;
-    const bool count  = (sch.flags & kCount) != 0;
-    const bool sample = (sch.flags & kSample) != 0 && (!TEMPER || rung == 0u);
+    if constexpr (kSpec) {
+        sch.nbefore = a.sched_inline.nbefore;
+    } else {
+        int eager_late = eager ? 1 : 0;
+        asm volatile("" : "+v"(eager_late));
+        eager_late = __builtin_amdgcn_readfirstlane(eager_late);
+        if (eager_late != 0) sch = a.sched_inline;
+    }
+    const bool count  = kSpec || (sch.flags & kCount) != 0;
+    const bool sample = !kSpec && (sch.flags & kSample) != 0 && (!TEMPER || rung == 0u);
     double beta = 1.0;
     if constexpr (TEMPER) beta = reinterpret_cast<const double*>(a.peer_pos[1])[rung];
     DrawConsts dc = a.dc;
     dc.seed_lo = f.seed_lo; dc.seed_hi = f.seed_hi; dc.nhalf = f.nhalf;
     if (over != nullptr) { dc.c0 = over->c0; dc.c1 = over->c1; }
-    const bool do_mom = count && a.msum != nullptr && (!TEMPER || rung == 0u);
+    const bool do_mom = kSpec || (count && a.msum != nullptr && (!TEMPER || rung == 0u));
     constexpr bool kPrefetchAcc = K <= 2 && L != 64;
     constexpr bool kMomRing = !kPrefetchAcc && !FoldT<L, K>::on && L == 64;
     if constexpr (kMomRing) asm volatile("" :: "s"(a.mring), "s"(a.mring_w), "s"(a.mcnt), "s"(a.mswept), "s"(a.mring_depth));
@@ -550,7 +560,7 @@
     } else if (!fresh) {
         dr.lu = log_pos_normal(ua);
         if constexpr (kRing) {
-            if (ring_on && jq >= 1 && jq < Q && iA < nact) {
+            if (ring_on && jq >= 1 && jq < Q && (kSpec || iA < nact)) {
                 double2* slot = a.ring + ((int64_t)((a.ring_slot + jq) & 3) * a.ring_rows + rowA) * 2;
                 store_wt(&slot[0], make_double2(dr.t1, dr.lu));
                 store_wt(&slot[1], make_double2(dr.z, __hiloint2double((int)(uint32_t)(step + 2ull * (uint64_t)jq), (int)dr.partner)));
@@ -771,6 +781,11 @@
 __global__ __launch_bounds__(vec_tpb(L)) void half_step_vec(KMC_FRONT_PARAMS, const HalfStepArgs a)
 {
     half_step_vec_body<Dens, L, K, ITER, P2P, RAGGED, T>(KMC_FRONT_PACK, a);
+}
+template <class Dens, int L, int K, int ITER, Spec SP>
+__global__ __launch_bounds__(vec_tpb(L)) void half_step_vec_spec(KMC_FRONT_PARAMS, const HalfStepArgs a)
+{
+    half_step_vec_body<Dens, L, K, ITER, false, false, double, Move::Stretch, false, SP>(KMC_FRONT_PACK, a);
 }
 template <class Dens, int L, int K, int ITER, bool RAGGED>
 __global__ __launch_bounds__(vec_tpb(L)) void half_step_de_vec(KMC_FRONT_PARAMS, const HalfStepArgs a)
diff --git a/kissmcmc.jl_amd/csrc/kmc_launch.hip b/kissmcmc.jl_amd/csrc/kmc_launch.hip
--- a/kissmcmc.jl_amd/csrc/kmc_launch.hip
+++ b/kissmcmc.jl_amd/csrc/kmc_launch.hip
@@ -663,7 +663,7 @@
     constexpr int64_t kWorthMeasuring = 4096;
     const bool long_job = s->cfg.ngenerations >= kWorthMeasuring || s->generation + *left >= kWorthMeasuring;
     const bool updated_asked = env == LaunchEnv::updated || env == LaunchEnv::updated_budget;
-    if (use_graph && s->launch_mode == 0 && s->user && updated_graph_possible(s) && !s->uexec[0] && (updated_asked || (long_job && *left >= calib_min(s)))) {
+    if (use_graph && s->launch_mode == 0 && s->user && updated_graph_possible(s) && !s->uexec[0][0] && (updated_asked || (long_job && *left >= calib_min(s)))) {
         if (ensure_updated_graph(s) != KMC_OK) {
             (void)hipGetLastError();
             drop_updated_graph(s);
diff --git a/kissmcmc.jl_amd/csrc/kmc_plan.hip b/kissmcmc.jl_amd/csrc/kmc_plan.hip
--- a/kissmcmc.jl_amd/csrc/kmc_plan.hip
+++ b/kissmcmc.jl_amd/csrc/kmc_plan.hip
@@ -41,6 +41,11 @@
         else temper_part<D, Move::Stretch>(L, K, iter, ragged, vec, gen);
         return true;
     });
+}
+
+HalfStepFn lookup_spec(int density, int L, int K, int iter)
+{
+    return with_density(density, HalfStepFn(nullptr), [&](auto d) { return spec_part<decltype(d)>(L, K, iter); });
 }
 
 LogpdfFn logpdf_fn(int density)
@@ -159,6 +164,7 @@
     else lookup(c.density, L, K, iter, (c.flags & KMC_P2P) != 0, ragged, f32, &vec, &gen);
     if (!force_generic && L > 0 && 2 * L * K >= c.ndim && vec != nullptr) {
         p.fn = vec; p.vec = true; p.L = L; p.K = K; p.ITER = iter;
+        if (!tempered(c) && !de && !(c.flags & KMC_P2P) && !ragged && !f32 && iter <= 2) p.fn_credit = lookup_spec(c.density, L, K, iter);
     } else {
         p.fn = gen; p.vec = false; p.L = 1; p.K = 1; p.ITER = 1;
     }
@@ -213,3 +219,8 @@
         return fail(KMC_ERR_BAD_ARG, "unknown density id");
     }
 }
+
+KMC_EXPORT int kmc_debug_phase_spec(int density, int L, int K, int iter)
+{
+    return kmc_host::lookup_spec(density, L, K, iter) != nullptr ? 1 : 0;
+}
diff --git a/kissmcmc.jl_amd/csrc/kmc_sampler.hip b/kissmcmc.jl_amd/csrc/kmc_sampler.hip
--- a/kissmcmc.jl_amd/csrc/kmc_sampler.hip
+++ b/kissmcmc.jl_amd/csrc/kmc_sampler.hip
@@ -1018,6 +1018,11 @@
         o << "multi-launch (exact): half_step_vec L=" << s->plan.L << " K=" << s->plan.K << " ITER=" << s->plan.ITER
           << (s->plan.ragged ? " ragged" : " exact-size") << ", grid " << s->grid << " x " << s->tpb
           << launch_mode_text(s, "step");
+        if (s->launch_mode == 3 && !(s->cfg.flags & KMC_NO_GRAPH)) {
+            const char* why = nullptr;
+            if (spec_variant_possible(s, kVarCredit, &why)) o << "; phase-specialised kernel instance in counted replays";
+            else o << "; generic kernel in every phase (" << why << ")";
+        }
     } else
         o << "multi-launch (exact): " << (s->user && s->uk.staged ? "half_step_staged (one walker per lane, rows staged through LDS)" : "half_step_generic (one walker per lane)")
           << ", grid " << s->grid << " x " << s->tpb;
diff --git a/kissmcmc.jl_amd/csrc/kmc_sampler.hpp b/kissmcmc.jl_amd/csrc/kmc_sampler.hpp
--- a/kissmcmc.jl_amd/csrc/kmc_sampler.hpp
+++ b/kissmcmc.jl_amd/csrc/kmc_sampler.hpp
@@ -13,11 +13,13 @@
 constexpr int64_t kDrawTableGens = 1024;
 constexpr int64_t kGraphChunk = 64;
 constexpr int kUExec = 6;
+enum : int { kVarGeneric = 0, kVarCredit = 1, kUVariants = 2 };
 constexpr size_t kGuardBytes = 4096;
 constexpr int kHostPieces = 8;
 
 struct Plan {
     kmc::HalfStepFn fn = nullptr;
+    kmc::HalfStepFn fn_credit = nullptr;
     bool vec = false;
     bool ragged = false;
     int L = 1, K = 1, ITER = 1;
@@ -136,12 +138,12 @@
     float calib_graph_ms = 0.f, calib_eager_ms = 0.f;
     hipGraphExec_t graph_exec = nullptr;
     hipGraph_t graph = nullptr;
-    hipGraph_t ugraph = nullptr;
-    hipGraphExec_t uexec[kmc_host::kUExec] = {};
+    hipGraph_t ugraph[kmc_host::kUVariants] = {};
+    hipGraphExec_t uexec[kmc_host::kUVariants][kmc_host::kUExec] = {};
     hipEvent_t udone[kmc_host::kUExec] = {};
     bool uinflight[kmc_host::kUExec] = {};
     int unext = 0;
-    std::vector<hipGraphNode_t> unodes;
+    std::vector<hipGraphNode_t> unodes[kmc_host::kUVariants];
     int64_t uchunk = 128;
     bool updated_forced = false;
     int64_t feed_wait_ns = 0, feed_update_ns = 0, feed_launch_ns = 0, feed_replays = 0;
@@ -258,6 +260,8 @@
 kmc::GenerationFront generation_front_of(const kmc::GenerationArgs& a, int tpb);
 
 bool updated_graph_possible(const kmc_sampler* s);
+bool spec_variant_possible(const kmc_sampler* s, int variant, const char** why_not = nullptr);
+int spec_of_chunk(const kmc_sampler* s, int64_t g0, int64_t n);
 kmc_status ensure_updated_graph(kmc_sampler* s);
 kmc_status launch_updated_graph(kmc_sampler* s, bool* launched);
 void drop_updated_graph(kmc_sampler* s);
diff --git a/kissmcmc.jl_amd/csrc/kmc_tables.hpp b/kissmcmc.jl_amd/csrc/kmc_tables.hpp
--- a/kissmcmc.jl_amd/csrc/kmc_tables.hpp
+++ b/kissmcmc.jl_amd/csrc/kmc_tables.hpp
@@ -18,6 +18,7 @@
 
 template <class D, int PART> void density_part(int L, int K, int iter, bool ragged, bool f32, HalfStepFn* vec, HalfStepFn* gen);
 template <class D, Move M> void temper_part(int L, int K, int iter, bool ragged, HalfStepFn* vec, HalfStepFn* gen);
+template <class D> HalfStepFn spec_part(int L, int K, int iter);
 template <class D> LogpdfFn logpdf_lookup();
 template <class D> InitBallFn init_ball_lookup();
 template <class D> IslandFn island_lookup(int S, int K, bool ragged);
@@ -132,6 +133,24 @@
     }
 }
 
+template <class D, int L, int K, int ITER>
+HalfStepFn spec_one()
+{
+    if constexpr (ITER <= L && ITER * K <= 16) return half_step_vec_spec<D, L, K, ITER, Spec::Credit>;
+    else return nullptr;
+}
+template <class D>
+HalfStepFn spec_part(int L, int K, int iter)
+{
+    if constexpr (D::kHasFrag && BlobTrait<D>::n == 0 && RowEvalTrait<D>::n == 0) {
+#define KMC_LK(l, k) if (L == l && K == k) return iter == 1 ? spec_one<D, l, k, 1>() : iter == 2 ? spec_one<D, l, k, 2>() : nullptr;
+        KMC_LK(1, 1) KMC_LK(2, 1) KMC_LK(4, 1) KMC_LK(4, 2) KMC_LK(8, 2) KMC_LK(16, 2) KMC_LK(32, 2) KMC_LK(64, 2)
+        KMC_LK(64, 4) KMC_LK(64, 8)
+#undef KMC_LK
+    }
+    return nullptr;
+}
+
 template <class D>
 LogpdfFn logpdf_lookup() { return logpdf_rows<D>; }
 template <class D>
@@ -274,6 +293,7 @@
 }
 #define KMC_INSTANTIATE_PART(D, PART) template void density_part<D, PART>(int, int, int, bool, bool, HalfStepFn*, HalfStepFn*)
 #define KMC_INSTANTIATE_TEMPER(D, M) template void temper_part<D, M>(int, int, int, bool, HalfStepFn*, HalfStepFn*)
+#define KMC_INSTANTIATE_SPEC(D) template HalfStepFn spec_part<D>(int, int, int)
 #define KMC_INSTANTIATE_ROWS(D) \
     template LogpdfFn logpdf_lookup<D>(); \
     template InitBallFn init_ball_lookup<D>()
diff --git a/kissmcmc.jl_amd/csrc/kmc_updated.hip b/kissmcmc.jl_amd/csrc/kmc_updated.hip
--- a/kissmcmc.jl_amd/csrc/kmc_updated.hip
+++ b/kissmcmc.jl_amd/csrc/kmc_updated.hip
@@ -28,7 +28,12 @@
     }
 };
 
-hipKernelNodeParams node_params(const kmc_sampler* s, ParamPack* pk)
+HalfStepFn variant_fn(const kmc_sampler* s, int variant)
+{
+    return variant == kVarCredit ? s->plan.fn_credit : s->plan.fn;
+}
+
+hipKernelNodeParams node_params(const kmc_sampler* s, int variant, ParamPack* pk)
 {
     hipKernelNodeParams np{};
     if (s->fused) {
@@ -37,7 +42,7 @@
         np.blockDim = dim3((unsigned)s->fused_tpb);
         np.sharedMemBytes = 0u;
     } else {
-        np.func = s->user ? reinterpret_cast<void*>(s->uk.vec) : reinterpret_cast<void*>(s->plan.fn);
+        np.func = s->user ? reinterpret_cast<void*>(s->uk.vec) : reinterpret_cast<void*>(variant_fn(s, variant));
         np.gridDim = dim3((unsigned)s->grid);
         np.blockDim = dim3((unsigned)s->tpb);
         np.sharedMemBytes = s->user ? s->vec_lds : 0u;
@@ -48,7 +53,7 @@
 }
 
 template <class Visit>
-kmc_status for_each_node(const kmc_sampler* s, int64_t g0, Visit&& visit)
+kmc_status for_each_node(const kmc_sampler* s, int variant, int64_t g0, Visit&& visit)
 {
     ParamPack pk(s->fused);
     const int64_t per_gen = launches_per_generation(s);
@@ -61,7 +66,7 @@
             pk.ha = make_args(s, (int)(k & 1), false, g0 + g);
             pk.hf = front_of(pk.ha, s->ragged_vec());
         }
-        KMC_TRY(visit(k, node_params(s, &pk)));
+        KMC_TRY(visit(k, node_params(s, variant, &pk)));
     }
     return KMC_OK;
 }
@@ -70,12 +75,37 @@
 void drop_updated_graph(kmc_sampler* s)
 {
     for (int i = 0; i < kUExec; ++i) {
-        if (s->uexec[i]) { (void)hipGraphExecDestroy(s->uexec[i]); s->uexec[i] = nullptr; }
+        for (int v = 0; v < kUVariants; ++v)
+            if (s->uexec[v][i]) { (void)hipGraphExecDestroy(s->uexec[v][i]); s->uexec[v][i] = nullptr; }
         if (s->udone[i]) { (void)hipEventDestroy(s->udone[i]); s->udone[i] = nullptr; }
         s->uinflight[i] = false;
     }
     s->unext = 0;
-    if (s->ugraph) { (void)hipGraphDestroy(s->ugraph); s->ugraph = nullptr; }
+    for (int v = 0; v < kUVariants; ++v)
+        if (s->ugraph[v]) { (void)hipGraphDestroy(s->ugraph[v]); s->ugraph[v] = nullptr; }
+}
+
+bool spec_variant_possible(const kmc_sampler* s, int variant, const char** why_not)
+{
+    const char* why = nullptr;
+    std::string v;
+    const int64_t per_wg = (int64_t)(s->tpb / 64) * (64 / s->plan.L) * s->plan.ITER;
+    if (variant == kVarGeneric) return true;
+    if (debug_opt("spec", &v) && v == "0") why = "KMC_DEBUG=spec=0";
+    else if (s->user || s->fused || s->host_eval || !s->plan.vec) why = "not the two-launch vector route of a menu density";
+    else if (variant_fn(s, variant) == nullptr) why = "no instance for this move, row type or geometry";
+    else if (s->h_loc != (int64_t)s->grid * per_wg) why = "grid not full";
+    else if (variant == kVarCredit && !s->d_msum) why = "moments off";
+    else if (variant == kVarCredit && (s->d_chain || s->d_chain_logp || s->d_chain_blob)) why = "chain on";
+    if (why_not) *why_not = why;
+    return why == nullptr;
+}
+
+int spec_of_chunk(const kmc_sampler* s, int64_t g0, int64_t n)
+{
+    (void)n;
+    if (g0 >= s->cfg.nburnin) return spec_variant_possible(s, kVarCredit) ? kVarCredit : kVarGeneric;
+    return kVarGeneric;
 }
 
 bool updated_graph_possible(const kmc_sampler* s)
@@ -88,21 +118,22 @@
 
 kmc_status ensure_updated_graph(kmc_sampler* s)
 {
-    if (s->uexec[0]) return KMC_OK;
-    HIP_TRY(hipGraphCreate(&s->ugraph, 0));
-    s->unodes.assign((size_t)(launches_per_generation(s) * s->uchunk), nullptr);
-    hipGraphNode_t prev = nullptr;
-    KMC_TRY(for_each_node(s, 0, [&](int64_t k, const hipKernelNodeParams& np) -> kmc_status {
-        hipGraphNode_t node = nullptr;
-        HIP_TRY(hipGraphAddKernelNode(&node, s->ugraph, prev ? &prev : nullptr, prev ? 1 : 0, &np));
-        s->unodes[(size_t)k] = node;
-        prev = node;
-        return KMC_OK;
-    }));
-    for (int i = 0; i < kUExec; ++i) {
-        HIP_TRY(hipGraphInstantiate(&s->uexec[i], s->ugraph, nullptr, nullptr, 0));
-        HIP_TRY(hipEventCreateWithFlags(&s->udone[i], hipEventDisableTiming));
-    }
+    if (s->uexec[kVarGeneric][0]) return KMC_OK;
+    for (int v = 0; v < kUVariants; ++v) {
+        if (!spec_variant_possible(s, v)) continue;
+        HIP_TRY(hipGraphCreate(&s->ugraph[v], 0));
+        s->unodes[v].assign((size_t)(launches_per_generation(s) * s->uchunk), nullptr);
+        hipGraphNode_t prev = nullptr;
+        KMC_TRY(for_each_node(s, v, 0, [&](int64_t k, const hipKernelNodeParams& np) -> kmc_status {
+            hipGraphNode_t node = nullptr;
+            HIP_TRY(hipGraphAddKernelNode(&node, s->ugraph[v], prev ? &prev : nullptr, prev ? 1 : 0, &np));
+            s->unodes[v][(size_t)k] = node;
+            prev = node;
+            return KMC_OK;
+        }));
+        for (int i = 0; i < kUExec; ++i) HIP_TRY(hipGraphInstantiate(&s->uexec[v][i], s->ugraph[v], nullptr, nullptr, 0));
+    }
+    for (int i = 0; i < kUExec; ++i) HIP_TRY(hipEventCreateWithFlags(&s->udone[i], hipEventDisableTiming));
     return KMC_OK;
 }
 
@@ -150,15 +181,17 @@
     KMC_TRY(ensure_updated_graph(s));
     g_update_calls.fetch_add(launches_per_generation(s) * s->uchunk, std::memory_order_relaxed);
     const int i = s->unext;
+    int v = spec_of_chunk(s, s->generation, s->uchunk);
+    if (!s->uexec[v][i]) v = kVarGeneric;
     const auto t_wait0 = std::chrono::steady_clock::now();
     if (s->uinflight[i]) { HIP_TRY(hipEventSynchronize(s->udone[i])); s->uinflight[i] = false; }
     const auto t_upd0 = std::chrono::steady_clock::now();
-    KMC_TRY(for_each_node(s, s->generation, [&](int64_t k, const hipKernelNodeParams& np) -> kmc_status {
-        HIP_TRY(hipGraphExecKernelNodeSetParams(s->uexec[i], s->unodes[(size_t)k], &np));
+    KMC_TRY(for_each_node(s, v, s->generation, [&](int64_t k, const hipKernelNodeParams& np) -> kmc_status {
+        HIP_TRY(hipGraphExecKernelNodeSetParams(s->uexec[v][i], s->unodes[v][(size_t)k], &np));
         return KMC_OK;
     }));
     const auto t_upd1 = std::chrono::steady_clock::now();
-    HIP_TRY(hipGraphLaunch(s->uexec[i], s->stream));
+    HIP_TRY(hipGraphLaunch(s->uexec[v][i], s->stream));
     const auto t_launch1 = std::chrono::steady_clock::now();
     s->feed_wait_ns += std::chrono::duration_cast<std::chrono::nanoseconds>(t_upd0 - t_wait0).count();
     s->feed_update_ns += std::chrono::duration_cast<std::chrono::nanoseconds>(t_upd1 - t_upd0).count();
```

Result: faster. 8.969 billion (median of 6 runs) (+2.2%).
